# ansonb/FeTA_TMLR

Hardware: AMD Instinct MI355X
Metric: graphs/sec fwd+bwd, ZINC batch (N<=37,d=64,K=16) (higher is better)
Workload: dtype f32; 1 GPU; ZINC-shaped synthetic padded-graph batch, ChebConvDynamic block (attention + coefficient generator + spectral filter), fwd+bwd; graphs_per_gpu=128, global_batch=128, n_pad=37, d_model=64, heads=4, filter_order=4, k_eig=16, filter_mode=spectral, layers=3, norm=batch(per-rank stats), hip_graph=True, backward=single, two_phase=False, graph_collectives=False, ranks=1, parallelism=dp1

## Files before the change

feta_tmlr_amd/build.py:

```python
import os
import subprocess
import sys
from concurrent.futures import ThreadPoolExecutor

PKG = os.path.dirname(os.path.abspath(__file__))
ROOT = os.path.dirname(PKG)
CSRC = os.path.join(PKG, 'csrc')
OUT = os.path.join(PKG, 'libfeta_hip.so')
OBJ = os.path.join(PKG, 'csrc', 'build')
ARCH = 'gfx950'


def _hipcc():
    for c in (os.environ.get('HIPCC'), '/opt/rocm/bin/hipcc', 'hipcc'):
        if c and (os.path.isabs(c) and os.path.exists(c) or not os.path.isabs(c)):
            return c
    raise RuntimeError('hipcc not found')


def sources():
    return sorted(os.path.join(CSRC, f) for f in os.listdir(CSRC) if f.endswith('.hip'))


def _deps():
    hdr = [os.path.join(CSRC, f) for f in os.listdir(CSRC) if f.endswith('.h')]
    return hdr + [os.path.join(ROOT, 'include', 'feta_hip.h'), os.path.abspath(__file__)]


def build(force=False, report=False, verbose=True):
    os.makedirs(OBJ, exist_ok=True)
    flags = ['--offload-arch=' + ARCH, '-O3', '-std=c++17', '-fPIC',
             '-I' + os.path.join(ROOT, 'include'), '-I' + CSRC]
    if report:
        flags.append('-Rpass-analysis=kernel-resource-usage')
    dep_t = max(os.path.getmtime(p) for p in _deps())
    jobs = []
    for src in sources():
        obj = os.path.join(OBJ, os.path.basename(src)[:-4] + '.o')
        if force or not os.path.exists(obj) or os.path.getmtime(obj) < max(os.path.getmtime(src), dep_t):
            jobs.append((src, obj))

    def cc(job):
        src, obj = job
        r = subprocess.run([_hipcc()] + flags + ['-c', src, '-o', obj], capture_output=True, text=True)
        return job, r

    with ThreadPoolExecutor(max_workers=min(4, max(1, len(jobs)))) as ex:
        for (src, obj), r in ex.map(cc, jobs):
            if r.returncode != 0:
                raise RuntimeError('hipcc failed on %s:\n%s' % (src, r.stderr[-4000:]))
            if report:
                sys.stderr.write(r.stderr)
            if verbose:
                print('hipcc -c', os.path.relpath(src, ROOT))
    objs = [os.path.join(OBJ, os.path.basename(s)[:-4] + '.o') for s in sources()]
    if jobs or not os.path.exists(OUT):
        r = subprocess.run([_hipcc(), '--offload-arch=' + ARCH, '-shared', '-fPIC', '-o', OUT] + objs,
                           capture_output=True, text=True)
        if r.returncode != 0:
            raise RuntimeError('link failed:\n' + r.stderr[-4000:])
        if verbose:
            print('linked', os.path.relpath(OUT, ROOT))
    return OUT


if __name__ == '__main__':
    build(force='--force' in sys.argv, report='--report' in sys.argv)
```

feta_tmlr_amd/csrc/block.hip:

```cpp
#include <cstdlib>
#include <type_traits>

#include "feta_abi_common.h"
#include "feta_colsum.h"
#include "feta_ln.h"
#include "feta_lp.h"
#include "feta_rowops.h"

namespace feta {

typedef feta_attn_block BlockArgs;

constexpr int kBlkD = 64, kBlkH = 4, kBlkDH = 16;
constexpr int kBlkP = kBlkD + 4;
constexpr int kBlkMaxGrid = 256;

template <class T>
__host__ __device__ inline int block_lds_bytes(int nt, bool attn) {
  const int nr = 16 * nt, P = kBlkD + Lp<T>::PAD;
  int b = (int)sizeof(T) * (3 * kBlkD * P + kBlkD * P);
  b += (int)sizeof(T) * 2 * nr * P;
  int f = 2 * kBlkD;
  const int fin = reduce_scratch_floats(kBlkD);
  const int stg = attn ? kBlkH * 16 * (nr + 1) : 0;
// ... 113 lines not shown
        a.x_bn_out[3 * D + c] = rstd;
        if (a.x_rmean != nullptr) {
          const float unbiased = a.M > 1 ? var * (float)a.M / (float)(a.M - 1) : var;
          a.x_rmean[c] = (1.0f - a.momentum) * a.x_rmean[c] + a.momentum * mean;
          a.x_rvar[c] = (1.0f - a.momentum) * a.x_rvar[c] + a.momentum * unbiased;
        }
        if (c == 0 && a.x_nbt != nullptr) *a.x_nbt += 1;
      }
    }
  } else if (a.x_bn != nullptr) {
    for (int c = tid; c < 2 * D; c += kRowThreads) xss[c] = a.x_bn[c];
  } else if (a.x_ln_gamma != nullptr) {
    for (int c = tid; c < 2 * D; c += kRowThreads) xss[c] = c < D ? a.x_ln_gamma[c] : a.x_ln_beta[c - D];
  }
  const bool x_ln = a.x_ln_gamma != nullptr;
  FETA_STAMP(7);
  bool first = true;
  for (int b = blockIdx.x; b < a.B; b += main_grid) {
  if (!first) {
    __syncthreads();
    request_graph(b);
  }
  const bool late_weights = first && weights_last;
  first = false;
  if (late_weights) lds_barrier();
  else __syncthreads();
#pragma unroll
  for (int i = 0; i < XI; ++i) {
    const int idx = tid + kRowThreads * i, node = idx / RV, q = idx % RV;
    if (XI * kRowThreads != NR * RV && idx >= NR * RV) continue;
    Vec v = xv[i];
    if (x_norm) {
      float f[L::VEC];
      L::unpack(v, f);
#pragma unroll
      for (int e = 0; e < L::VEC; ++e) f[e] = f[e] * xss[L::VEC * q + e] + xss[D + L::VEC * q + e];
      v = L::pack(f);
    } else if (x_ln) {
      float f[L::VEC];
      L::unpack(v, f);
      ln_apply<L::VEC>(f, xss + L::VEC * q, xss + D + L::VEC * q, a.eps);
      v = L::pack(f);
    }
    L::stv(Xs + node * P + L::VEC * q, v);
  }
  {
    const float rn = 1.0f / (float)a.N;
#pragma unroll
    for (int i = 0; i < PEI; ++i) {
      const int idx = tid + kRowThreads * i;
      const int qq = (int)(((float)idx + 0.5f) * rn), kk = idx - qq * a.N;
      if (idx < nn) Pe[qq * PEP + kk] = pel[i];
    }
  }
  if (late_weights) store_weights();
  __syncthreads();
  FETA_STAMP(1);

  Op qs[NT], kf[NT], vbo[NT];
  {
    RowOp<T, D> xf[NT];
#pragma unroll
    for (int nt = 0; nt < NT; ++nt) load_row_op<T, D>(xf[nt], Xs + (16 * nt + lq) * P, g);
#pragma unroll
    for (int part = 0; part < 3; ++part) {
      if (part == 1 && a.tie_qk) continue;
      RowOp<T, D> wf;
      load_row_op<T, D>(wf, Wi + (part * D + DH * h + lq) * P, g);
      const float4 bv4 = bin4[part];
      const float bv1 = bin1;
#pragma unroll
      for (int nt = 0; nt < NT; ++nt) {
        const int node = 16 * nt + lq;
        if (part > 0 && 16 * nt >= n) {
          if (part == 1) kf[nt] = L::zero();
          else vbo[nt] = L::zero();
          continue;
        }
        if (part < 2) {
          f32x4 t = dot_row_ops<T, D>(wf, xf[nt], zero4());
          t[0] += bv4.x; t[1] += bv4.y; t[2] += bv4.z; t[3] += bv4.w;
          if (node < a.N) {
            const int64_t row = (int64_t)b * a.row_sb + (int64_t)node * a.row_sn;
            L::st4(gqkv + row * 3 * D + part * D + DH * h + 4 * g, t[0], t[1], t[2], t[3]);
          }
          if (part == 0) {
            qs[nt] = L::mk(t[0] * a.scale, t[1] * a.scale, t[2] * a.scale, t[3] * a.scale);
            if (a.tie_qk) kf[nt] = L::mk(t);
          } else {
            kf[nt] = L::mk(t);
          }
        } else {
          f32x4 t = dot_row_ops<T, D>(xf[nt], wf, zero4());
#pragma unroll
          for (int r = 0; r < 4; ++r) {
            t[r] += bv1;
            const int nd = 16 * nt + 4 * g + r;
            if (nd < a.N) {
              const int64_t row = (int64_t)b * a.row_sb + (int64_t)nd * a.row_sn;
              L::st1(gqkv + row * 3 * D + 2 * D + DH * h + lq, t[r]);
            }
            if (nd >= n) t[r] = 0.0f;
          }
          vbo[nt] = L::mk(t);
        }
      }
    }
  }

  FETA_STAMP(2);
  const int bh = b * kBlkH + h;
  float* stg = scr + h * 16 * KP;
  f32x4 acc[NT][NT];
#pragma unroll
  for (int kt = 0; kt < NT; ++kt) {
#pragma unroll
    for (int qb = 0; qb < NT; ++qb) acc[qb][kt] = zero4();
    if (16 * kt < n) {
#pragma unroll
      for (int qb = 0; qb < NT; ++qb) acc[qb][kt] = L::mma(kf[kt], qs[qb], zero4());
    }
  }
  float mx[NT], zs[NT], rinv[NT];
#pragma unroll
  for (int qb = 0; qb < NT; ++qb) {
    float m = -INFINITY;
#pragma unroll
    for (int kt = 0; kt < NT; ++kt)
#pragma unroll
      for (int r = 0; r < 4; ++r)
        if (16 * kt + 4 * g + r < n) m = fmaxf(m, acc[qb][kt][r]);
    mx[qb] = m;
  }
#pragma unroll
  for (int qb = 0; qb < NT; ++qb) mx[qb] = fmaxf(mx[qb], shfl_xor(mx[qb], 16));
#pragma unroll
  for (int qb = 0; qb < NT; ++qb) mx[qb] = fmaxf(mx[qb], shfl_xor(mx[qb], 32));
#pragma unroll
  for (int qb = 0; qb < NT; ++qb) zs[qb] = 0.0f;
  float pv[NT][NT][4];
#pragma unroll
  for (int qb = 0; qb < NT; ++qb) {
    const int qc = min(16 * qb + lq, a.N - 1);
#pragma unroll
    for (int kt = 0; kt < NT; ++kt) {
      const float4 t = *reinterpret_cast<const float4*>(Pe + qc * PEP + 16 * kt + 4 * g);
      pv[qb][kt][0] = t.x; pv[qb][kt][1] = t.y; pv[qb][kt][2] = t.z; pv[qb][kt][3] = t.w;
    }
  }
#pragma unroll
  for (int kt = 0; kt < NT; ++kt) {
    if (16 * kt >= n) continue;
#pragma unroll
    for (int qb = 0; qb < NT; ++qb)
#pragma unroll
      for (int r = 0; r < 4; ++r) {
        const bool kok = 16 * kt + 4 * g + r < n;
        const float e = kok ? fast_exp(acc[qb][kt][r] - mx[qb]) * pv[qb][kt][r] : 0.0f;
        acc[qb][kt][r] = e;
        zs[qb] += e;
      }
  }
#pragma unroll
  for (int qb = 0; qb < NT; ++qb) zs[qb] += shfl_xor(zs[qb], 16);
#pragma unroll
  for (int qb = 0; qb < NT; ++qb) zs[qb] += shfl_xor(zs[qb], 32);
  f32x4 o[NT];
#pragma unroll
  for (int qb = 0; qb < NT; ++qb) {
    rinv[qb] = 1.0f / fmaxf(zs[qb], 1e-6f);
    o[qb] = zero4();
    const int q = 16 * qb + lq;
    if (g == 0 && q < a.N) {
      float* st = a.attn_stats + ((int64_t)bh * a.N + q) * 2;
      st[0] = mx[qb];
      st[1] = zs[qb];
    }
  }
#pragma unroll
  for (int kt = 0; kt < NT; ++kt) {
    if (16 * kt >= n) continue;
#pragma unroll
    for (int qb = 0; qb < NT; ++qb) {
#pragma unroll
      for (int r = 0; r < 4; ++r) acc[qb][kt][r] *= rinv[qb];
      o[qb] = L::mma(L::mk(acc[qb][kt]), vbo[kt], o[qb]);
    }
  }
#pragma unroll
  for (int qb = 0; qb < NT; ++qb)
#pragma unroll
    for (int r = 0; r < 4; ++r) L::st1(Os + (16 * qb + 4 * g + r) * P + DH * h + lq, o[qb][r]);
  if (a.attn != nullptr) {
#pragma unroll
    for (int qb = 0; qb < NT; ++qb) {
#pragma unroll
      for (int kt = 0; kt < NT; ++kt)
#pragma unroll
        for (int r = 0; r < 4; ++r) stg[lq * KP + 16 * kt + 4 * g + r] = acc[qb][kt][r];
      wave_lds_sync();
      const int rows = min(16, a.N - 16 * qb);
      float* dst = a.attn + ((int64_t)bh * a.N + 16 * qb) * a.N;
      for (int i = lane; i < rows * a.N; i += 64) {
        const int qq = i / a.N, kk = i - qq * a.N;
        dst[i] = stg[qq * KP + kk];
      }
      wave_lds_sync();
    }
  }
  FETA_STAMP(3);
  __syncthreads();
  FETA_STAMP(4);

#pragma unroll
  for (int i = 0; i < XI; ++i) {
    const int idx = tid + kRowThreads * i, node = idx / RV, q = idx % RV;
    if (node < a.N) {
      const int64_t row = (int64_t)b * a.row_sb + (int64_t)node * a.row_sn;
      const Vec ov = L::ldv(Os + node * P + L::VEC * q);
      L::stv(gout + row * D + L::VEC * q, ov);
      if (a.out_f32 != nullptr) {
        float f[L::VEC];
        L::unpack(ov, f);
#pragma unroll
        for (int e = 0; e < L::VEC; e += 4)
          *reinterpret_cast<float4*>(a.out_f32 + row * D + L::VEC * q + e) = make_float4(f[e], f[e + 1], f[e + 2], f[e + 3]);
      }
    }
  }
  {
    RowOp<T, D> wf;
    load_row_op<T, D>(wf, Wo + (DH * h + lq) * P, g);
    const int o0 = DH * h + 4 * g;
    float s1[4] = {0.0f, 0.0f, 0.0f, 0.0f}, s2[4] = {0.0f, 0.0f, 0.0f, 0.0f};
    float4 ks = make_float4(0.0f, 0.0f, 0.0f, 0.0f);
    if (a.y_shift != nullptr) ks = *reinterpret_cast<const float4*>(a.y_shift + o0);
    const float kv[4] = {ks.x, ks.y, ks.z, ks.w};
#pragma unroll
    for (int nt = 0; nt < NT; ++nt) {
      if (16 * nt >= a.N) break;
      const int node = 16 * nt + lq;
      const bool rok = node < a.N;
      const int64_t row = (int64_t)b * a.row_sb + (int64_t)min(node, a.N - 1) * a.row_sn;
      const float rs = rsv[nt];
      RowOp<T, D> of;
      load_row_op<T, D>(of, Os + node * P, g);
      const f32x4 t = dot_row_ops<T, D>(wf, of, zero4());
      float res[4];
      L::ld4(Xs + node * P + o0, res);
      float v[4] = {(t[0] + bo.x) * rs + res[0], (t[1] + bo.y) * rs + res[1], (t[2] + bo.z) * rs + res[2],
                    (t[3] + bo.w) * rs + res[3]};
      if (rok) L::st4(gy + row * D + o0, v[0], v[1], v[2], v[3]);
      if (a.y_stats != nullptr) {
#pragma unroll
        for (int r = 0; r < 4; ++r) {
          const float x1 = rok ? v[r] - kv[r] : 0.0f;
          s1[r] += row16_sum(x1);
          s2[r] += row16_sum(x1 * x1);
        }
      }
    }
    if (lq == 0 && a.y_stats != nullptr) {
      float* st = a.y_stats + (int64_t)b * 2 * D;
      *reinterpret_cast<float4*>(st + o0) = make_float4(s1[0], s1[1], s1[2], s1[3]);
      *reinterpret_cast<float4*>(st + D + o0) = make_float4(s2[0], s2[1], s2[2], s2[3]);
      if (b == 0) *reinterpret_cast<float4*>(a.y_stats + (int64_t)a.B * 2 * D + o0) = ks;
    }
  }
  }
  FETA_STAMP(5);
  FETA_RT_LAUNCH_DONE(feta_block_launch);
}

constexpr int kBlk8Threads = 512;

template <class T>
__host__ __device__ inline int block8_region_floats(int nt) {
  const int stg = 16 * (16 * nt + 1), xch = nt * 64 * (int)sizeof(typename Lp<T>::Op) / 4;
  return stg > xch ? stg : xch;
}

template <class T>
__host__ __device__ inline int block8_lds_bytes(int nt) {
  const int nr = 16 * nt, P = kBlkD + Lp<T>::PAD;
  int b = (int)sizeof(T) * (4 * kBlkD * P + 2 * nr * P);
  int f = 2 * kBlkD + 128;
  const int fin = reduce_scratch_floats(kBlkD, kBlk8Threads), reg = 8 * block8_region_floats<T>(nt);
  f += fin > reg ? fin : reg;
  f += nr * (nr + 4);
  const int role = 4 * colsum_role_lds_floats(kBlk8Threads);
  const int tot = b + 4 * f;
  return tot > role ? tot : role;
}

template <class T, int NT, int WGS, bool TWO>
__global__ __launch_bounds__(kBlk8Threads) void attn_block_fwd8_kernel(BlockArgs a, ColsumPlan sums, int main_grid) {
  typedef Lp<T> L;
  typedef typename L::Op Op;
  typedef typename L::Vec Vec;
  constexpr int TH = kBlk8Threads;
  constexpr int D = kBlkD, DH = kBlkDH, P = kBlkD + L::PAD, NR = 16 * NT, KP = NR + 1;
  constexpr int S = 2 * WGS;
  constexpr int NQ = (NT + S - 1) / S;
  constexpr int KVU = NT >= 4 ? 2 : NT;
  constexpr int RV = D / L::VEC;
  constexpr int XI = (NR * RV + TH - 1) / TH;
  constexpr int QR = WGS == 1 ? NR : (NR < 32 ? NR : 32);
  constexpr int PEI = (QR * NR + TH - 1) / TH;
  if ((int)blockIdx.x >= main_grid) {
    colsum_role<TH>(sums, (int)blockIdx.x - main_grid);
    return;
  }
  const int tid = threadIdx.x, lane = tid & 63, wv = tid >> 6, h = wv & 3, p = wv >> 2, lq = lane & 15, g = lane >> 4;
  const int gp = main_grid / WGS;
  const int w = (int)blockIdx.x / gp, b0 = (int)blockIdx.x % gp;
  const int slot = 2 * w + p;
  T* Wi = reinterpret_cast<T*>(lds_bytes());
  T* Wo = Wi + 3 * D * P;
  T* Xs = Wo + D * P;
  T* Os = Xs + NR * P;
  float* xss = reinterpret_cast<float*>(Os + NR * P);
  float* sx = xss + 2 * D;
  float* scr = sx + 128;
  const int PER = block8_region_floats<T>(NT);
  Op* XK = reinterpret_cast<Op*>(scr + (2 * h) * PER);
  Op* XV = reinterpret_cast<Op*>(scr + (2 * h + 1) * PER);
  float* stg = scr + (2 * h + p) * PER;
  constexpr int PEP = NR + 4;
  float* Pe = reinterpret_cast<float*>(lds_bytes() + block8_lds_bytes<T>(NT)) - NR * PEP;
  const T* gx = reinterpret_cast<const T*>(a.x);
  const T* gpe = reinterpret_cast<const T*>(a.pe);
  T* gqkv = reinterpret_cast<T*>(a.qkv);
  T* gout = reinterpret_cast<T*>(a.out);
  T* gy = reinterpret_cast<T*>(a.y);
  const bool x_norm = a.x_stats != nullptr || a.x_bn != nullptr;
  FETA_STAMP(0);

  PartialBatchT<16> pb;
  partials_request_t<TH, 16>(a.x_stats != nullptr ? a.x_stats : a.w_in, a.x_stats != nullptr ? a.Gx : 0, D, pb);
  const bool has_pe = a.pe != nullptr;
  Vec xv[XI];
  T pel[PEI];
  float rsn[NQ], rsv[NQ];
  int n = 0, n_req = 0;
  const int nn = a.N * a.N;
  const int q0 = WGS == 1 ? 0 : 32 * w, q1 = WGS == 1 ? a.N : min(a.N, 32 * w + 32);
  const int pe0 = q0 * a.N, pecnt = max(q1 - q0, 0) * a.N;
  auto request_graph = [&](int b) {
    n_req = a.n_real[b];
// ... 47 lines not shown
      bn_moments_k(xk, D, a.M, scr, c, mean, var);
      const float rstd = rsqrtf(var + a.eps);
      const float scale = xg * rstd;
      const float shift = xb - mean * scale;
      xss[c] = scale;
      xss[D + c] = shift;
      if (blockIdx.x == 0) {
        a.x_bn_out[c] = scale;
        a.x_bn_out[D + c] = shift;
        a.x_bn_out[2 * D + c] = mean;
        a.x_bn_out[3 * D + c] = rstd;
        if (a.x_rmean != nullptr) {
          const float unbiased = a.M > 1 ? var * (float)a.M / (float)(a.M - 1) : var;
          a.x_rmean[c] = (1.0f - a.momentum) * a.x_rmean[c] + a.momentum * mean;
          a.x_rvar[c] = (1.0f - a.momentum) * a.x_rvar[c] + a.momentum * unbiased;
        }
        if (c == 0 && a.x_nbt != nullptr) *a.x_nbt += 1;
      }
    }
  } else if (a.x_bn != nullptr) {
    for (int c = tid; c < 2 * D; c += TH) xss[c] = a.x_bn[c];
  } else if (a.x_ln_gamma != nullptr) {
    for (int c = tid; c < 2 * D; c += TH) xss[c] = c < D ? a.x_ln_gamma[c] : a.x_ln_beta[c - D];
  }
  const bool x_ln = a.x_ln_gamma != nullptr;
  FETA_STAMP(7);
  const int lane0 = lane;
  float s1[4] = {0.0f, 0.0f, 0.0f, 0.0f}, s2[4] = {0.0f, 0.0f, 0.0f, 0.0f};
  for (int b = b0; b < a.B; b += gp) {
  n = n_req;
#pragma unroll
  for (int i = 0; i < NQ; ++i) rsv[i] = rsn[i];
  int lane_l = lane0;
  FETA_OPAQUE_LANE(lane_l);
  const int lane = lane_l, tid = (wv << 6) | lane, lq = lane & 15, g = lane >> 4;
  lds_barrier();
#pragma unroll
  for (int i = 0; i < XI; ++i) {
    const int idx = tid + TH * i, node = idx / RV, q = idx % RV;
    if (XI * TH != NR * RV && idx >= NR * RV) continue;
    Vec v = xv[i];
    if (x_norm) {
      float f[L::VEC];
      L::unpack(v, f);
#pragma unroll
      for (int e = 0; e < L::VEC; ++e) f[e] = f[e] * xss[L::VEC * q + e] + xss[D + L::VEC * q + e];
      v = L::pack(f);
    } else if (x_ln) {
      float f[L::VEC];
      L::unpack(v, f);
      ln_apply<L::VEC>(f, xss + L::VEC * q, xss + D + L::VEC * q, a.eps);
      v = L::pack(f);
    }
    L::stv(Xs + node * P + L::VEC * q, v);
  }
  {
    const float rn = 1.0f / (float)a.N;
#pragma unroll
    for (int i = 0; i < PEI; ++i) {
      const int idx = tid + TH * i, e = pe0 + idx;
      const int qq = (int)(((float)e + 0.5f) * rn), kk = e - qq * a.N;
      if (idx < pecnt) Pe[qq * PEP + kk] = L::to_f(pel[i]);
    }
  }
  if (b + gp < a.B) request_graph(b + gp);
  lds_barrier();
  FETA_STAMP(1);

  Op qs[NQ], kf[NT], vbo[NT];
  {
    {
      RowOp<T, D> wf;
      load_row_op<T, D>(wf, Wi + (DH * h + lq) * P, g);
#pragma unroll
      for (int nt = 0; nt < NT; ++nt) {
        if ((nt & (S - 1)) != slot) continue;
        const int node = 16 * nt + lq;
        RowOp<T, D> xf;
        load_row_op<T, D>(xf, Xs + node * P, g);
        f32x4 t = dot_row_ops<T, D>(wf, xf, zero4());
        t[0] += binq.x; t[1] += binq.y; t[2] += binq.z; t[3] += binq.w;
        if (node < a.N) {
          const int64_t row = (int64_t)b * a.row_sb + (int64_t)node * a.row_sn;
          L::st4(gqkv + row * 3 * D + DH * h + 4 * g, t[0], t[1], t[2], t[3]);
        }
        qs[nt / S] = L::mk(t[0] * a.scale, t[1] * a.scale, t[2] * a.scale, t[3] * a.scale);
      }
    }
    if (p == 0) {
      RowOp<T, D> wf;
      load_row_op<T, D>(wf, Wi + ((a.tie_qk ? 0 : D) + DH * h + lq) * P, g);
#pragma unroll KVU
      for (int nt = 0; nt < NT; ++nt) {
        Op kk = L::zero();
        if (16 * nt < n) {
          const int node = 16 * nt + lq;
          RowOp<T, D> xf;
          load_row_op<T, D>(xf, Xs + node * P, g);
          f32x4 t = dot_row_ops<T, D>(wf, xf, zero4());
          t[0] += bink.x; t[1] += bink.y; t[2] += bink.z; t[3] += bink.w;
          if (!a.tie_qk && node < a.N && (nt % WGS) == w) {
            const int64_t row = (int64_t)b * a.row_sb + (int64_t)node * a.row_sn;
            L::st4(gqkv + row * 3 * D + D + DH * h + 4 * g, t[0], t[1], t[2], t[3]);
          }
          kk = L::mk(t);
        }
        L::sto(XK + nt * 64 + lane, kk);
      }
    } else {
      RowOp<T, D> wf;
      load_row_op<T, D>(wf, Wi + (2 * D + DH * h + lq) * P, g);
#pragma unroll KVU
      for (int nt = 0; nt < NT; ++nt) {
        Op vv = L::zero();
        if (16 * nt < n) {
          RowOp<T, D> xf;
          load_row_op<T, D>(xf, Xs + (16 * nt + lq) * P, g);
          f32x4 t = dot_row_ops<T, D>(xf, wf, zero4());
#pragma unroll
          for (int r = 0; r < 4; ++r) {
            t[r] += bin1;
            const int nd = 16 * nt + 4 * g + r;
            if (nd < a.N && (nt % WGS) == w) {
              const int64_t row = (int64_t)b * a.row_sb + (int64_t)nd * a.row_sn;
              L::st1(gqkv + row * 3 * D + 2 * D + DH * h + lq, t[r]);
            }
            if (nd >= n) t[r] = 0.0f;
          }
          vv = L::mk(t);
        }
        L::sto(XV + nt * 64 + lane, vv);
      }
    }
  }
  lds_barrier();
#pragma unroll
  for (int nt = 0; nt < NT; ++nt) {
    kf[nt] = L::ldo(XK + nt * 64 + lane);
    vbo[nt] = L::ldo(XV + nt * 64 + lane);
  }
  FETA_STAMP(2);

  if constexpr (!TWO) {
  const int bh = b * kBlkH + h;
  float acc[NQ][NT][4];
#pragma unroll
  for (int kt = 0; kt < NT; ++kt) {
#pragma unroll
    for (int i = 0; i < NQ; ++i) {
      f32x4 t = zero4();
      if (16 * kt < n && slot + S * i < NT) t = L::mma(kf[kt], qs[i], zero4());
#pragma unroll
      for (int r = 0; r < 4; ++r) acc[i][kt][r] = t[r];
    }
  }
  float mx[NQ], zs[NQ], rinv[NQ];
#pragma unroll
  for (int i = 0; i < NQ; ++i) {
    float m = -INFINITY;
#pragma unroll
    for (int kt = 0; kt < NT; ++kt)
#pragma unroll
      for (int r = 0; r < 4; ++r)
        if (16 * kt + 4 * g + r < n) m = fmaxf(m, acc[i][kt][r]);
    mx[i] = m;
  }
#pragma unroll
  for (int i = 0; i < NQ; ++i) mx[i] = fmaxf(mx[i], shfl_xor(mx[i], 16));
#pragma unroll
  for (int i = 0; i < NQ; ++i) mx[i] = fmaxf(mx[i], shfl_xor(mx[i], 32));
#pragma unroll
  for (int i = 0; i < NQ; ++i) zs[i] = 0.0f;
#pragma unroll
  for (int kt = 0; kt < NT; ++kt) {
    if (16 * kt >= n) continue;
#pragma unroll
    for (int i = 0; i < NQ; ++i) {
      if (slot + S * i >= NT) continue;
      const int qc = min(16 * (slot + S * i) + lq, a.N - 1);
      const float4 t = *reinterpret_cast<const float4*>(Pe + qc * PEP + 16 * kt + 4 * g);
      const float pv[4] = {t.x, t.y, t.z, t.w};
#pragma unroll
      for (int r = 0; r < 4; ++r) {
        const bool kok = 16 * kt + 4 * g + r < n;
        const float e = kok ? fast_exp(acc[i][kt][r] - mx[i]) * pv[r] : 0.0f;
        acc[i][kt][r] = e;
        zs[i] += e;
      }
    }
  }
#pragma unroll
  for (int i = 0; i < NQ; ++i) zs[i] += shfl_xor(zs[i], 16);
#pragma unroll
  for (int i = 0; i < NQ; ++i) zs[i] += shfl_xor(zs[i], 32);
  f32x4 o[NQ];
#pragma unroll
  for (int i = 0; i < NQ; ++i) {
    rinv[i] = 1.0f / fmaxf(zs[i], 1e-6f);
    o[i] = zero4();
    const int qb = slot + S * i, q = 16 * qb + lq;
    if (g == 0 && qb < NT && q < a.N) {
      float* st = a.attn_stats + ((int64_t)bh * a.N + q) * 2;
      st[0] = mx[i];
      st[1] = zs[i];
    }
  }
#pragma unroll
  for (int kt = 0; kt < NT; ++kt) {
    if (16 * kt >= n) continue;
#pragma unroll
    for (int i = 0; i < NQ; ++i) {
      if (slot + S * i >= NT) continue;
#pragma unroll
      for (int r = 0; r < 4; ++r) acc[i][kt][r] *= rinv[i];
      o[i] = L::mma(L::mk(acc[i][kt][0], acc[i][kt][1], acc[i][kt][2], acc[i][kt][3]), vbo[kt], o[i]);
    }
  }
#pragma unroll
  for (int i = 0; i < NQ; ++i) {
    const int qb = slot + S * i;
    if (qb < NT) {
#pragma unroll
      for (int r = 0; r < 4; ++r) L::st1(Os + (16 * qb + 4 * g + r) * P + DH * h + lq, o[i][r]);
    }
  }
  if (a.attn != nullptr) {
    lds_barrier();
#pragma unroll
    for (int i = 0; i < NQ; ++i) {
      const int qb = slot + S * i;
      if (qb >= NT) continue;
#pragma unroll
      for (int kt = 0; kt < NT; ++kt)
#pragma unroll
        for (int r = 0; r < 4; ++r) stg[lq * KP + 16 * kt + 4 * g + r] = acc[i][kt][r];
      wave_lds_sync();
      const int rows = min(16, a.N - 16 * qb);
      float* dst = a.attn + ((int64_t)bh * a.N + 16 * qb) * a.N;
      for (int j = lane; j < rows * a.N; j += 64) {
        const int qq = j / a.N, kk = j - qq * a.N;
        dst[j] = stg[qq * KP + kk];
      }
      wave_lds_sync();
    }
  }
  } else {
  constexpr int NS = TWO ? 2 : 1;
  f32x4 o[NQ];
  auto attn_head = [&](auto shc) __attribute__((always_inline)) {
  constexpr int sh = decltype(shc)::value;
  const bool ga = (g >> 1) == sh, la = (lq >> 3) == sh;
  const int bh = b * (kBlkH * NS) + NS * h + sh;
  float acc[NQ][NT][4];
#pragma unroll
  for (int kt = 0; kt < NT; ++kt) {
#pragma unroll
    for (int i = 0; i < NQ; ++i) {
      f32x4 t = zero4();
      if (16 * kt < n && slot + S * i < NT) t = L::mma(kf[kt], L::sel(ga, qs[i], L::zero()), zero4());
#pragma unroll
      for (int r = 0; r < 4; ++r) acc[i][kt][r] = t[r];
    }
  }
  float mx[NQ], zs[NQ], rinv[NQ];
#pragma unroll
  for (int i = 0; i < NQ; ++i) {
    float m = -INFINITY;
#pragma unroll
    for (int kt = 0; kt < NT; ++kt)
#pragma unroll
      for (int r = 0; r < 4; ++r)
        if (16 * kt + 4 * g + r < n) m = fmaxf(m, acc[i][kt][r]);
    mx[i] = m;
  }
#pragma unroll
  for (int i = 0; i < NQ; ++i) mx[i] = fmaxf(mx[i], shfl_xor(mx[i], 16));
#pragma unroll
  for (int i = 0; i < NQ; ++i) mx[i] = fmaxf(mx[i], shfl_xor(mx[i], 32));
#pragma unroll
  for (int i = 0; i < NQ; ++i) zs[i] = 0.0f;
#pragma unroll
  for (int kt = 0; kt < NT; ++kt) {
    if (16 * kt >= n) continue;
#pragma unroll
    for (int i = 0; i < NQ; ++i) {
      if (slot + S * i >= NT) continue;
      const int qc = min(16 * (slot + S * i) + lq, a.N - 1);
      const float4 t = *reinterpret_cast<const float4*>(Pe + qc * PEP + 16 * kt + 4 * g);
      const float pv[4] = {t.x, t.y, t.z, t.w};
#pragma unroll
      for (int r = 0; r < 4; ++r) {
        const bool kok = 16 * kt + 4 * g + r < n;
        const float e = kok ? fast_exp(acc[i][kt][r] - mx[i]) * pv[r] : 0.0f;
        acc[i][kt][r] = e;
        zs[i] += e;
      }
    }
  }
#pragma unroll
  for (int i = 0; i < NQ; ++i) zs[i] += shfl_xor(zs[i], 16);
#pragma unroll
  for (int i = 0; i < NQ; ++i) zs[i] += shfl_xor(zs[i], 32);
#pragma unroll
  for (int i = 0; i < NQ; ++i) {
    rinv[i] = 1.0f / fmaxf(zs[i], 1e-6f);
    if (sh == 0) o[i] = zero4();
    const int qb = slot + S * i, q = 16 * qb + lq;
    if (g == 0 && qb < NT && q < a.N) {
      float* st = a.attn_stats + ((int64_t)bh * a.N + q) * 2;
      st[0] = mx[i];
      st[1] = zs[i];
    }
  }
#pragma unroll
  for (int kt = 0; kt < NT; ++kt) {
    if (16 * kt >= n) continue;
#pragma unroll
    for (int i = 0; i < NQ; ++i) {
      if (slot + S * i >= NT) continue;
#pragma unroll
      for (int r = 0; r < 4; ++r) acc[i][kt][r] *= rinv[i];
      o[i] = L::mma(L::mk(acc[i][kt][0], acc[i][kt][1], acc[i][kt][2], acc[i][kt][3]),
                    L::sel(la, vbo[kt], L::zero()), o[i]);
    }
  }
  if (sh == NS - 1) {
#pragma unroll
    for (int i = 0; i < NQ; ++i) {
      const int qb = slot + S * i;
      if (qb < NT) {
#pragma unroll
        for (int r = 0; r < 4; ++r) L::st1(Os + (16 * qb + 4 * g + r) * P + DH * h + lq, o[i][r]);
      }
    }
  }
  if (a.attn != nullptr) {
    if (sh == 0) lds_barrier();
#pragma unroll
    for (int i = 0; i < NQ; ++i) {
      const int qb = slot + S * i;
      if (qb >= NT) continue;
#pragma unroll
      for (int kt = 0; kt < NT; ++kt)
#pragma unroll
        for (int r = 0; r < 4; ++r) stg[lq * KP + 16 * kt + 4 * g + r] = acc[i][kt][r];
      wave_lds_sync();
      const int rows = min(16, a.N - 16 * qb);
      float* dst = a.attn + ((int64_t)bh * a.N + 16 * qb) * a.N;
      for (int j = lane; j < rows * a.N; j += 64) {
        const int qq = j / a.N, kk = j - qq * a.N;
        dst[j] = stg[qq * KP + kk];
      }
      wave_lds_sync();
    }
  }
  };
  attn_head(std::integral_constant<int, 0>{});
  attn_head(std::integral_constant<int, 1>{});
  }
  FETA_STAMP(3);
  lds_barrier();
  FETA_STAMP(4);

#pragma unroll
  for (int i = 0; i < XI; ++i) {
    const int idx = tid + TH * i, node = idx / RV, q = idx % RV;
    if (node < a.N && (((node >> 4) & (S - 1)) >> 1) == w) {
      const int64_t row = (int64_t)b * a.row_sb + (int64_t)node * a.row_sn;
      const Vec ov = L::ldv(Os + node * P + L::VEC * q);
      L::stv(gout + row * D + L::VEC * q, ov);
      if (a.out_f32 != nullptr) {
        float f[L::VEC];
        L::unpack(ov, f);
#pragma unroll
        for (int e = 0; e < L::VEC; e += 4)
          *reinterpret_cast<float4*>(a.out_f32 + row * D + L::VEC * q + e) = make_float4(f[e], f[e + 1], f[e + 2], f[e + 3]);
      }
    }
  }
  {
    RowOp<T, D> wf;
    load_row_op<T, D>(wf, Wo + (DH * h + lq) * P, g);
    const int o0 = DH * h + 4 * g;
    float4 ks = make_float4(0.0f, 0.0f, 0.0f, 0.0f);
    if (a.y_shift != nullptr) ks = *reinterpret_cast<const float4*>(a.y_shift + o0);
    const float kv[4] = {ks.x, ks.y, ks.z, ks.w};
#pragma unroll
    for (int i = 0; i < NQ; ++i) {
      const int qb = slot + S * i;
      if (qb >= NT) continue;
      const int node = 16 * qb + lq;
      const bool rok = node < a.N;
      const int64_t row = (int64_t)b * a.row_sb + (int64_t)min(node, a.N - 1) * a.row_sn;
      const float rs = rsv[i];
      RowOp<T, D> of;
      load_row_op<T, D>(of, Os + node * P, g);
      const f32x4 t = dot_row_ops<T, D>(wf, of, zero4());
      float res[4];
      L::ld4(Xs + node * P + o0, res);
      float v[4] = {(t[0] + bo.x) * rs + res[0], (t[1] + bo.y) * rs + res[1], (t[2] + bo.z) * rs + res[2],
                    (t[3] + bo.w) * rs + res[3]};
      if (rok) L::st4(gy + row * D + o0, v[0], v[1], v[2], v[3]);
      if (a.y_stats != nullptr) {
#pragma unroll
        for (int r = 0; r < 4; ++r) {
          const float x1 = rok ? v[r] - kv[r] : 0.0f;
          s1[r] += row16_sum(x1);
          s2[r] += row16_sum(x1 * x1);
        }
      }
    }
  }
  }
  if (a.y_stats != nullptr) {
    const int o0 = DH * h + 4 * g;
    if (p == 1 && lq == 0) {
      float* e = sx + (4 * h + g) * 8;
      *reinterpret_cast<float4*>(e) = make_float4(s1[0], s1[1], s1[2], s1[3]);
      *reinterpret_cast<float4*>(e + 4) = make_float4(s2[0], s2[1], s2[2], s2[3]);
    }
    lds_barrier();
    if (p == 0 && lq == 0) {
      const float* e = sx + (4 * h + g) * 8;
      const float4 t1 = *reinterpret_cast<const float4*>(e), t2 = *reinterpret_cast<const float4*>(e + 4);
      float* st = a.y_stats + ((int64_t)b0 * WGS + w) * 2 * D;
      *reinterpret_cast<float4*>(st + o0) = make_float4(s1[0] + t1.x, s1[1] + t1.y, s1[2] + t1.z, s1[3] + t1.w);
      *reinterpret_cast<float4*>(st + D + o0) = make_float4(s2[0] + t2.x, s2[1] + t2.y, s2[2] + t2.z, s2[3] + t2.w);
      if (b0 == 0 && w == 0) {
        float4 ks = make_float4(0.0f, 0.0f, 0.0f, 0.0f);
        if (a.y_shift != nullptr) ks = *reinterpret_cast<const float4*>(a.y_shift + o0);
        *reinterpret_cast<float4*>(a.y_stats + (int64_t)gp * WGS * 2 * D + o0) = ks;
      }
    }
  }
  FETA_STAMP(5);
  FETA_RT_LAUNCH_DONE(feta_block_launch);
}

struct BlockFwdForm {
  int waves, wgs, cap;
};
static BlockFwdForm block_fwd_form(int B, int N) {
  BlockFwdForm f{8, 1, kBlkMaxGrid};
  if (const char* e = getenv("FETA_BLOCK_MAX_GRID")) f.cap = atoi(e) > 0 ? atoi(e) : f.cap;
  if (const char* e = getenv("FETA_BLOCK_FWD_WAVES")) f.waves = atoi(e) == 4 ? 4 : 8;
  if (f.waves == 4) return f;
  const int nt = (N + 15) / 16;
  f.wgs = (nt >= 3 && 2 * B <= f.cap) ? 2 : 1;
  if (const char* e = getenv("FETA_BLOCK_FWD_WGS")) {
    const int v = atoi(e);
    if (v == 1 || (v == 2 && nt >= 3)) f.wgs = v;
  }
  return f;
}

template <class T, int NT, int WGS, bool TWO = false>
int launch_block_fwd8(const BlockArgs& a, const feta_colsum_seg* segs, int nseg, int cap, hipStream_t stream) {
  const size_t lds = block8_lds_bytes<T>(NT);
  auto kern = attn_block_fwd8_kernel<T, NT, WGS, TWO>;
  static LdsSeen lds_seen;
  allow_dynamic_lds(kern, lds, lds_seen);
  int gp = cap / WGS;
  if (gp < 1) gp = 1;
  if (a.B < gp) gp = a.B;
  const int grid = gp * WGS;
  ColsumPlan plan{};
  const int tiles = plan_colsum(segs, nseg, plan);
  hipLaunchKernelGGL(kern, dim3(grid + tiles), dim3(kBlk8Threads), lds, stream, a, plan, grid);
  return check_launch("feta_attn_block_fwd");
}

template <class T, int NT>
int launch_block_fwd(const BlockArgs& a, const feta_colsum_seg* segs, int nseg, hipStream_t stream) {
  const size_t lds = block_lds_bytes<T>(NT, a.attn != nullptr);
  auto kern = attn_block_fwd_kernel<T, NT>;
  static LdsSeen lds_seen;
  allow_dynamic_lds(kern, lds, lds_seen);
  int cap = kBlkMaxGrid;
  if (const char* e = getenv("FETA_BLOCK_MAX_GRID")) cap = atoi(e) > 0 ? atoi(e) : cap;
  const int grid = a.B < cap ? a.B : cap;
  ColsumPlan plan{};
  const int tiles = plan_colsum(segs, nseg, plan);
  int weights_last = 0;
  if (const char* e = getenv("FETA_BLOCK_WEIGHTS_LAST")) weights_last = atoi(e) != 0 && !(NT == 4 && sizeof(T) == sizeof(float));
  hipLaunchKernelGGL(kern, dim3(grid + tiles), dim3(kRowThreads), lds, stream, a, plan, grid, weights_last);
  return check_launch("feta_attn_block_fwd");
}

static int dispatch_block_fwd_two(const BlockArgs& a, const feta_colsum_seg* segs, int nseg, hipStream_t stream) {
  BlockFwdForm f = block_fwd_form(a.B, a.N);
  if (f.waves == 4) {
    f.wgs = 1;
    f.cap = a.B;
  }
  if (f.wgs == 2) {
    if ((a.N + 15) / 16 == 3) return launch_block_fwd8<float, 3, 2, true>(a, segs, nseg, f.cap, stream);
    return launch_block_fwd8<float, 4, 2, true>(a, segs, nseg, f.cap, stream);
  }
  switch ((a.N + 15) / 16) {
    case 1: return launch_block_fwd8<float, 1, 1, true>(a, segs, nseg, f.cap, stream);
    case 2: return launch_block_fwd8<float, 2, 1, true>(a, segs, nseg, f.cap, stream);
    case 3: return launch_block_fwd8<float, 3, 1, true>(a, segs, nseg, f.cap, stream);
    default: return launch_block_fwd8<float, 4, 1, true>(a, segs, nseg, f.cap, stream);
  }
}

template <class T>
int dispatch_block_fwd(const BlockArgs& a, const feta_colsum_seg* segs, int nseg, hipStream_t stream) {
  const BlockFwdForm f = block_fwd_form(a.B, a.N);
  if (f.waves == 8) {
    if (f.wgs == 2) {
      if ((a.N + 15) / 16 == 3) return launch_block_fwd8<T, 3, 2>(a, segs, nseg, f.cap, stream);
      return launch_block_fwd8<T, 4, 2>(a, segs, nseg, f.cap, stream);
    }
// ... 71 lines not shown
```

feta_tmlr_amd/csrc/block_bwd.hip:

```cpp
#include <cstdlib>
#include <type_traits>

#include "feta_abi_common.h"
#include "feta_colsum.h"
#include "feta_lin_dw.h"
#include "feta_ln.h"
#include "feta_lp.h"
#include "feta_rowops.h"

namespace feta {

typedef feta_attn_block_grad BwdArgs;

constexpr int kBbD = 64, kBbH = 4, kBbDH = 16;
constexpr int kBbP = kBbD + 4;
constexpr int kBbThreads = 512;
constexpr int kBbMaxGrid = 256;

template <class T>
__host__ __device__ inline int block_bwd_lds_bytes(int nt, bool gbn, bool gln = false, int heads = kBbH) {
  const int nr = 16 * nt, P = kBbD + Lp<T>::PAD;
  return (int)sizeof(T) * 7 * nr * P
         + 4 * (nr * (nr + 1)
                + heads * nr * 2 + nr
                + 8 * kBbD + 8 * 2 * 16
                + (gbn ? 5 * kBbD + reduce_scratch_floats(kBbD, 512) : 0)
                + (gln ? 8 * 2 * kBbD : 0));
}

#ifdef FETA_TIMING
__device__ unsigned long long feta_bbwd_stamps[4 * 8 * 8];
__device__ unsigned int feta_bbwd_launch;
#endif
#define BB_STAMP(i) FETA_RT_STAMP(feta_bbwd_stamps, feta_bbwd_launch, i)

__device__ __forceinline__ void acc_to(float* p, float v, bool first) {
  if (first) *p = v;
  else atomicAdd(p, v);
}

static_assert(kDwThreads == kBbThreads, "the dW role is written for the workgroup size of attn_block_bwd_kernel");

template <class T, int NT, bool SPLIT, bool LOOP, bool TWO, bool DW = false>
__global__ __launch_bounds__(kBbThreads) void attn_block_bwd_kernel(BwdArgs a, ColsumPlan sums, int main_grid, LinDwHost<DW> dw) {
  static_assert(!DW || (std::is_same<T, float>::value && !SPLIT && !LOOP), "the dW role: fp32, one workgroup per graph");
  if ((int)blockIdx.x >= main_grid) {
    int rb = (int)blockIdx.x - main_grid;
    if constexpr (DW) {
      if (rb < dw.p.wgs) {
        lin_dw_role(dw.p, rb);
        return;
      }
      rb -= dw.p.wgs;
    }
    colsum_role<kBbThreads>(sums, rb);
    return;
  }
  typedef Lp<T> L;
  typedef typename L::Op Op;
  typedef typename L::Vec Vec;
  constexpr int NS = TWO ? 2 : 1;
  constexpr int D = kBbD, DH = kBbDH, H = kBbH * NS, P = kBbD + L::PAD, NR = 16 * NT, PEP = NR + 1;
  constexpr int VEC = L::VEC, RV = D / VEC;
  const int tid = threadIdx.x, lane = tid & 63, wv = tid >> 6, lq = lane & 15, g = lane >> 4;
  const int hp = SPLIT ? ((int)blockIdx.x >= a.B ? 1 : 0) : 0;
  const int h = SPLIT ? 2 * hp + (wv & 1) : (wv & 3);
  const int role = SPLIT ? ((wv >> 1) & 1) : (wv >> 2);
  const int half = wv >> 2;
  const int ct = SPLIT ? 2 * hp + (wv & 1) : (wv & 3);
  const int ktile = wv & 3;
  auto mine_dc = [&](int rt) { return SPLIT ? rt == (wv >> 1) : (rt & 1) == (wv >> 2); };
  auto mine_dx = [&](int rt) { return (rt & 1) == (wv >> 2); };
  T* Qs = reinterpret_cast<T*>(lds_bytes());
  T* Ks = Qs + NR * P;
  T* Vs = Ks + NR * P;
  T* Ds = Vs + NR * P;
  T* Os = Ds + NR * P;
  T* Gt = Os + NR * P;
  T* X0 = Gt + NR * P;
  float* PE = reinterpret_cast<float*>(X0 + NR * P);
  float* ST = PE + NR * PEP;
  float* RS = ST + H * NR * 2;
  float* DBO = RS + NR;
  float* DBS = DBO + 8 * D;
  float* gv = DBS + 8 * 2 * 16;
  const T* gdy = reinterpret_cast<const T*>(a.dy);
  const T* gy1 = reinterpret_cast<const T*>(a.y1);
  const T* gqkv = reinterpret_cast<const T*>(a.qkv);
  const T* gout = reinterpret_cast<const T*>(a.out);
  const T* gd2 = reinterpret_cast<const T*>(a.dout2);
  const T* gpe = reinterpret_cast<const T*>(a.pe);
  const T* gx0 = reinterpret_cast<const T*>(a.x0);
  const bool gbn = a.bn1 != nullptr;
  const bool gln = a.ln1_gamma != nullptr, x0ln = a.x0_ln_gamma != nullptr;
  const bool has_y1 = a.y1 != nullptr;
  float* DGL = gv;
  const bool has_pe = a.pe != nullptr;
  const bool want_sums = a.sum_out != nullptr;
  const bool xbn = a.bn0 != nullptr;
  const bool d2_f32 = a.dout2 != nullptr && a.dout2_f32 != 0 && sizeof(T) != sizeof(float);
  BB_STAMP(0);

  if (gbn) {
    float* scr = gv + 5 * D;
    const int cpre = min(tid, D - 1);
    const float bn_scale = a.bn1[cpre], bn_mean = a.bn1[2 * D + cpre], bn_rstd = a.bn1[3 * D + cpre];
    if (a.g_sum != nullptr) {
      reduce_partials_t<kBbThreads, 16>(a.g_sum, a.Gs, D, scr + 2 * D, scr);
      for (int c = tid; c < D; c += kBbThreads) {
        gv[3 * D + c] = scr[c] / (float)a.M;
        gv[4 * D + c] = scr[D + c] / (float)a.M;
        if (blockIdx.x == 0) {
          if (a.dbeta != nullptr) a.dbeta[c] = scr[c];
          if (a.dgamma != nullptr) a.dgamma[c] = scr[D + c];
          if (a.fin_out != nullptr) {
            a.fin_out[c] = gv[3 * D + c];
            a.fin_out[D + c] = gv[4 * D + c];
          }
        }
      }
    }
    if (tid < D) {
      gv[tid] = bn_scale;
      gv[D + tid] = bn_mean;
      gv[2 * D + tid] = bn_rstd;
    }
    __syncthreads();
  }
// ... 113 lines not shown
          for (int e = 0; e < VEC; ++e) f[e] = keep ? f[e] : 0.0f;
          L::stv(dst + off, L::pack(f));
        };
        put(Qs, qv[i], rk);
        put(Ks, kv[i], rkv);
        put(Vs, vv[i], rkv);
        put(Os, ov[i], rk);
        if (x0ln) {
          float f[VEC];
          L::unpack(x0v[i], f);
          ln_apply<VEC>(f, gl0, bl0, a.ln_eps);
#pragma unroll
          for (int e = 0; e < VEC; ++e) f[e] = rk ? f[e] : 0.0f;
          L::stv(X0 + off, L::pack(f));
        } else {
          put(X0, x0v[i], rk);
        }
        put(Ds, d2v[i], dk2);
        float v[VEC];
        L::unpack(dyv[i], v);
        if (gln) {
          float yy[VEC];
          L::unpack(y1v[i], yy);
          ln_backward<VEC>(v, yy, gl1, a.ln_eps, rk, dgam, dbet);
        }
        if (gbn) {
          float yy[VEC];
          L::unpack(y1v[i], yy);
#pragma unroll
          for (int s = 0; s < VEC; ++s) {
            const int o = c4 + s;
            const float xh = (yy[s] - gv[D + o]) * gv[2 * D + o];
            v[s] = gv[o] * (v[s] - gv[3 * D + o] - xh * gv[4 * D + o]);
          }
        }
#pragma unroll
        for (int s = 0; s < VEC; ++s) {
          v[s] = rk ? v[s] : 0.0f;
          dbo[s] += rsn[i] * v[s];
        }
        L::stv(Gt + off, L::pack(v));
      }
    }
#pragma unroll
    for (int e = 0; e < VEC; ++e) {
      float sv = dbo[e];
      if (RV <= 8) sv += shfl_xor(sv, 8);
      sv += shfl_xor(sv, 16);
      sv += shfl_xor(sv, 32);
      if (lane < RV) DBO[wv * D + VEC * lane + e] = sv;
    }
    if (gln) {
#pragma unroll
      for (int e = 0; e < VEC; ++e) {
        float sg = dgam[e], sb = dbet[e];
        if (RV <= 8) {
          sg += shfl_xor(sg, 8);
          sb += shfl_xor(sb, 8);
        }
        sg += shfl_xor(sg, 16);
        sb += shfl_xor(sb, 16);
        sg += shfl_xor(sg, 32);
        sb += shfl_xor(sb, 32);
        if (lane < RV) {
          DGL[(wv * 2 + 0) * D + VEC * lane + e] = sg;
          DGL[(wv * 2 + 1) * D + VEC * lane + e] = sb;
        }
      }
    }
#pragma unroll
    for (int i = 0; i < PEI; ++i) {
      const int idx = tid + kBbThreads * i;
      if (idx < NR * NR) PE[(idx / NR) * PEP + idx % NR] = pev[i];
    }
    __syncthreads();
    BB_STAMP(2);
    float* prow = a.partial + (int64_t)(SPLIT ? b : (int)blockIdx.x) *
                                  (a.partial_ld > 0 ? (int64_t)a.partial_ld
                                                    : (int64_t)(4 * D * D + 4 * D + (gln ? 2 * D : 0)));
    if (hp == 0 && tid < D) {
      float sv = 0.0f;
#pragma unroll
      for (int w8 = 0; w8 < 8; ++w8) sv += DBO[w8 * D + tid];
      acc_to(prow + D * D + tid, sv, first);
    }
    if (gln && hp == 0 && tid >= D && tid < 3 * D) {
      const int which = (tid - D) / D, c = (tid - D) % D;
      float sv = 0.0f;
#pragma unroll
      for (int w8 = 0; w8 < 8; ++w8) sv += DGL[(w8 * 2 + which) * D + c];
      acc_to(prow + 4 * D * D + 4 * D + which * D + c, sv, first);
    }

    {
      Op woA[4];
#pragma unroll
      for (int j = 0; j < 4; ++j) {
        const feta_gcf p = w_out_p + (int64_t)(16 * j + 4 * g) * D + 16 * ct + lq;
        woA[j] = L::mk(p[0], p[D], p[2 * D], p[3 * D]);
      }
#pragma unroll
      for (int rt = 0; rt < NT; ++rt) {
        if (!mine_dc(rt)) continue;
        const int rowl = 16 * rt + lq;
        RowOp<T, D> gf;
        load_row_op_scaled<T, D>(gf, Gt + rowl * P, g, RS[rowl]);
        f32x4 acc = zero4();
#pragma unroll
        for (int j = 0; j < 4; ++j) acc = L::mma(woA[j], gf.o[j], acc);
        T* dst = Ds + rowl * P + 16 * ct + 4 * g;
        float d2[4];
        L::ld4(dst, d2);
        L::st4(dst, acc[0] + d2[0], acc[1] + d2[1], acc[2] + d2[2], acc[3] + d2[3]);
      }
    }
    __syncthreads();
    BB_STAMP(3);

    const int co = DH * h;
    f32x4 r0[NT], r1[NT];
#pragma unroll
    for (int t = 0; t < NT; ++t) {
      r0[t] = zero4();
      r1[t] = zero4();
    }
    if constexpr (!TWO) {
    if (role == 0) {
      Op kf[NT], vf[NT], kb[NT];
#pragma unroll
      for (int t = 0; t < NT; ++t) {
        const int rowl = 16 * t + lq;
        kf[t] = L::ld(Ks + rowl * P + co + 4 * g);
        vf[t] = L::ld(Vs + rowl * P + co + 4 * g);
        kb[t] = L::gather(Ks + (16 * t + 4 * g) * P + co + lq, P);
      }
#pragma unroll
      for (int qb = 0; qb < NT; ++qb) {
        const int q = 16 * qb + lq;
        const Op qf = L::ld_scaled(Qs + q * P + co + 4 * g, a.scale);
        const Op dof = L::ld(Ds + q * P + co + 4 * g);
        const Op of = L::ld(Os + q * P + co + 4 * g);
        float delta = L::get(dof, 0) * L::get(of, 0) + L::get(dof, 1) * L::get(of, 1) + L::get(dof, 2) * L::get(of, 2) +
                      L::get(dof, 3) * L::get(of, 3);
        delta += shfl_xor(delta, 16);
        delta += shfl_xor(delta, 32);
        const float m = ST[(h * NR + q) * 2], z = ST[(h * NR + q) * 2 + 1];
        const float rinv = fast_rcp(fmaxf(z, 1e-6f));
        if (z < 1e-6f) delta = 0.0f;
#pragma unroll
        for (int kt = 0; kt < NT; ++kt) {
          if (16 * kt >= n) continue;
          if (SPLIT && ((qb * NT + kt) & 1) != half) continue;
          const f32x4 s = L::mma(kf[kt], qf, zero4());
          const f32x4 da = L::mma(vf[kt], dof, zero4());
          float pd[4];
#pragma unroll
          for (int r = 0; r < 4; ++r) {
            const int key = 16 * kt + 4 * g + r;
            const float p = key < n ? fast_exp(s[r] - m) * PE[q * PEP + key] * rinv : 0.0f;
            pd[r] = p * (da[r] - delta);
          }
          r0[qb] = L::mma(L::mk(pd[0], pd[1], pd[2], pd[3]), kb[kt], r0[qb]);
        }
      }
    } else {
      Op qf[NT], dof[NT], qb4[NT], dob[NT];
      float sd[NT][4], mq[NT][4], rz[NT][4];
#pragma unroll
      for (int t = 0; t < NT; ++t) {
        const int rowl = 16 * t + lq;
        qf[t] = L::ld_scaled(Qs + rowl * P + co + 4 * g, a.scale);
        dof[t] = L::ld(Ds + rowl * P + co + 4 * g);
        const T* colq = Qs + (16 * t + 4 * g) * P + co + lq;
        const T* cold = Ds + (16 * t + 4 * g) * P + co + lq;
// ... 102 lines not shown
          const int rr = 16 * t + 4 * g + r;
          const bool ok = rr < a.N;
          dv4[r] = L::ld1(cold + r * P);
          qv4[r] = L::ld1(colq + r * P) * a.scale;
          if (!la) dv4[r] = qv4[r] = 0.0f;
          sd[t][r] = row16_sum(dv4[r] * L::ld1(colo + r * P));
          const float z = ST[(hs * NR + rr) * 2 + 1];
          mq[t][r] = ST[(hs * NR + rr) * 2];
          rz[t][r] = ok ? fast_rcp(fmaxf(z, 1e-6f)) : 0.0f;
          if (z < 1e-6f) sd[t][r] = 0.0f;
        }
        qb4[t] = L::mk(qv4[0], qv4[1], qv4[2], qv4[3]);
        dob[t] = L::mk(dv4[0], dv4[1], dv4[2], dv4[3]);
      }
#pragma unroll
      for (int kt = 0; kt < NT; ++kt) {
        if (16 * kt >= n) continue;
        const int key = 16 * kt + lq;
        const Op kf = L::ld(Ks + key * P + co + 4 * g);
        const Op vf = L::ld(Vs + key * P + co + 4 * g);
#pragma unroll
        for (int qb = 0; qb < NT; ++qb) {
          if (SPLIT && ((kt * NT + qb) & 1) != half) continue;
          const Op qfq = LOOP ? mg(L::ld_scaled(Qs + (16 * qb + lq) * P + co + 4 * g, a.scale)) : qf[qb];
          const Op dfq = LOOP ? mg(L::ld(Ds + (16 * qb + lq) * P + co + 4 * g)) : dof[qb];
          const f32x4 s = L::mma(qfq, kf, zero4());
          const f32x4 da = L::mma(dfq, vf, zero4());
          float pp[4], ds[4];
#pragma unroll
          for (int r = 0; r < 4; ++r) {
            const int q = 16 * qb + 4 * g + r;
            pp[r] = key < n ? fast_exp(s[r] - mq[qb][r]) * PE[q * PEP + key] * rz[qb][r] : 0.0f;
            ds[r] = pp[r] * (da[r] - sd[qb][r]);
          }
          r1[kt] = L::mma(L::mk(pp[0], pp[1], pp[2], pp[3]), dob[qb], r1[kt]);
          r0[kt] = L::mma(L::mk(ds[0], ds[1], ds[2], ds[3]), qb4[qb], r0[kt]);
        }
      }
    }
    };
    attn_head(std::integral_constant<int, 0>{});
    attn_head(std::integral_constant<int, 1>{});
    }
    {
      float c0 = 0.0f, c1 = 0.0f;
#pragma unroll
      for (int t = 0; t < NT; ++t)
#pragma unroll
        for (int r = 0; r < 4; ++r) {
          c0 += r0[t][r];
          c1 += r1[t][r];
        }
      c0 += shfl_xor(c0, 16);
      c0 += shfl_xor(c0, 32);
      c1 += shfl_xor(c1, 16);
      c1 += shfl_xor(c1, 32);
      if (g == 0) {
        DBS[(wv * 2 + 0) * 16 + lq] = role == 0 ? c0 * a.scale : c0;
        DBS[(wv * 2 + 1) * 16 + lq] = c1;
      }
    }
    constexpr int NWO = SPLIT ? 2 : 4;
    if (role == 0) {
      const int ot = SPLIT ? (wv & 1) + 2 * (wv >> 2) : (wv & 3);
      f32x4 aWo[NWO];
#pragma unroll
      for (int i = 0; i < NWO; ++i) aWo[i] = zero4();
#pragma unroll 1
      for (int q4 = 0; q4 < NT; ++q4) {
        const int rr = 16 * q4 + g;
        float gvv[4];
#pragma unroll
        for (int s4 = 0; s4 < 4; ++s4) gvv[s4] = RS[rr + 4 * s4] * L::ld1(Gt + (rr + 4 * s4) * P + 16 * ot + lq);
        const Op ga = L::mk(gvv[0], gvv[1], gvv[2], gvv[3]);
#pragma unroll
        for (int i = 0; i < NWO; ++i)
          aWo[i] = L::mma(ga, L::gather(Os + rr * P + 16 * (SPLIT ? 2 * hp + i : i) + lq, 4 * P), aWo[i]);
      }
#pragma unroll
      for (int i = 0; i < NWO; ++i)
#pragma unroll
        for (int r = 0; r < 4; ++r)
        {
          acc_to(prow + (int64_t)(16 * ot + 4 * g + r) * D + 16 * (SPLIT ? 2 * hp + i : i) + lq, aWo[i][r], first);
        }
    }
    BB_STAMP(4);
    __syncthreads();
#pragma unroll
    for (int pass = 0; pass < (SPLIT ? 2 : 1); ++pass) {
      if (!SPLIT || half == pass) {
#pragma unroll
        for (int t = 0; t < NT; ++t) {
#pragma unroll
          for (int r = 0; r < 4; ++r) {
            const int rr = 16 * t + 4 * g + r;
            if (role == 0) {
              T* dq = Qs + rr * P + co + lq;
              L::st1(dq, (pass == 0 ? 0.0f : L::ld1(dq)) + r0[t][r] * a.scale);
            } else {
              T* dk = Ks + rr * P + co + lq;
              T* dv = Vs + rr * P + co + lq;
              L::st1(dk, (pass == 0 ? 0.0f : L::ld1(dk)) + r0[t][r]);
              L::st1(dv, (pass == 0 ? 0.0f : L::ld1(dv)) + r1[t][r]);
            }
          }
        }
      }
      __syncthreads();
    }

    BB_STAMP(5);
    constexpr int NJX = SPLIT ? 2 : 4;
    f32x4 dxa[NT];
#pragma unroll
    for (int rt = 0; rt < NT; ++rt) dxa[rt] = zero4();
#pragma unroll
    for (int part = 0; part < 3; ++part) {
      Op wiA[NJX];
#pragma unroll
      for (int j = 0; j < NJX; ++j) {
        const feta_gcf p = w_in_p + (int64_t)(64 * part + 16 * (SPLIT ? 2 * hp + j : j) + 4 * g) * D + 16 * ktile + lq;
        wiA[j] = L::mk(p[0], p[D], p[2 * D], p[3 * D]);
      }
#pragma unroll
      for (int rt = 0; rt < NT; ++rt) {
        if (!mine_dx(rt)) continue;
        const T* drow = (part == 0 ? Qs : (part == 1 ? Ks : Vs)) + (16 * rt + lq) * P + (SPLIT ? 32 * hp : 0);
#pragma unroll
        for (int j = 0; j < NJX; ++j) dxa[rt] = L::mma(wiA[j], L::ld(drow + 16 * j + 4 * g), dxa[rt]);
      }
    }
    T* dxo = reinterpret_cast<T*>((SPLIT && hp == 1) ? a.dx_b : a.dx);
    const float resw = (SPLIT && hp == 1) ? 0.0f : 1.0f;
#pragma unroll
    for (int rt = 0; rt < NT; ++rt) {
      if (!mine_dx(rt)) continue;
      const int rowl = 16 * rt + lq;
      const f32x4 acc = dxa[rt];
      float res[4];
      L::ld4(Gt + rowl * P + 16 * ktile + 4 * g, res);
      const float v[4] = {acc[0] + resw * res[0], acc[1] + resw * res[1], acc[2] + resw * res[2], acc[3] + resw * res[3]};
      const bool rok = rowl < a.N;
      if (rok) L::st4(dxo + grow(rowl) * D + 16 * ktile + 4 * g, v[0], v[1], v[2], v[3]);
      if (want_sums) {
        float xx[4];
        L::ld4(X0 + rowl * P + 16 * ktile + 4 * g, xx);
#pragma unroll
        for (int r = 0; r < 4; ++r) {
          const float s1 = rok ? v[r] : 0.0f;
          sum1[r] += s1;
          sum2[r] += s1 * (xx[r] - mean0[r]) * rstd0[r];
        }
      }
    }
    if (want_sums) {
      float s1v[4], s2v[4];
#pragma unroll
      for (int r = 0; r < 4; ++r) {
        s1v[r] = row16_sum(sum1[r]);
        s2v[r] = row16_sum(sum2[r]);
      }
      if (SPLIT) {
        float* red = PE;
        if ((wv >> 2) == 1 && lq == 0) {
#pragma unroll
          for (int r = 0; r < 4; ++r) {
            red[(ktile * 2 + 0) * 16 + 4 * g + r] = s1v[r];
            red[(ktile * 2 + 1) * 16 + 4 * g + r] = s2v[r];
          }
        }
        __syncthreads();
        if ((wv >> 2) == 0 && lq == 0) {
#pragma unroll
          for (int r = 0; r < 4; ++r) {
            a.sum_out[((int64_t)blockIdx.x * 2 + 0) * D + 16 * ktile + 4 * g + r] = s1v[r] + red[(ktile * 2 + 0) * 16 + 4 * g + r];
            a.sum_out[((int64_t)blockIdx.x * 2 + 1) * D + 16 * ktile + 4 * g + r] = s2v[r] + red[(ktile * 2 + 1) * 16 + 4 * g + r];
          }
        }
      } else if (lq == 0 && (!LOOP || b + nwg >= a.B)) {
        const int64_t prow2 = (int64_t)blockIdx.x * 2 + (wv >> 2);
#pragma unroll
        for (int r = 0; r < 4; ++r) {
          a.sum_out[(prow2 * 2 + 0) * D + 16 * ktile + 4 * g + r] = s1v[r];
          a.sum_out[(prow2 * 2 + 1) * D + 16 * ktile + 4 * g + r] = s2v[r];
        }
      }
    }

    BB_STAMP(6);
    constexpr int NWI = SPLIT ? 3 : 6;
    const int grp = wv >> 2;
    f32x4 aWi[NWI];
#pragma unroll
    for (int i = 0; i < NWI; ++i) aWi[i] = zero4();
    auto wi_part = [&](int i) { return SPLIT ? (3 * grp + i) >> 1 : (6 * grp + i) >> 2; };
    auto wi_head = [&](int i) { return SPLIT ? 2 * hp + ((3 * grp + i) & 1) : ((6 * grp + i) & 3); };
#pragma unroll 1
    for (int q4 = 0; q4 < NT; ++q4) {
      const int rr = 16 * q4 + g;
      float xv4[4];
#pragma unroll
      for (int s4 = 0; s4 < 4; ++s4) xv4[s4] = L::ld1(X0 + (rr + 4 * s4) * P + 16 * ktile + lq) * sc0 + sh0;
      const Op xb = L::mk(xv4[0], xv4[1], xv4[2], xv4[3]);
#pragma unroll
      for (int i = 0; i < NWI; ++i) {
        const int part = wi_part(i);
        const T* src = part == 0 ? Qs : (part == 1 ? Ks : Vs);
        aWi[i] = L::mma(L::gather(src + rr * P + 16 * wi_head(i) + lq, 4 * P), xb, aWi[i]);
      }
    }
    float* pWi = prow + D * D + D;
    float* pbi = pWi + 3 * D * D;
#pragma unroll
    for (int i = 0; i < NWI; ++i)
#pragma unroll
      for (int r = 0; r < 4; ++r)
      {
        acc_to(pWi + (int64_t)(64 * wi_part(i) + 16 * wi_head(i) + 4 * g + r) * D + 16 * ktile + lq, aWi[i][r], first);
      }
    if (tid < 3 * D) {
      const int part = tid >> 6, hh = (tid >> 4) & 3, c = tid & 15;
      const int rl = part == 0 ? 0 : 1, which = part == 2 ? 1 : 0;
      if (SPLIT) {
        if ((hh >> 1) == hp) {
          const int wa = (hh & 1) + 2 * rl;
          pbi[tid] = DBS[(wa * 2 + which) * 16 + c] + DBS[((wa + 4) * 2 + which) * 16 + c];
        }
      } else {
        acc_to(pbi + tid, DBS[((hh + 4 * rl) * 2 + which) * 16 + c], first);
      }
    }
    b += nwg;
  } while (LOOP && b < a.B);
  BB_STAMP(7);
  FETA_RT_LAUNCH_DONE(feta_bbwd_launch);
}

template <int NT, bool TWO>
size_t block_bwd_dw_lds() {
  size_t lds = block_bwd_lds_bytes<float>(NT, true, false, TWO ? 2 * kBbH : kBbH);
  const size_t lds_ln = block_bwd_lds_bytes<float>(NT, false, true, TWO ? 2 * kBbH : kBbH);
  if (lds < lds_ln) lds = lds_ln;
  if (lds < (size_t)lin_dw_lds_bytes()) lds = lin_dw_lds_bytes();
  if (lds < sizeof(float) * colsum_role_lds_floats(kBbThreads)) lds = sizeof(float) * colsum_role_lds_floats(kBbThreads);
  return lds;
}
template <int NT, bool TWO>
int block_bwd_dw_slots() {
  static std::atomic<int> slots[kMaxDevices];
  int dev = 0;
  if (hipGetDevice(&dev) != hipSuccess || dev < 0 || dev >= kMaxDevices) {
    (void)hipGetLastError();
    return 0;
  }
  int have = slots[dev].load(std::memory_order_acquire);
  if (have == 0) {
    const size_t lds = block_bwd_dw_lds<NT, TWO>();
    auto kern = attn_block_bwd_kernel<float, NT, false, false, TWO, true>;
    static LdsSeen lds_seen;
    allow_dynamic_lds(kern, lds, lds_seen);
    int cus = 0, per = 0;
    if (hipDeviceGetAttribute(&cus, hipDeviceAttributeMultiprocessorCount, dev) != hipSuccess ||
        hipOccupancyMaxActiveBlocksPerMultiprocessor(&per, kern, kBbThreads, lds) != hipSuccess || cus < 1 || per < 1) {
      (void)hipGetLastError();
      return 0;
    }
    have = cus * per;
    slots[dev].store(have, std::memory_order_release);
  }
  return have;
}
static int block_bwd_dw_slots_of(int N, int heads) {
  const bool two = heads == 8;
  switch ((N + 15) / 16) {
    case 1: return two ? block_bwd_dw_slots<1, true>() : block_bwd_dw_slots<1, false>();
    case 2: return two ? block_bwd_dw_slots<2, true>() : block_bwd_dw_slots<2, false>();
    case 3: return two ? block_bwd_dw_slots<3, true>() : block_bwd_dw_slots<3, false>();
    default: return two ? block_bwd_dw_slots<4, true>() : block_bwd_dw_slots<4, false>();
  }
}
static int block_bwd_dw_wgs(int slots, int grid, int tiles) {
  if (const char* e = getenv("FETA_LIN_DW_WGS")) if (atoi(e) > 0) return atoi(e) < tiles ? atoi(e) : tiles;
  int free_slots = slots - grid;
  if (free_slots < 1) return 0;
  if (free_slots > tiles) free_slots = tiles;
  return free_slots >= 8 ? (free_slots & ~7) : free_slots;
}

template <class T, int NT, bool TWO = false>
int launch_block_bwd(const BwdArgs& a, const feta_colsum_seg* segs, int nseg, const feta_lin_dw* dw, hipStream_t stream) {
  size_t lds = block_bwd_lds_bytes<T>(NT, a.bn1 != nullptr, a.ln1_gamma != nullptr, TWO ? 2 * kBbH : kBbH);
  const int grid = feta_attn_block_bwd_blocks(a.B);
  ColsumPlan plan{};
  const int tiles = plan_colsum(segs, nseg, plan);
  if (tiles > 0 && lds < sizeof(float) * colsum_role_lds_floats(kBbThreads)) lds = sizeof(float) * colsum_role_lds_floats(kBbThreads);
  if (a.dx_b != nullptr) {
    auto kern = attn_block_bwd_kernel<T, NT, true, false, TWO>;
    static LdsSeen lds_seen;
    allow_dynamic_lds(kern, lds, lds_seen);
    hipLaunchKernelGGL(kern, dim3(2 * a.B + tiles), dim3(kBbThreads), lds, stream, a, plan, 2 * a.B, LinDwHost<false>{});
  } else if (grid == a.B) {
    if constexpr (std::is_same<T, float>::value) {
      if (dw != nullptr) {
        LinDwHost<true> host{};
        LinDwPlan& p = host.p;
        p.dy = dw->dy; p.x = dw->x; p.dw = dw->dw; p.db = dw->db;
        p.R = dw->R; p.K = dw->K; p.N = dw->N;
        p.tj = dw->K / kDwJ;
        p.tiles = lin_dw_tiles(dw->K, dw->N);
        p.wgs = block_bwd_dw_wgs(block_bwd_dw_slots<NT, TWO>(), grid, p.tiles);
        FETA_REQUIRE(p.wgs > 0, "attn_block_bwd_sums_dw: %d graphs leave no workgroup slot free (feta_attn_block_bwd_dw_supported)", a.B);
        lds = block_bwd_dw_lds<NT, TWO>();
// ... 127 lines not shown
```

feta_tmlr_amd/csrc/feta_coeff.h:

```cpp
#pragma once
#include <cmath>

#include "feta_abi_common.h"
#include <feta_device.h>

namespace feta {

constexpr int kCoeffThreads = 256;
constexpr int kCoeffWideThreads = 1024;
constexpr int kCoeffGroupsMax = 128;
constexpr int kCoeffLdsTileMax = 12 * 1024;

template <int TH = 256>
__device__ __forceinline__ void coeff_fwd_body(
    const float* __restrict__ attn, const int32_t* __restrict__ n_real, const float* __restrict__ s,
    const float* __restrict__ gbias, float* __restrict__ cj_out, float* __restrict__ pooled, int B,
    int N, int H, int C, int stage, int blk, int cs = 0, int CS = 1) {
  float* dis = feta_lds;
  float* cjs = feta_lds + N;
  float* ps = feta_lds + 2 * N;
  float* tile = ps + 4 * 64;
  const int h = blk / B, b = blk % B;
  const int n = n_real[b];
  const float* a = attn + ((int64_t)b * H + h) * N * N;
  const int j = threadIdx.x;

  if (stage && N <= 64) {
    const int cnt = n * N;
    float v[16];
#pragma unroll
    for (int u = 0; u < 16; ++u) {
      const int idx = threadIdx.x + u * TH;
      v[u] = a[idx < cnt ? idx : (cnt > 0 ? cnt - 1 : 0)];
    }
#pragma unroll
    for (int u = 0; u < 16; ++u) {
      const int idx = threadIdx.x + u * TH;
      if (idx < cnt) tile[idx] = v[u];
    }
    __syncthreads();
    const int col = threadIdx.x & 63, sl = threadIdx.x >> 6;
    float wjj = 0.0f;
    if (col < n) {
      wjj = tile[col * N + col];
      if (wjj == 0.0f) wjj = 1.0f;
    }
    float part = 0.0f;
    if (col < n)
      for (int i = sl; i < n; i += 4) part += (i == col) ? wjj : tile[i * N + col];
    ps[sl * 64 + col] = part;
    __syncthreads();
    if (sl == 0 && col < n) {
      const float deg = (ps[col] + ps[64 + col]) + (ps[128 + col] + ps[192 + col]);
      dis[col] = deg > 0.0f ? rsqrtf(deg) : 0.0f;
    }
    __syncthreads();
    part = 0.0f;
    if (col < n)
      for (int i = sl; i < n; i += 4) part += dis[i] * ((i == col) ? wjj : tile[i * N + col]);
    __syncthreads();
    ps[sl * 64 + col] = part;
    __syncthreads();
    if (sl == 0 && col < N) {
      float c = 0.0f;
      if (col < n) c = ((ps[col] + ps[64 + col]) + (ps[128 + col] + ps[192 + col])) * dis[col];
      cjs[col] = c;
      if (cs == 0) cj_out[(int64_t)blk * N + col] = c;
    }
    __syncthreads();
  } else if (stage == 2) {
    const int NP = (N + 3) & ~3, NC4 = NP >> 2, SL = TH / NC4;
    float* ps2 = feta_lds + 2 * N;
    float* tl = ps2 + 4 * TH;
    if ((N & 3) == 0) {
      const int cnt4 = n * NC4;
      const float4* a4 = reinterpret_cast<const float4*>(a);
      for (int base = threadIdx.x; base < cnt4; base += 8 * TH) {
        float4 v[8];
#pragma unroll
        for (int u = 0; u < 8; ++u) {
          const int idx = base + u * TH;
          v[u] = a4[idx < cnt4 ? idx : cnt4 - 1];
        }
#pragma unroll
        for (int u = 0; u < 8; ++u) {
          const int idx = base + u * TH;
          if (idx < cnt4) reinterpret_cast<float4*>(tl)[idx] = v[u];
        }
      }
    } else {
      const int cnt = n * N;
      for (int base = threadIdx.x; base < cnt; base += 8 * TH) {
        float v[8];
#pragma unroll
        for (int u = 0; u < 8; ++u) {
          const int idx = base + u * TH;
          v[u] = a[idx < cnt ? idx : cnt - 1];
        }
#pragma unroll
        for (int u = 0; u < 8; ++u) {
          const int idx = base + u * TH;
          if (idx < cnt) tl[(idx / N) * NP + idx % N] = v[u];
        }
      }
      for (int i = threadIdx.x; i < n * (NP - N); i += TH) tl[(i / (NP - N)) * NP + N + i % (NP - N)] = 0.0f;
    }
    __syncthreads();
    const int cg = threadIdx.x % NC4, sl = threadIdx.x / NC4;
    const bool act = sl < SL;
    float4 acc = make_float4(0.0f, 0.0f, 0.0f, 0.0f);
    if (act)
      for (int i = sl; i < n; i += SL) {
        const float4 v = *reinterpret_cast<const float4*>(tl + i * NP + 4 * cg);
        acc.x += v.x; acc.y += v.y; acc.z += v.z; acc.w += v.w;
      }
    if (act) *reinterpret_cast<float4*>(ps2 + sl * NP + 4 * cg) = acc;
    __syncthreads();
    float dj = 0.0f, diag0 = 0.0f;
    if (j < n) {
      float deg = 0.0f;
      for (int q = 0; q < SL; ++q) deg += ps2[q * NP + j];
      diag0 = tl[j * NP + j] == 0.0f ? 1.0f : 0.0f;
      deg += diag0;
      dj = deg > 0.0f ? rsqrtf(deg) : 0.0f;
      dis[j] = dj;
    }
    __syncthreads();
    acc = make_float4(0.0f, 0.0f, 0.0f, 0.0f);
    if (act)
      for (int i = sl; i < n; i += SL) {
        const float4 v = *reinterpret_cast<const float4*>(tl + i * NP + 4 * cg);
        const float di = dis[i];
        acc.x += di * v.x; acc.y += di * v.y; acc.z += di * v.z; acc.w += di * v.w;
      }
    if (act) *reinterpret_cast<float4*>(ps2 + sl * NP + 4 * cg) = acc;
    __syncthreads();
    if (j < N) {
      float c = 0.0f;
      if (j < n) {
        for (int q = 0; q < SL; ++q) c += ps2[q * NP + j];
        c = (c + diag0 * dj) * dj;
      }
      cjs[j] = c;
      if (cs == 0) cj_out[(int64_t)blk * N + j] = c;
    }
    __syncthreads();
  } else {
    const float* src = a;
    if (stage) {
      const int cnt = n * N;
      for (int base = threadIdx.x; base < cnt; base += 8 * TH) {
        float v[8];
#pragma unroll
        for (int u = 0; u < 8; ++u) {
          const int idx = base + u * TH;
          v[u] = a[idx < cnt ? idx : cnt - 1];
        }
#pragma unroll
        for (int u = 0; u < 8; ++u) {
          const int idx = base + u * TH;
          if (idx < cnt) tile[idx] = v[u];
        }
      }
      __syncthreads();
      src = tile;
    }
    float wjj = 0.0f, deg = 0.0f;
    if (j < n) {
      wjj = src[j * N + j];
      if (wjj == 0.0f) wjj = 1.0f;
      for (int i = 0; i < n; ++i) deg += (i == j) ? wjj : src[i * N + j];
      dis[j] = deg > 0.0f ? rsqrtf(deg) : 0.0f;
    }
    __syncthreads();
    if (j < N) {
      float c = 0.0f;
      if (j < n) {
        for (int i = 0; i < n; ++i) c += dis[i] * ((i == j) ? wjj : src[i * N + j]);
        c *= dis[j];
      }
      cjs[j] = c;
      if (cs == 0) cj_out[(int64_t)blk * N + j] = c;
    }
    __syncthreads();
  }
  const float inv_n = 1.0f / (float)n;
  const int cw = ((C + CS - 1) / CS + TH - 1) / TH * TH;
  const int cend = min(C, (cs + 1) * cw);
  if (cw < 4 * TH) {
    for (int c = cs * cw + threadIdx.x; c < cend; c += TH) {
      const float sc = s[c], bc = gbias[c];
      float acc = 0.0f;
      for (int i = 0; i < n; ++i) acc += fast_tanh(cjs[i] * sc + bc);
      pooled[(int64_t)blk * C + c] = acc * inv_n;
    }
    return;
  }
  for (int c0 = cs * cw + threadIdx.x; c0 < cend; c0 += 4 * TH) {
    float sc[4], bc[4], acc[4];
#pragma unroll
    for (int k = 0; k < 4; ++k) {
      const int c = min(c0 + k * TH, C - 1);
      sc[k] = s[c];
      bc[k] = gbias[c];
      acc[k] = 0.0f;
    }
#pragma unroll 2
    for (int i = 0; i < n; ++i) {
      const float ci = cjs[i];
#pragma unroll
      for (int k = 0; k < 4; ++k) acc[k] += fast_tanh(ci * sc[k] + bc[k]);
    }
#pragma unroll
    for (int k = 0; k < 4; ++k) {
      const int c = c0 + k * TH;
      if (c < cend) pooled[(int64_t)blk * C + c] = acc[k] * inv_n;
    }
  }
}

constexpr int kCoeffPass = 4;
__device__ __forceinline__ void coeff_bwd_body(
    const float* __restrict__ cj, const int32_t* __restrict__ n_real, const float* __restrict__ s,
    const float* __restrict__ gbias, const float* __restrict__ dpooled, float* __restrict__ partial,
    int B, int N, int H, int C, int G, int bx, int grp) {
  float* cjs = feta_lds;
  const int c = bx * kCoeffThreads + threadIdx.x;
  const int cc = c < C ? c : C - 1;
  const int total = B * H;
  const float sc = s[cc], bc = gbias[cc];
  float as = 0.0f, ab = 0.0f;
  for (int blk0 = grp; blk0 < total; blk0 += G * kCoeffPass) {
    float dp[kCoeffPass];
    int nn[kCoeffPass];
#pragma unroll
    for (int u = 0; u < kCoeffPass; ++u) {
      const int blk = blk0 + u * G;
      const int bc_ = blk < total ? blk : total - 1;
      nn[u] = blk < total ? n_real[bc_ % B] : 0;
      dp[u] = dpooled[(int64_t)bc_ * C + cc];
    }
    __syncthreads();
    for (int i = threadIdx.x; i < kCoeffPass * N; i += kCoeffThreads) {
      const int u = i / N, k = i - u * N;
      const int blk = blk0 + u * G;
      cjs[i] = blk < total ? cj[(int64_t)blk * N + k] : 0.0f;
    }
    __syncthreads();
    int nmax = 0;
#pragma unroll
    for (int u = 0; u < kCoeffPass; ++u) nmax = max(nmax, nn[u]);
    if (N <= 64 && (int64_t)total * N <= 32768) {
      float dpn[kCoeffPass], as_[kCoeffPass], ab_[kCoeffPass];
#pragma unroll
      for (int u = 0; u < kCoeffPass; ++u) {
        dpn[u] = nn[u] > 0 ? dp[u] / (float)nn[u] : 0.0f;
        as_[u] = ab_[u] = 0.0f;
      }
      for (int i = 0; i < nmax; ++i) {
#pragma unroll
        for (int u = 0; u < kCoeffPass; ++u) {
          const float ci = cjs[u * N + i];
          const float z = fast_tanh(ci * sc + bc);
          const float t = i < nn[u] ? dpn[u] * (1.0f - z * z) : 0.0f;
          as_[u] += t * ci;
          ab_[u] += t;
        }
      }
#pragma unroll
      for (int u = 0; u < kCoeffPass; ++u) {
        as += as_[u];
        ab += ab_[u];
      }
    } else {
#pragma unroll
      for (int u = 0; u < kCoeffPass; ++u) {
        const int n = nn[u];
        if (n == 0) continue;
        const float dpn = dp[u] / (float)n;
        for (int i = 0; i < n; ++i) {
          const float ci = cjs[u * N + i];
          const float z = fast_tanh(ci * sc + bc);
          const float t = dpn * (1.0f - z * z);
          as += t * ci;
          ab += t;
        }
      }
    }
  }
  if (c < C) {
    partial[(int64_t)grp * 2 * C + c] = as;
    partial[(int64_t)grp * 2 * C + C + c] = ab;
  }
}


__device__ __forceinline__ void coeff_dsum_body(
    const float* __restrict__ cj, const int32_t* __restrict__ n_real, const float* __restrict__ s,
    const float* __restrict__ gbias, float* __restrict__ A, float* __restrict__ Bm, int B, int N, int C, int blk) {
  float* cjs = feta_lds;
  const int n = min(n_real[blk % B], N);
  __syncthreads();
  for (int i = threadIdx.x; i < N; i += kCoeffThreads) cjs[i] = cj[(int64_t)blk * N + i];
  __syncthreads();
  const float inv_n = n > 0 ? 1.0f / (float)n : 0.0f;
  for (int c0 = threadIdx.x; c0 < C; c0 += 4 * kCoeffThreads) {
    float sc[4], bc[4], as[4], ab[4];
#pragma unroll
    for (int k = 0; k < 4; ++k) {
      const int c = min(c0 + k * kCoeffThreads, C - 1);
      sc[k] = s[c];
      bc[k] = gbias[c];
      as[k] = ab[k] = 0.0f;
    }
#pragma unroll 2
    for (int i = 0; i < n; ++i) {
      const float ci = cjs[i];
#pragma unroll
      for (int k = 0; k < 4; ++k) {
        const float z = fast_tanh(ci * sc[k] + bc[k]);
        const float t = 1.0f - z * z;
        as[k] += t * ci;
        ab[k] += t;
      }
    }
#pragma unroll
    for (int k = 0; k < 4; ++k) {
      const int c = c0 + k * kCoeffThreads;
      if (c < C) {
        A[(int64_t)blk * C + c] = as[k] * inv_n;
        Bm[(int64_t)blk * C + c] = ab[k] * inv_n;
      }
    }
  }
}

__host__ __device__ inline int coeff_bwd_saved_groups(int total) {
  const int g = total / 64 > 8 ? total / 64 : 8;
  return total < g ? total : g;
}

constexpr int kCoeffSavedPass = 8;
__device__ __forceinline__ void coeff_bwd_saved_body(
    const float* __restrict__ dpooled, const float* __restrict__ A, const float* __restrict__ Bm,
    float* __restrict__ partial, int total, int C, int G, int bx, int grp) {
  const int c = bx * kCoeffThreads + threadIdx.x;
  const int cc = c < C ? c : C - 1;
  float as = 0.0f, ab = 0.0f;
  for (int blk0 = grp; blk0 < total; blk0 += G * kCoeffSavedPass) {
    float dp[kCoeffSavedPass], av[kCoeffSavedPass], bv[kCoeffSavedPass];
#pragma unroll
    for (int u = 0; u < kCoeffSavedPass; ++u) {
      const int blk = blk0 + u * G;
      const int64_t o = (int64_t)(blk < total ? blk : total - 1) * C + cc;
      dp[u] = blk < total ? dpooled[o] : 0.0f;
      av[u] = blk < total ? A[o] : 0.0f;
      bv[u] = blk < total ? Bm[o] : 0.0f;
    }
#pragma unroll
    for (int u = 0; u < kCoeffSavedPass; ++u) {
      as += dp[u] * av[u];
      ab += dp[u] * bv[u];
    }
  }
  if (c < C) {
    partial[(int64_t)grp * 2 * C + c] = as;
    partial[(int64_t)grp * 2 * C + C + c] = ab;
  }
}

__host__ __device__ inline int coeff_fwd_stage(int N) {
  if (N <= 64) return 1;
  return N * ((N + 3) & ~3) <= kCoeffLdsTileMax ? 2 : 0;
}
__host__ __device__ inline int coeff_fwd_lds_floats_mode(int N, int stage, int threads = kCoeffThreads) {
  return 2 * N + (stage == 2 ? 4 * threads + N * ((N + 3) & ~3) : 4 * 64 + (stage == 1 ? N * N : 0));
}
__host__ __device__ inline int coeff_fwd_lds_floats(int N) { return coeff_fwd_lds_floats_mode(N, coeff_fwd_stage(N)); }

struct CoeffFwdRole {
  const float* attn; const int32_t* n_real; const float* s; const float* gbias; float* cj; float* pooled;
  int B, N, H, C;
};
struct CoeffBwdRole {
  const float* cj; const int32_t* n_real; const float* s; const float* gbias; const float* dpooled; float* partial;
  int B, N, H, C, G;
  const float* A; const float* Bm;
};
struct CoeffDsumRole {
  const float* cj; const int32_t* n_real; const float* s; const float* gbias; float* A; float* Bm;
  int B, N, H, C;
};

}
```

feta_tmlr_amd/csrc/feta_colsum.h:

```cpp
#pragma once
#include <cstdlib>

#include "feta_abi_common.h"
#include <feta_device.h>

namespace feta {

constexpr int kColsumRoleThreads = 256;
constexpr int kColsumMixedThreads = 1024;

struct ColsumPlan {
  feta_colsum_seg seg[FETA_COLSUM_MAX_SEGS];
  int tile_end[FETA_COLSUM_MAX_SEGS];
  int wide[FETA_COLSUM_MAX_SEGS];
  int nseg;
  int wq;
};

inline bool colsum_seg_ok(const feta_colsum_seg& s) {
  return s.in && s.out && s.R > 0 && s.C > 0 && (s.ld == 0 || s.ld >= s.C) && (s.bcast_out == nullptr || s.bcast_rows > 0);
}

inline bool colsum_seg_wide(const feta_colsum_seg& s, int min_cols) {
  const int ld = s.ld > 0 ? s.ld : s.C;
  return s.R <= 512 && s.C >= min_cols && (s.C & 3) == 0 && (ld & 3) == 0 && aligned16(s.in) && aligned16(s.out) &&
         s.bcast_out == nullptr;
}

constexpr int colsum_wide_q(int threads) { return threads >= 1024 ? 64 : 256; }
inline int colsum_wide_adapt() {
  const char* e = getenv("FETA_COLSUM_ADAPT");
  return (e != nullptr && e[0] == '0') ? 0 : 1;
}

inline int plan_colsum(const feta_colsum_seg* segs, int nseg, ColsumPlan& p, int threads = 256) {
  int wq = colsum_wide_q(threads);
  p.nseg = nseg;
  for (;;) {
    int tiles = 0;
    for (int i = 0; i < nseg; ++i) {
      const bool wide = colsum_seg_wide(segs[i], 4096);
      p.seg[i] = segs[i];
      p.wide[i] = wide ? 1 : 0;
      tiles += wide ? (segs[i].C / 4 + wq - 1) / wq : (segs[i].C + 15) / 16;
      p.tile_end[i] = tiles;
    }
    p.wq = wq;
    if (threads < 1024 || tiles <= 512 || wq >= 256 || colsum_wide_adapt() == 0) return tiles;
    wq *= 2;
  }
}

constexpr int colsum_role_lds_floats(int threads) { return threads > 256 ? 4 * threads : threads; }

__device__ __forceinline__ void add4(float4& a, const float4& v) {
  a.x += v.x; a.y += v.y; a.z += v.z; a.w += v.w;
}

template <int THREADS>
__device__ __forceinline__ void colsum_role(const ColsumPlan& sg, int tile_id) {
  int si = 0;
  while (si + 1 < sg.nseg && tile_id >= sg.tile_end[si]) ++si;
  const feta_colsum_seg s = sg.seg[si];
  const int tile = tile_id - (si > 0 ? sg.tile_end[si - 1] : 0);
  const int ld = s.ld > 0 ? s.ld : s.C;
  const int tid = threadIdx.x;
  if (sg.wide[si]) {
    const int WQ = sg.wq, SLW = THREADS / WQ;
    const int c4 = tile * WQ + (tid % WQ), slice = tid / WQ;
    const bool ok = c4 < s.C / 4;
    const float* p = s.in + 4 * (int64_t)(ok ? c4 : 0);
    float4 acc = make_float4(0.0f, 0.0f, 0.0f, 0.0f);
    int r = slice;
    for (; r + 7 * SLW < s.R; r += 8 * SLW) {
      float4 v[8];
#pragma unroll
      for (int i = 0; i < 8; ++i) v[i] = *reinterpret_cast<const float4*>(p + (int64_t)(r + i * SLW) * ld);
#pragma unroll
      for (int i = 0; i < 8; ++i) add4(acc, v[i]);
    }
    for (; r < s.R; r += SLW) add4(acc, *reinterpret_cast<const float4*>(p + (int64_t)r * ld));
    if (SLW > 1) {
      float4* red = reinterpret_cast<float4*>(feta_lds);
      red[tid] = acc;
      __syncthreads();
      for (int half = SLW / 2; half >= 1; half >>= 1) {
        if (slice < half) add4(red[tid], red[tid + half * WQ]);
        __syncthreads();
      }
      acc = red[tid % WQ];
    }
    if (ok && slice == 0) *reinterpret_cast<float4*>(s.out + 4 * (int64_t)c4) = acc;
    return;
  }
  constexpr int COLS = 16, SL = THREADS / COLS;
  float* red = feta_lds;
  const int lc = tid & (COLS - 1), slice = tid / COLS;
  const int col = tile * COLS + lc;
  float acc = 0.0f;
  if (col < s.C) {
    const float* p = s.in + col;
    int r = slice;
    for (; r + 3 * SL < s.R; r += 4 * SL) {
      const float v0 = p[(int64_t)r * ld], v1 = p[(int64_t)(r + SL) * ld], v2 = p[(int64_t)(r + 2 * SL) * ld],
                  v3 = p[(int64_t)(r + 3 * SL) * ld];
      acc += v0; acc += v1; acc += v2; acc += v3;
    }
    for (; r < s.R; r += SL) acc += p[(int64_t)r * ld];
  }
  red[tid] = acc;
  __syncthreads();
  for (int half = SL / 2; half >= 1; half >>= 1) {
    if (slice < half) red[tid] += red[tid + half * COLS];
    __syncthreads();
  }
  if (col < s.C) {
    const float v = red[lc];
    if (slice == 0) s.out[col] = v;
    if (s.bcast_out != nullptr)
      for (int r = slice; r < s.bcast_rows; r += SL) s.bcast_out[(int64_t)r * s.C + col] = v;
  }
}

}
```

feta_tmlr_amd/csrc/feta_device.h:

```cpp
#pragma once
#include <hip/hip_runtime.h>

typedef float f32x4 __attribute__((ext_vector_type(4)));

extern __shared__ __attribute__((aligned(16))) float feta_lds[];

#define FETA_OPAQUE_PTR(p) asm volatile("" : "+s"(p))
#define FETA_OPAQUE_LANE(x) asm volatile("" : "+v"(x))
typedef const float __attribute__((address_space(1)))* feta_gcf;

namespace feta {

__device__ __forceinline__ int lane_id() { return threadIdx.x & 63; }
__device__ __forceinline__ int wave_id() { return threadIdx.x >> 6; }

__device__ __forceinline__ f32x4 mfma16(float a, float b, f32x4 c) {
  return __builtin_amdgcn_mfma_f32_16x16x4f32(a, b, c, 0, 0, 0);
}

struct bf16_t {
  unsigned short bits;
};
struct __attribute__((aligned(8))) bf16x4_raw {
  bf16_t v[4];
};
typedef short bf16x4_mfma __attribute__((ext_vector_type(4)));

__device__ __forceinline__ float bf2f(bf16_t x) { return __builtin_bit_cast(float, (unsigned)x.bits << 16); }
__device__ __forceinline__ bf16_t f2bf(float x) {
  bf16_t r;
  r.bits = __builtin_bit_cast(unsigned short, static_cast<__bf16>(x));
  return r;
}
__device__ __forceinline__ f32x4 mfma16_bf16(const float (&a)[4], const float (&b)[4], f32x4 c) {
  bf16x4_mfma av, bv;
#pragma unroll
  for (int i = 0; i < 4; ++i) {
    av[i] = (short)f2bf(a[i]).bits;
    bv[i] = (short)f2bf(b[i]).bits;
  }
  return __builtin_amdgcn_mfma_f32_16x16x16bf16_1k(av, bv, c, 0, 0, 0);
}

struct __attribute__((aligned(8))) bf16x4_pk {
  bf16x4_mfma v;
};
__device__ __forceinline__ bf16x4_pk pack_bf16x4(float a, float b, float c, float d) {
  typedef __bf16 bf16x4_native __attribute__((ext_vector_type(4)));
  const f32x4 v = {a, b, c, d};
  bf16x4_pk r;
  r.v = __builtin_bit_cast(bf16x4_mfma, __builtin_convertvector(v, bf16x4_native));
  return r;
}
__device__ __forceinline__ bf16x4_pk pack_bf16x4_raw(bf16_t a, bf16_t b, bf16_t c, bf16_t d) {
  bf16x4_pk r;
  r.v[0] = (short)a.bits; r.v[1] = (short)b.bits; r.v[2] = (short)c.bits; r.v[3] = (short)d.bits;
  return r;
}
__device__ __forceinline__ float bf16x4_get(const bf16x4_pk& p, int i) {
  bf16_t t;
  t.bits = (unsigned short)p.v[i];
  return bf2f(t);
}
__device__ __forceinline__ f32x4 mfma16_bf16_pk(const bf16x4_pk& a, const bf16x4_pk& b, f32x4 c) {
  return __builtin_amdgcn_mfma_f32_16x16x16bf16_1k(a.v, b.v, c, 0, 0, 0);
}

__device__ __forceinline__ float shfl_xor(float v, int mask) { return __shfl_xor(v, mask, 64); }
__device__ __forceinline__ float shfl(float v, int src) { return __shfl(v, src, 64); }

__device__ __forceinline__ float row16_sum(float v) {
  v += __builtin_bit_cast(float, __builtin_amdgcn_update_dpp(0, __builtin_bit_cast(int, v), 0x128, 0xf, 0xf, false));
  v += __builtin_bit_cast(float, __builtin_amdgcn_update_dpp(0, __builtin_bit_cast(int, v), 0x124, 0xf, 0xf, false));
  v += __builtin_bit_cast(float, __builtin_amdgcn_update_dpp(0, __builtin_bit_cast(int, v), 0x122, 0xf, 0xf, false));
  v += __builtin_bit_cast(float, __builtin_amdgcn_update_dpp(0, __builtin_bit_cast(int, v), 0x121, 0xf, 0xf, false));
  return v;
}

__device__ __forceinline__ float row8_sum(float v) {
  v += __builtin_bit_cast(float, __builtin_amdgcn_update_dpp(0, __builtin_bit_cast(int, v), 0xB1, 0xf, 0xf, false));
  v += __builtin_bit_cast(float, __builtin_amdgcn_update_dpp(0, __builtin_bit_cast(int, v), 0x4E, 0xf, 0xf, false));
  v += __builtin_bit_cast(float, __builtin_amdgcn_update_dpp(0, __builtin_bit_cast(int, v), 0x141, 0xf, 0xf, false));
  return v;
}

__device__ __forceinline__ void wave_lds_sync() {
  __builtin_amdgcn_fence(__ATOMIC_RELEASE, "wavefront");
  __builtin_amdgcn_wave_barrier();
  __builtin_amdgcn_fence(__ATOMIC_ACQUIRE, "wavefront");
}

__device__ __forceinline__ void lds_barrier() {
  __builtin_amdgcn_fence(__ATOMIC_RELEASE, "workgroup", "local");
  __builtin_amdgcn_s_barrier();
  __builtin_amdgcn_fence(__ATOMIC_ACQUIRE, "workgroup", "local");
}

__device__ __forceinline__ float fast_exp(float x) { return __expf(x); }
__device__ __forceinline__ float fast_tanh(float x) {
  return 1.0f - 2.0f * __builtin_amdgcn_rcpf(1.0f + __expf(2.0f * x));
}

__device__ __forceinline__ float fast_rcp(float x) { return __builtin_amdgcn_rcpf(x); }
__device__ __forceinline__ float fast_sqrt(float x) { return __builtin_amdgcn_sqrtf(x); }
__device__ __forceinline__ float fast_rsqrt(float x) { return __builtin_amdgcn_rsqf(x); }

}
```

feta_tmlr_amd/csrc/feta_lin_dw.h:

```cpp
#pragma once
#include "feta_abi_common.h"
#include <feta_device.h>
#include "feta_tiles.h"

namespace feta {

constexpr int kDwThreads = 512;
constexpr int kDwI = 128, kDwJ = 64, kDwK = 64;
constexpr int kDwPP = kDwI + 4, kDwQP = kDwJ + 4;
constexpr int kDwPSZ = kDwK * kDwPP, kDwQSZ = kDwK * kDwQP;

__host__ __device__ constexpr int lin_dw_lds_bytes() { return 2 * (kDwPSZ + kDwQSZ) * (int)sizeof(float); }

struct LinDwPlan {
  const float* dy;
  const float* x;
  float* dw;
  float* db;
  int R, K, N;
  int tj;
  int tiles;
  int wgs;
};

inline int lin_dw_tiles(int K, int N) { return (N / kDwI) * (K / kDwJ); }

inline bool lin_dw_shape_ok(int R, int K, int N) {
  return R >= kDwK && R % kDwK == 0 && K >= kDwJ && K % kDwJ == 0 && N >= kDwI && N % kDwI == 0;
}

__device__ __forceinline__ void lin_dw_tile_of(int t, int tiles, int TJ, int& ti, int& tj) {
  const int lin = (tiles & 7) == 0 ? (t & 7) * (tiles >> 3) + (t >> 3) : t;
  ti = lin / TJ;
  tj = lin - ti * TJ;
}

template <int COLS>
struct DwStage {
  static constexpr int NV = kDwK * COLS / 4 / kDwThreads;
  f32x4 v0, v1, v2, v3;
  __device__ __forceinline__ static const f32x4* at(const float* src, int64_t ld, int r0, int c0, int u) {
    const int idx = threadIdx.x + u * kDwThreads, rr = idx / (COLS / 4), c4 = idx % (COLS / 4);
    return reinterpret_cast<const f32x4*>(src + (int64_t)(r0 + rr) * ld + c0 + 4 * c4);
  }
  __device__ __forceinline__ void load(const float* src, int64_t ld, int r0, int c0) {
    v0 = *at(src, ld, r0, c0, 0);
    v1 = *at(src, ld, r0, c0, 1);
    if constexpr (NV > 2) {
      v2 = *at(src, ld, r0, c0, 2);
      v3 = *at(src, ld, r0, c0, 3);
    }
  }
  __device__ __forceinline__ static f32x4* slot(float* tile, int pitch, int u) {
    const int idx = threadIdx.x + u * kDwThreads, rr = idx / (COLS / 4), c4 = idx % (COLS / 4);
    return reinterpret_cast<f32x4*>(tile + rr * pitch + 4 * c4);
  }
  __device__ __forceinline__ void store(float* tile, int pitch) const {
    *slot(tile, pitch, 0) = v0;
    *slot(tile, pitch, 1) = v1;
    if constexpr (NV > 2) {
      *slot(tile, pitch, 2) = v2;
      *slot(tile, pitch, 3) = v3;
    }
  }
};

__device__ __forceinline__ void lin_dw_tile(const LinDwPlan& a, int ti, int tj) {
  const int lane = threadIdx.x & 63, wv = threadIdx.x >> 6, lq = lane & 15, g = lane >> 4;
  const int iw = wv & 3, jw = wv >> 2;
  float* base = feta_lds;
  const int i0 = kDwI * ti, j0 = kDwJ * tj;
  DwStage<kDwI> psA, psB;
  DwStage<kDwJ> qsA, qsB;
  const float* gp = a.dy;
  const float* gq = a.x;
  const int ldp = a.N, ldq = a.K;
  auto request = [gp, gq, ldp, ldq, i0, j0](DwStage<kDwI>& ps, DwStage<kDwJ>& qs, int c) __attribute__((always_inline)) {
    ps.load(gp, ldp, kDwK * c, i0);
    qs.load(gq, ldq, kDwK * c, j0);
  };
  float rs0 = 0.0f, rs1 = 0.0f, rs2 = 0.0f, rs3 = 0.0f;
  auto commit = [&rs0, &rs1, &rs2, &rs3, base](const DwStage<kDwI>& ps, const DwStage<kDwJ>& qs, int buf) __attribute__((always_inline)) {
    ps.store(base + buf * kDwPSZ, kDwPP);
    qs.store(base + 2 * kDwPSZ + buf * kDwQSZ, kDwQP);
    rs0 += ps.v0[0]; rs1 += ps.v0[1]; rs2 += ps.v0[2]; rs3 += ps.v0[3];
    rs0 += ps.v1[0]; rs1 += ps.v1[1]; rs2 += ps.v1[2]; rs3 += ps.v1[3];
    rs0 += ps.v2[0]; rs1 += ps.v2[1]; rs2 += ps.v2[2]; rs3 += ps.v2[3];
    rs0 += ps.v3[0]; rs1 += ps.v3[1]; rs2 += ps.v3[2]; rs3 += ps.v3[3];
  };
  f32x4 a00 = zero4(), a01 = zero4(), a10 = zero4(), a11 = zero4();
  auto compute = [&a00, &a01, &a10, &a11, base, iw, jw, lq, g](int buf) __attribute__((always_inline)) {
    const float* pt = base + buf * kDwPSZ + g * kDwPP + 32 * iw + 2 * lq;
    const float* qt = base + 2 * kDwPSZ + buf * kDwQSZ + g * kDwQP + 32 * jw + 2 * lq;
#pragma unroll
    for (int s = 0; s < kDwK / 4; ++s) {
      const float2 p = *reinterpret_cast<const float2*>(pt + 4 * s * kDwPP);
      const float2 q = *reinterpret_cast<const float2*>(qt + 4 * s * kDwQP);
      a00 = mfma16(p.x, q.x, a00);
      a01 = mfma16(p.x, q.y, a01);
      a10 = mfma16(p.y, q.x, a10);
      a11 = mfma16(p.y, q.y, a11);
    }
  };
  const int nc = a.R / kDwK;
  request(psA, qsA, 0);
  commit(psA, qsA, 0);
  if (1 < nc) request(psA, qsA, 1);
  if (2 < nc) request(psB, qsB, 2);
  __syncthreads();
  for (int c = 0; c < nc; c += 2) {
    compute(0);
    if (c + 1 < nc) commit(psA, qsA, 1);
    if (c + 3 < nc) request(psA, qsA, c + 3);
    __syncthreads();
    if (c + 1 < nc) {
      compute(1);
      if (c + 2 < nc) commit(psB, qsB, 0);
      if (c + 4 < nc) request(psB, qsB, c + 4);
      __syncthreads();
    }
  }
  float* out = a.dw + (int64_t)(i0 + 32 * iw + 8 * g) * a.K + j0 + 32 * jw + 2 * lq;
#pragma unroll
  for (int r = 0; r < 4; ++r) {
    float2 v0, v1;
    v0.x = a00[r]; v0.y = a01[r];
    v1.x = a10[r]; v1.y = a11[r];
    *reinterpret_cast<float2*>(out + (int64_t)(2 * r) * a.K) = v0;
    *reinterpret_cast<float2*>(out + (int64_t)(2 * r + 1) * a.K) = v1;
  }
  if (a.db != nullptr && tj == 0) {
    float* red = feta_lds;
    red[threadIdx.x * 4 + 0] = rs0; red[threadIdx.x * 4 + 1] = rs1;
    red[threadIdx.x * 4 + 2] = rs2; red[threadIdx.x * 4 + 3] = rs3;
    __syncthreads();
    if (threadIdx.x < kDwI) {
      const int c4 = threadIdx.x >> 2, e = threadIdx.x & 3;
      float sv = 0.0f;
      for (int k = 0; k < kDwThreads / 32; ++k) sv += red[(c4 + 32 * k) * 4 + e];
      a.db[i0 + threadIdx.x] = sv;
    }
  }
}

__device__ __forceinline__ void lin_dw_role(const LinDwPlan& a, int w) {
  for (int t = w; t < a.tiles; t += a.wgs) {
    if (t != w) __syncthreads();
    int ti, tj;
    lin_dw_tile_of(t, a.tiles, a.tj, ti, tj);
    lin_dw_tile(a, ti, tj);
  }
}

template <bool ON>
struct LinDwHost {};
template <>
struct LinDwHost<true> {
  LinDwPlan p;
};

}
```

feta_tmlr_amd/csrc/feta_lp.h:

```cpp
#pragma once
#include "feta_tiles.h"

namespace feta {

template <class T>
struct Lp;

template <>
struct Lp<float> {
  static constexpr int VEC = 4;
  static constexpr int PAD = 4;
  struct Op {
    float v[4];
  };
  struct Vec {
    float4 raw;
  };
  static __device__ __forceinline__ Op zero() { return Op{{0.0f, 0.0f, 0.0f, 0.0f}}; }
  static __device__ __forceinline__ Op mk(float a, float b, float c, float d) { return Op{{a, b, c, d}}; }
  static __device__ __forceinline__ Op mk(const f32x4& a) { return Op{{a[0], a[1], a[2], a[3]}}; }
  static __device__ __forceinline__ Op ld(const float* p) {
    const float4 x = *reinterpret_cast<const float4*>(p);
    return Op{{x.x, x.y, x.z, x.w}};
  }
  static __device__ __forceinline__ Op ldo(const Op* p) { return ld(reinterpret_cast<const float*>(p)); }
  static __device__ __forceinline__ void sto(Op* p, const Op& o) {
    *reinterpret_cast<float4*>(p) = make_float4(o.v[0], o.v[1], o.v[2], o.v[3]);
  }
  static __device__ __forceinline__ Op ld_scaled(const float* p, float s) {
    const float4 x = *reinterpret_cast<const float4*>(p);
    return Op{{x.x * s, x.y * s, x.z * s, x.w * s}};
  }
  static __device__ __forceinline__ Op gather(const float* p, int stride) {
    return Op{{p[0], p[stride], p[2 * stride], p[3 * stride]}};
  }
  static __device__ __forceinline__ float get(const Op& o, int i) { return o.v[i]; }
  static __device__ __forceinline__ Op sel(bool c, const Op& a, const Op& b) {
    return Op{{c ? a.v[0] : b.v[0], c ? a.v[1] : b.v[1], c ? a.v[2] : b.v[2], c ? a.v[3] : b.v[3]}};
  }
  static __device__ __forceinline__ f32x4 mma(const Op& a, const Op& b, f32x4 acc) {
#pragma unroll
    for (int s = 0; s < 4; ++s) acc = mfma16(a.v[s], b.v[s], acc);
    return acc;
  }
  static __device__ __forceinline__ float ld1(const float* p) { return *p; }
  static __device__ __forceinline__ float to_f(float v) { return v; }
  static __device__ __forceinline__ float one() { return 1.0f; }
  static __device__ __forceinline__ void st1(float* p, float v) { *p = v; }
  static __device__ __forceinline__ void ld4(const float* p, float (&v)[4]) {
    const float4 x = *reinterpret_cast<const float4*>(p);
    v[0] = x.x; v[1] = x.y; v[2] = x.z; v[3] = x.w;
  }
  static __device__ __forceinline__ void st4(float* p, float a, float b, float c, float d) {
    *reinterpret_cast<float4*>(p) = make_float4(a, b, c, d);
  }
  static __device__ __forceinline__ Vec ldv(const float* p) { return Vec{*reinterpret_cast<const float4*>(p)}; }
  static __device__ __forceinline__ void stv(float* p, const Vec& v) { *reinterpret_cast<float4*>(p) = v.raw; }
  static __device__ __forceinline__ void unpack(const Vec& v, float (&f)[VEC]) {
    f[0] = v.raw.x; f[1] = v.raw.y; f[2] = v.raw.z; f[3] = v.raw.w;
  }
  static __device__ __forceinline__ Vec pack(const float (&f)[VEC]) { return Vec{make_float4(f[0], f[1], f[2], f[3])}; }
};

template <>
struct Lp<bf16_t> {
  static constexpr int VEC = 8;
  static constexpr int PAD = 8;
  typedef bf16x4_pk Op;
  struct __attribute__((aligned(16))) Vec {
    bf16x4_pk lo, hi;
  };
  static __device__ __forceinline__ Op zero() { return pack_bf16x4(0.0f, 0.0f, 0.0f, 0.0f); }
  static __device__ __forceinline__ Op mk(float a, float b, float c, float d) { return pack_bf16x4(a, b, c, d); }
  static __device__ __forceinline__ Op mk(const f32x4& a) { return pack_bf16x4(a[0], a[1], a[2], a[3]); }
  static __device__ __forceinline__ Op ld(const bf16_t* p) { return *reinterpret_cast<const bf16x4_pk*>(p); }
  static __device__ __forceinline__ Op ldo(const Op* p) { return *p; }
  static __device__ __forceinline__ void sto(Op* p, const Op& o) { *p = o; }
  static __device__ __forceinline__ Op ld_scaled(const bf16_t* p, float s) {
    const Op x = ld(p);
    return pack_bf16x4(bf16x4_get(x, 0) * s, bf16x4_get(x, 1) * s, bf16x4_get(x, 2) * s, bf16x4_get(x, 3) * s);
  }
  static __device__ __forceinline__ Op gather(const bf16_t* p, int stride) {
    return pack_bf16x4_raw(p[0], p[stride], p[2 * stride], p[3 * stride]);
  }
  static __device__ __forceinline__ float get(const Op& o, int i) { return bf16x4_get(o, i); }
  static __device__ __forceinline__ Op sel(bool c, const Op& a, const Op& b) {
    Op r;
    r.v[0] = c ? a.v[0] : b.v[0]; r.v[1] = c ? a.v[1] : b.v[1]; r.v[2] = c ? a.v[2] : b.v[2]; r.v[3] = c ? a.v[3] : b.v[3];
    return r;
  }
  static __device__ __forceinline__ f32x4 mma(const Op& a, const Op& b, f32x4 acc) { return mfma16_bf16_pk(a, b, acc); }
  static __device__ __forceinline__ float ld1(const bf16_t* p) { return bf2f(*p); }
  static __device__ __forceinline__ float to_f(bf16_t v) { return bf2f(v); }
  static __device__ __forceinline__ bf16_t one() { return f2bf(1.0f); }
  static __device__ __forceinline__ void st1(bf16_t* p, float v) { *p = f2bf(v); }
  static __device__ __forceinline__ void ld4(const bf16_t* p, float (&v)[4]) {
    const Op x = ld(p);
    v[0] = bf16x4_get(x, 0); v[1] = bf16x4_get(x, 1); v[2] = bf16x4_get(x, 2); v[3] = bf16x4_get(x, 3);
  }
  static __device__ __forceinline__ void st4(bf16_t* p, float a, float b, float c, float d) {
    *reinterpret_cast<bf16x4_pk*>(p) = pack_bf16x4(a, b, c, d);
  }
  static __device__ __forceinline__ Vec ldv(const bf16_t* p) { return *reinterpret_cast<const Vec*>(p); }
  static __device__ __forceinline__ void stv(bf16_t* p, const Vec& v) { *reinterpret_cast<Vec*>(p) = v; }
  static __device__ __forceinline__ void unpack(const Vec& v, float (&f)[VEC]) {
#pragma unroll
    for (int i = 0; i < 4; ++i) {
      f[i] = bf16x4_get(v.lo, i);
      f[4 + i] = bf16x4_get(v.hi, i);
    }
  }
  static __device__ __forceinline__ Vec pack(const float (&f)[VEC]) {
    Vec v;
    v.lo = pack_bf16x4(f[0], f[1], f[2], f[3]);
    v.hi = pack_bf16x4(f[4], f[5], f[6], f[7]);
    return v;
  }
};

template <class T, int DH>
struct RowOp {
  static constexpr int NJ = (DH + 15) / 16;
  typename Lp<T>::Op o[NJ];
};

template <class T, int DH>
__device__ __forceinline__ void load_row_op(RowOp<T, DH>& t, const T* row, int g) {
#pragma unroll
  for (int j = 0; j < RowOp<T, DH>::NJ; ++j) t.o[j] = Lp<T>::ld(row + 16 * j + 4 * g);
}
template <class T, int DH>
__device__ __forceinline__ void load_row_op_scaled(RowOp<T, DH>& t, const T* row, int g, float scale) {
#pragma unroll
  for (int j = 0; j < RowOp<T, DH>::NJ; ++j) t.o[j] = Lp<T>::ld_scaled(row + 16 * j + 4 * g, scale);
}
template <class T, int DH>
__device__ __forceinline__ f32x4 dot_row_ops(const RowOp<T, DH>& a, const RowOp<T, DH>& b, f32x4 acc) {
#pragma unroll
  for (int j = 0; j < RowOp<T, DH>::NJ; ++j) acc = Lp<T>::mma(a.o[j], b.o[j], acc);
  return acc;
}

__device__ __forceinline__ char* lds_bytes() { return reinterpret_cast<char*>(feta_lds); }

}
```

feta_tmlr_amd/csrc/ffn.hip:

```cpp
#include <cstdlib>

#include "feta_abi_common.h"
#include "feta_coeff.h"
#include "feta_ln.h"
#include "feta_lp.h"
#include "feta_rowops.h"

namespace feta {

typedef feta_ffn FfnArgs;

constexpr int kFfnD = 64;
constexpr int kFfnRows = 32;

template <class T>
__host__ __device__ inline int ffn_lds_bytes(int ff) {
  const int pad = Lp<T>::PAD;
  return (int)sizeof(T) * (ff * (kFfnD + pad) + kFfnD * (ff + pad))
         + 4 * (2 * kFfnD
                + reduce_scratch_floats(kFfnD)
                + 4 * 2 * 4 * 64);
}

inline int ffn_grid(int M) {
// ... 106 lines not shown
        if (a.x_rmean != nullptr) {
          const float unbiased = a.M > 1 ? var * (float)a.M / (float)(a.M - 1) : var;
          a.x_rmean[c] = (1.0f - a.momentum) * a.x_rmean[c] + a.momentum * mean;
          a.x_rvar[c] = (1.0f - a.momentum) * a.x_rvar[c] + a.momentum * unbiased;
        }
        if (c == 0 && a.x_nbt != nullptr) *a.x_nbt += 1;
      }
    }
  } else if (a.x_ln_gamma != nullptr) {
    for (int c = tid; c < 2 * D; c += kRowThreads) xss[c] = c < D ? a.x_ln_gamma[c] : a.x_ln_beta[c - D];
  } else {
    for (int c = tid; c < 2 * D; c += kRowThreads) xss[c] = a.x_bn != nullptr ? a.x_bn[c] : (c < D ? 1.0f : 0.0f);
  }
  const bool x_ln = a.x_ln_gamma != nullptr;
  const float ln_eps = a.eps;
  __syncthreads();
  FFN_STAMP(2);
  const bool want_stats = a.y_stats != nullptr;
  float tot1[1] = {0.0f};
  const int lane0 = lane;
  for (int blk = blockIdx.x; blk < nblk; blk += main_grid) {
  int lane_l = lane0;
  FETA_OPAQUE_LANE(lane_l);
  const int lane = lane_l, tid = (wv << 6) | lane, lq = lane & 15, g = lane >> 4;
  if (blk != (int)blockIdx.x) {
    lds_barrier();
    row = blk * kFfnRows + 16 * rt + lq;
    rok = row < a.M;
    rowc = min(row, a.M - 1);
  }
#pragma unroll
  for (int j = 0; j < 4; ++j)
#pragma unroll
    for (int e = 0; e < 4; ++e) xr[j][e] = L::get(xq[j], e);
  if (blk + main_grid < nblk)
    request_x(min((blk + main_grid) * kFfnRows + 16 * rt + lq, a.M - 1));
  RowOp<T, D> xf;
  if (x_ln) {
    float s0 = 0.0f;
#pragma unroll
    for (int j = 0; j < 4; ++j) s0 += (xr[j][0] + xr[j][1]) + (xr[j][2] + xr[j][3]);
    s0 += shfl_xor(s0, 16);
    s0 += shfl_xor(s0, 32);
    const float mean = s0 * (1.0f / D);
    float q0 = 0.0f;
#pragma unroll
    for (int j = 0; j < 4; ++j)
#pragma unroll
      for (int e = 0; e < 4; ++e) {
        xr[j][e] -= mean;
        q0 += xr[j][e] * xr[j][e];
      }
    q0 += shfl_xor(q0, 16);
    q0 += shfl_xor(q0, 32);
    const float rstd = 1.0f / sqrtf(q0 * (1.0f / D) + ln_eps);
#pragma unroll
    for (int j = 0; j < 4; ++j)
#pragma unroll
      for (int e = 0; e < 4; ++e) xr[j][e] *= rstd;
  }
#pragma unroll
  for (int j = 0; j < 4; ++j) {
    const float4 sc = *reinterpret_cast<const float4*>(xss + 16 * j + 4 * g);
    const float4 sh = *reinterpret_cast<const float4*>(xss + D + 16 * j + 4 * g);
    xr[j][0] = xr[j][0] * sc.x + sh.x;
    xr[j][1] = xr[j][1] * sc.y + sh.y;
    xr[j][2] = xr[j][2] * sc.z + sh.z;
    xr[j][3] = xr[j][3] * sc.w + sh.w;
    xf.o[j] = L::mk(xr[j][0], xr[j][1], xr[j][2], xr[j][3]);
  }

  Op ho[HT];
#pragma unroll
  for (int t = 0; t < HT; ++t) {
    const int o = hh * (FF / 2) + 16 * t;
    RowOp<T, D> wf;
    load_row_op<T, D>(wf, W1 + (o + lq) * P1, g);
    f32x4 v = dot_row_ops<T, D>(wf, xf, zero4());
    v[0] = fmaxf(v[0] + b1v[t].x, 0.0f);
    v[1] = fmaxf(v[1] + b1v[t].y, 0.0f);
    v[2] = fmaxf(v[2] + b1v[t].z, 0.0f);
    v[3] = fmaxf(v[3] + b1v[t].w, 0.0f);
    ho[t] = L::mk(v);
    if (rok) L::st4(gh + (int64_t)row * FF + o + 4 * g, v[0], v[1], v[2], v[3]);
  }
  FFN_STAMP(3);
  f32x4 yp[4];
#pragma unroll
  for (int t2 = 0; t2 < 4; ++t2) {
    f32x4 acc = zero4();
#pragma unroll
    for (int t = 0; t < HT; ++t)
      acc = L::mma(L::ld(W2 + (16 * t2 + lq) * P2 + hh * (FF / 2) + 16 * t + 4 * g), ho[t], acc);
    yp[t2] = acc;
  }
  FFN_STAMP(4);
  {
    float* mine = xch + wv * (2 * 4 * 64);
#pragma unroll
    for (int t = 0; t < 2; ++t)
#pragma unroll
      for (int r = 0; r < 4; ++r)
        mine[(t * 4 + r) * 64 + lane] = hh ? yp[t][r] : yp[2 + t][r];
  }
  lds_barrier();
  const float* theirs = xch + (wv ^ 1) * (2 * 4 * 64);
  float* red = scr;
  float vv[2][4];
#pragma unroll
  for (int t = 0; t < 2; ++t) {
    const int t2 = 2 * hh + t, o2 = 16 * t2 + 4 * g;
    const float bb[4] = {b2v[t].x, b2v[t].y, b2v[t].z, b2v[t].w};
    float* v = vv[t];
#pragma unroll
    for (int r = 0; r < 4; ++r) {
      const float own = hh ? yp[2 + t][r] : yp[t][r];
      float x_hi = xr[2 + t][r], x_lo = xr[t][r];
      asm volatile("" : "+v"(x_hi), "+v"(x_lo));
      const float res = hh ? x_hi : x_lo;
      v[r] = own + theirs[(t * 4 + r) * 64 + lane] + bb[r] + res;
    }
    if (rok) {
      if (a.y_f32) *reinterpret_cast<float4*>(a.y + (int64_t)row * D + o2) = make_float4(v[0], v[1], v[2], v[3]);
      else L::st4(gy + (int64_t)row * D + o2, v[0], v[1], v[2], v[3]);
    }
    if (want_stats) {
      const float kk[4] = {ksv[t].x, ksv[t].y, ksv[t].z, ksv[t].w};
#pragma unroll
      for (int r = 0; r < 4; ++r) {
        const float x1 = rok ? v[r] - kk[r] : 0.0f;
        const float s1 = row16_sum(x1), s2 = row16_sum(x1 * x1);
        if (lq == 0) {
          red[(rt * 2 + 0) * D + o2 + r] = s1;
          red[(rt * 2 + 1) * D + o2 + r] = s2;
        }
      }
    }
  }
  if (want_stats) {
    lds_barrier();
    if (tid < 2 * D) tot1[0] += red[tid] + red[2 * D + tid];
  }
  if (y_ln) {
    float* lnx = scr;
    float s1 = ((vv[0][0] + vv[0][1]) + (vv[0][2] + vv[0][3])) + ((vv[1][0] + vv[1][1]) + (vv[1][2] + vv[1][3]));
    s1 += shfl_xor(s1, 16);
    s1 += shfl_xor(s1, 32);
    if (g == 0) lnx[wv * 16 + lq] = s1;
    lds_barrier();
    const float mean = (s1 + lnx[(wv ^ 1) * 16 + lq]) * (1.0f / (float)D);
    float s2 = 0.0f;
#pragma unroll
    for (int t = 0; t < 2; ++t)
#pragma unroll
      for (int r = 0; r < 4; ++r) {
        vv[t][r] -= mean;
        s2 += vv[t][r] * vv[t][r];
      }
    s2 += shfl_xor(s2, 16);
    s2 += shfl_xor(s2, 32);
    if (g == 0) lnx[64 + wv * 16 + lq] = s2;
    lds_barrier();
    const float rstd = rsqrtf((s2 + lnx[64 + (wv ^ 1) * 16 + lq]) * (1.0f / (float)D) + a.y_ln_eps);
    if (rok) {
#pragma unroll
      for (int t = 0; t < 2; ++t) {
        const int o2 = 16 * (2 * hh + t) + 4 * g;
        const float o0 = vv[t][0] * rstd * lgv[t].x + lbv[t].x, o1 = vv[t][1] * rstd * lgv[t].y + lbv[t].y;
        const float o2v = vv[t][2] * rstd * lgv[t].z + lbv[t].z, o3 = vv[t][3] * rstd * lgv[t].w + lbv[t].w;
        if (a.y_ln_f32) *reinterpret_cast<float4*>(a.y_ln_out + (int64_t)row * D + o2) = make_float4(o0, o1, o2v, o3);
        else L::st4(reinterpret_cast<T*>(a.y_ln_out) + (int64_t)row * D + o2, o0, o1, o2v, o3);
      }
    }
  }
  FFN_STAMP(5);
  }
  if (want_stats && tid < 2 * D) a.y_stats[(int64_t)blockIdx.x * 2 * D + tid] = tot1[0];
  if (want_stats && blockIdx.x == 0 && tid < D)
    a.y_stats[(int64_t)main_grid * 2 * D + tid] = a.y_shift != nullptr ? a.y_shift[tid] : 0.0f;
}

template <class T, int FF>
int launch_ffn_fwd(const FfnArgs& a, const CoeffFwdRole& cf, hipStream_t stream) {
  size_t lds = ffn_lds_bytes<T>(FF);
  const int role = cf.attn != nullptr ? cf.B * cf.H : 0;
  if (role > 0 && sizeof(float) * (size_t)coeff_fwd_lds_floats(cf.N) > lds) lds = sizeof(float) * coeff_fwd_lds_floats(cf.N);
  auto kern = ffn_fwd_kernel<T, FF>;
  static LdsSeen lds_seen;
  allow_dynamic_lds(kern, lds, lds_seen);
  const int grid = ffn_grid(a.M);
  hipLaunchKernelGGL(kern, dim3(grid + role), dim3(kRowThreads), lds, stream, a, cf, grid);
  return check_launch("feta_ffn_fwd");
}

template <class T>
int dispatch_ffn_fwd(const FfnArgs& a, const CoeffFwdRole& cf, hipStream_t stream) {
  switch (a.FF) {
    case 64: return launch_ffn_fwd<T, 64>(a, cf, stream);
    case 128: return launch_ffn_fwd<T, 128>(a, cf, stream);
    default: return launch_ffn_fwd<T, 256>(a, cf, stream);
  }
}

}

using namespace feta;

#ifdef FETA_TIMING
extern "C" int feta_debug_ffn_stamps(unsigned long long* out16) {
  return (int)hipMemcpyFromSymbol(out16, HIP_SYMBOL(feta_ffn_stamps), sizeof(unsigned long long) * 16);
}
#endif

extern "C" int feta_ffn_supported(int d_model, int ff) {
  return (d_model == kFfnD && (ff == 64 || ff == 128 || ff == 256)) ? 1 : 0;
}

extern "C" int feta_ffn_blocks(int M) { return ffn_grid(M); }

extern "C" int feta_ffn_fwd(const feta_ffn* d, feta_stream_t stream) { return feta_ffn_fwd_coeff(d, nullptr, stream); }

extern "C" int feta_ffn_fwd_coeff(const feta_ffn* d, const feta_coeff_fwd_role* c, feta_stream_t stream) {
  FETA_REQUIRE(d != nullptr, "ffn_fwd: null descriptor");
  CoeffFwdRole cf{};
  if (c != nullptr) {
    FETA_REQUIRE(c->attn && c->n_real && c->s && c->gcn_bias && c->cj && c->pooled, "ffn_fwd_coeff: null pointer");
    FETA_REQUIRE(c->B > 0 && c->H > 0 && c->C > 0 && c->N > 0 && c->N <= kCoeffThreads,
                 "ffn_fwd_coeff: need 0 < N <= %d (got %d)", kCoeffThreads, c->N);
    cf = CoeffFwdRole{c->attn, c->n_real, c->s, c->gcn_bias, c->cj, c->pooled, c->B, c->N, c->H, c->C};
  }
  const FfnArgs& a = *d;
  FETA_REQUIRE(a.x && a.w1 && a.w2 && a.h && a.y && a.M > 0, "ffn_fwd: null pointer / empty");
  FETA_REQUIRE(feta_ffn_supported(kFfnD, a.FF), "ffn_fwd: dim_feedforward %d not in {64,128,256}", a.FF);
  FETA_REQUIRE(a.x_stats == nullptr || (a.x_gamma && a.x_beta && a.x_bn_out && a.Gx > 0),
               "ffn_fwd: x_stats needs x_gamma, x_beta, x_bn_out, Gx");
  FETA_REQUIRE(a.x_ln_gamma == nullptr || (a.x_ln_beta != nullptr && a.x_stats == nullptr && a.x_bn == nullptr),
               "ffn_fwd: x_ln_gamma needs x_ln_beta and excludes x_bn / x_stats");
  FETA_REQUIRE(aligned16(a.x) && aligned16(a.w1) && aligned16(a.w2) && aligned16(a.h) && aligned16(a.y) &&
                   aligned16(a.b1) && aligned16(a.b2) && aligned16(a.x_stats) && aligned16(a.y_stats),
               "ffn_fwd: tensors must be 16-byte aligned");
  FETA_REQUIRE(a.y_ln_out == nullptr || (a.y_ln_gamma && a.y_ln_beta && a.y_stats == nullptr && aligned16(a.y_ln_out)),
               "ffn_fwd: y_ln_out needs y_ln_gamma, y_ln_beta and excludes y_stats");
  FETA_REQUIRE(a.dtype == FETA_F32 || a.dtype == FETA_BF16, "ffn_fwd: dtype %d", a.dtype);
  if (a.dtype == FETA_BF16) return dispatch_ffn_fwd<bf16_t>(a, cf, (hipStream_t)stream);
  return dispatch_ffn_fwd<float>(a, cf, (hipStream_t)stream);
}
```

feta_tmlr_amd/csrc/ffn_bwd.hip:

```cpp
#include <cstdlib>

#include "feta_abi_common.h"
#include "feta_coeff.h"
#include "feta_ln.h"
#include "feta_lp.h"
#include "feta_rowops.h"

namespace feta {

typedef feta_ffn_grad FfnGradArgs;

constexpr int kFbD = 64;
constexpr int kFbRows = 32;
constexpr int kFbSlice = 32;

struct FfnBwdGeom {
  int XB;
  int RC;
  int per;
  int NS;
  int xcd;
  int wxcd;
  int cxw;
  int main_grid;
// ... 174 lines not shown
    Op wA1[NJ2];
#pragma unroll
    for (int j = 0; j < NJ2; ++j) {
      const float* p = a.w1 + (int64_t)(16 * j + 4 * g) * D + 16 * w + lq;
      wA1[j] = L::mk(p[0], p[D], p[2 * D], p[3 * D]);
    }
    const bool want_sums = a.sum_out != nullptr;
    float mean1[4] = {0.0f, 0.0f, 0.0f, 0.0f}, rstd1[4] = {0.0f, 0.0f, 0.0f, 0.0f};
    if (want_sums) {
#pragma unroll
      for (int r = 0; r < 4; ++r) {
        mean1[r] = a.x_bn[2 * D + 16 * w + 4 * g + r];
        rstd1[r] = a.x_bn[3 * D + 16 * w + 4 * g + r];
      }
    }
    float sum1[4] = {0.0f, 0.0f, 0.0f, 0.0f}, sum2[4] = {0.0f, 0.0f, 0.0f, 0.0f};
    const int nblk = (a.M + kFbRows - 1) / kFbRows;
    const int row_last = a.M - 1;
    constexpr int NU = kFbRows * RV / kRowThreads;
    const int lane0 = lane;
    for (int blk = x_lo; blk < x_hi; blk += x_step) {
      int lane_l = lane0;
      FETA_OPAQUE_LANE(lane_l);
      const int lane = lane_l, tid = (w << 6) | lane, lq = lane & 15, g = lane >> 4;
      const int r0 = blk * kFbRows;
      if (blk != x_lo) __syncthreads();
      float dv[NU][VEC], yv[NU][VEC];
#pragma unroll
      for (int u = 0; u < NU; ++u) {
        const int idx = tid + u * kRowThreads, rr = idx / RV, c4 = idx % RV;
        load_g((int64_t)min(r0 + rr, row_last) * D + VEC * c4, dv[u], yv[u]);
      }
      float hv[2][CT2][4], sy[2][4];
#pragma unroll
      for (int rt = 0; rt < 2; ++rt) {
        const int64_t rowc = min(r0 + 16 * rt + lq, row_last);
#pragma unroll
        for (int t = 0; t < CT2; ++t) L::ld4(ghh + rowc * FF + 16 * (w * CT2 + t) + 4 * g, hv[rt][t]);
        L::ld4(gxx + rowc * D + 16 * w + 4 * g, sy[rt]);
      }
#pragma unroll
      for (int u = 0; u < NU; ++u) {
        const int idx = tid + u * kRowThreads, rr = idx / RV, c4 = idx % RV;
        g2_of<VEC>(dv[u], yv[u], gv, VEC * c4, gbn);
        const bool ok = r0 + rr < a.M;
        if (gln) {
          float dg_[VEC], db_[VEC];
#pragma unroll
          for (int e = 0; e < VEC; ++e) dg_[e] = db_[e] = 0.0f;
          ln_backward<VEC>(dv[u], yv[u], gl2, ln_eps, ok, dg_, db_);
        }
#pragma unroll
        for (int e = 0; e < VEC; ++e) dv[u][e] = ok ? dv[u][e] : 0.0f;
        L::stv(gt + rr * GP + VEC * c4, L::pack(dv[u]));
      }
      __syncthreads();
#pragma unroll
      for (int rt = 0; rt < 2; ++rt) {
        RowOp<T, D> gf;
        load_row_op<T, D>(gf, gt + (16 * rt + lq) * GP, g);
#pragma unroll
        for (int t = 0; t < CT2; ++t) {
          f32x4 acc = zero4();
#pragma unroll
          for (int j = 0; j < 4; ++j) acc = L::mma(wA2[t][j], gf.o[j], acc);
          L::st4(dht + (16 * rt + lq) * DP + 16 * (w * CT2 + t) + 4 * g,
                 hv[rt][t][0] > 0.0f ? acc[0] : 0.0f, hv[rt][t][1] > 0.0f ? acc[1] : 0.0f,
                 hv[rt][t][2] > 0.0f ? acc[2] : 0.0f, hv[rt][t][3] > 0.0f ? acc[3] : 0.0f);
        }
      }
      __syncthreads();
#pragma unroll
      for (int rt = 0; rt < 2; ++rt) {
        RowOp<T, FF> df;
        load_row_op<T, FF>(df, dht + (16 * rt + lq) * DP, g);
        f32x4 acc = zero4();
#pragma unroll
        for (int j = 0; j < NJ2; ++j) acc = L::mma(wA1[j], df.o[j], acc);
        float res[4];
        L::ld4(gt + (16 * rt + lq) * GP + 16 * w + 4 * g, res);
        const float v[4] = {acc[0] + res[0], acc[1] + res[1], acc[2] + res[2], acc[3] + res[3]};
        const int row = r0 + 16 * rt + lq;
        const bool rok = row < a.M;
        if (rok) L::st4(gdx + (int64_t)row * D + 16 * w + 4 * g, v[0], v[1], v[2], v[3]);
        if (want_sums) {
#pragma unroll
          for (int r = 0; r < 4; ++r) {
            const float xh = (sy[rt][r] - mean1[r]) * rstd1[r];
            const float s1 = rok ? v[r] : 0.0f;
            sum1[r] += s1;
            sum2[r] += s1 * xh;
          }
        }
      }
    }
    if (want_sums) {
#pragma unroll
      for (int r = 0; r < 4; ++r) {
        const float s1 = row16_sum(sum1[r]), s2 = row16_sum(sum2[r]);
        if (lq == 0) {
          a.sum_out[((int64_t)xblk * 2 + 0) * D + 16 * w + 4 * g + r] = s1;
          a.sum_out[((int64_t)xblk * 2 + 1) * D + 16 * w + 4 * g + r] = s2;
        }
      }
    }
    return;
  }

  constexpr int GPW = D + FbPad<T>::W, HP = kFbSlice + FbPad<T>::W, HV = kFbSlice / VEC;
  const int bi = wbi;
  const int si = bi % ge.NS, rc = bi / ge.NS;
  const int c0 = kFbSlice * si;
  T* gt = reinterpret_cast<T*>(after);
  T* xt = gt + 64 * GPW;
  T* hs = xt + 64 * GPW;
  T* dhs = hs + 64 * HP;
  Op wA2[2][4];
#pragma unroll
  for (int t = 0; t < 2; ++t)
#pragma unroll
    for (int j = 0; j < 4; ++j) {
      const float* p = a.w2 + (int64_t)(16 * j + 4 * g) * FF + c0 + 16 * t + lq;
      wA2[t][j] = L::mk(p[0], p[FF], p[2 * FF], p[3 * FF]);
    }
  const int row_lo = rc * ge.per * 16, row_hi = min((rc + 1) * ge.per * 16, a.M);
  const int row_last = max(row_hi - 1, 0);
  f32x4 aW2[2] = {zero4(), zero4()}, aW1[2] = {zero4(), zero4()};
  float cs2[VEC], cs1[2][4];
#pragma unroll
  for (int e = 0; e < VEC; ++e) cs2[e] = 0.0f;
#pragma unroll
  for (int t = 0; t < 2; ++t)
#pragma unroll
    for (int r = 0; r < 4; ++r) cs1[t][r] = 0.0f;
  const bool xbn = a.x_bn != nullptr;
  float dgam[VEC], dbet[VEC];
#pragma unroll
  for (int e = 0; e < VEC; ++e) dgam[e] = dbet[e] = 0.0f;
  constexpr int NG = 64 * RV / kRowThreads, NH = 64 * HV / kRowThreads;
  for (int r0 = row_lo; r0 < row_hi; r0 += 64) {
    if (r0 > row_lo) __syncthreads();
    float dv[NG][VEC], yv[NG][VEC];
    Vec xv[NG], hq[NH];
#pragma unroll
    for (int u = 0; u < NG; ++u) {
      const int idx = tid + u * kRowThreads, rr = idx / RV, c4 = idx % RV;
      const int64_t off = (int64_t)min(r0 + rr, row_last) * D + VEC * c4;
      load_g(off, dv[u], yv[u]);
      xv[u] = L::ldv(gxx + off);
    }
#pragma unroll
    for (int u = 0; u < NH; ++u) {
      const int idx = tid + u * kRowThreads, rr = idx / HV, c4 = idx % HV;
      hq[u] = L::ldv(ghh + (int64_t)min(r0 + rr, row_last) * FF + c0 + VEC * c4);
    }
#pragma unroll
    for (int u = 0; u < NG; ++u) {
      const int idx = tid + u * kRowThreads, rr = idx / RV, c4 = idx % RV;
      const bool ok = r0 + rr < row_hi;
      g2_of<VEC>(dv[u], yv[u], gv, VEC * c4, gbn);
      if (gln) ln_backward<VEC>(dv[u], yv[u], gl2, ln_eps, ok, dgam, dbet);
      float x[VEC];
      L::unpack(xv[u], x);
      if (xln) ln_apply<VEC>(x, gl1, bl1, ln_eps);
      if (xbn) {
#pragma unroll
        for (int e4 = 0; e4 < VEC; e4 += 4) {
          const float4 sc = *reinterpret_cast<const float4*>(a.x_bn + VEC * c4 + e4);
          const float4 sh = *reinterpret_cast<const float4*>(a.x_bn + D + VEC * c4 + e4);
          x[e4] = x[e4] * sc.x + sh.x;
          x[e4 + 1] = x[e4 + 1] * sc.y + sh.y;
          x[e4 + 2] = x[e4 + 2] * sc.z + sh.z;
          x[e4 + 3] = x[e4 + 3] * sc.w + sh.w;
        }
      }
#pragma unroll
      for (int e = 0; e < VEC; ++e) {
        dv[u][e] = ok ? dv[u][e] : 0.0f;
        cs2[e] += dv[u][e];
        x[e] = ok ? x[e] : 0.0f;
      }
      L::stv(gt + rr * GPW + VEC * c4, L::pack(dv[u]));
      L::stv(xt + rr * GPW + VEC * c4, L::pack(x));
    }
#pragma unroll
    for (int u = 0; u < NH; ++u) {
      const int idx = tid + u * kRowThreads, rr = idx / HV, c4 = idx % HV;
      const bool ok = r0 + rr < row_hi;
      float hf[VEC];
      L::unpack(hq[u], hf);
#pragma unroll
      for (int e = 0; e < VEC; ++e) hf[e] = ok ? hf[e] : 0.0f;
      L::stv(hs + rr * HP + VEC * c4, L::pack(hf));
    }
    __syncthreads();
    {
      RowOp<T, D> gf;
      load_row_op<T, D>(gf, gt + (16 * w + lq) * GPW, g);
#pragma unroll
      for (int t = 0; t < 2; ++t) {
        f32x4 acc = zero4();
#pragma unroll
        for (int j = 0; j < 4; ++j) acc = L::mma(wA2[t][j], gf.o[j], acc);
        float hh[4];
        L::ld4(hs + (16 * w + lq) * HP + 16 * t + 4 * g, hh);
        const float dm[4] = {hh[0] > 0.0f ? acc[0] : 0.0f, hh[1] > 0.0f ? acc[1] : 0.0f, hh[2] > 0.0f ? acc[2] : 0.0f,
                             hh[3] > 0.0f ? acc[3] : 0.0f};
        L::st4(dhs + (16 * w + lq) * HP + 16 * t + 4 * g, dm[0], dm[1], dm[2], dm[3]);
#pragma unroll
        for (int r = 0; r < 4; ++r) cs1[t][r] += dm[r];
      }
    }
    __syncthreads();
#pragma unroll 2
    for (int q = 0; q < 4; ++q) {
      const int rr = 16 * q + g;
      const Op ga = L::gather(gt + rr * GPW + 16 * w + lq, 4 * GPW);
      const Op xb = L::gather(xt + rr * GPW + 16 * w + lq, 4 * GPW);
#pragma unroll
      for (int ct = 0; ct < 2; ++ct) {
        const Op hb = L::gather(hs + rr * HP + 16 * ct + lq, 4 * HP);
        const Op da = L::gather(dhs + rr * HP + 16 * ct + lq, 4 * HP);
        aW2[ct] = L::mma(ga, hb, aW2[ct]);
        aW1[ct] = L::mma(da, xb, aW1[ct]);
      }
    }
  }
  float* p = a.partial + (int64_t)rc * (a.partial_ld > 0 ? (int64_t)a.partial_ld
                                                         : (int64_t)(2 * D * FF + D + FF + (gln ? 2 * D : 0)));
  float* pW2 = p;
  float* pb2 = p + D * FF;
  float* pW1 = pb2 + D;
  float* pb1 = pW1 + FF * D;
#pragma unroll
  for (int ct = 0; ct < 2; ++ct)
#pragma unroll
    for (int r = 0; r < 4; ++r) {
      pW2[(int64_t)(16 * w + 4 * g + r) * FF + c0 + 16 * ct + lq] = aW2[ct][r];
      pW1[(int64_t)(c0 + 16 * ct + 4 * g + r) * D + 16 * w + lq] = aW1[ct][r];
    }
  __syncthreads();
  float* red2 = after;
  float* red1 = after + kRowThreads * VEC;
  float* red3 = red1 + 4 * 2 * 16;
  float* red4 = red3 + kRowThreads * VEC;
  if (gln && si == 0) {
#pragma unroll
    for (int e = 0; e < VEC; ++e) {
      red3[tid * VEC + e] = dgam[e];
      red4[tid * VEC + e] = dbet[e];
    }
  }
#pragma unroll
  for (int e = 0; e < VEC; ++e) red2[tid * VEC + e] = cs2[e];
#pragma unroll
  for (int t = 0; t < 2; ++t)
#pragma unroll
    for (int r = 0; r < 4; ++r) {
      const float sv = row16_sum(cs1[t][r]);
      if (lq == 0) red1[(w * 2 + t) * 16 + 4 * g + r] = sv;
    }
  __syncthreads();
  if (si == 0 && tid < D) {
    const int c4 = tid / VEC, e = tid % VEC;
    float sv = 0.0f;
    for (int k = 0; k < kRowThreads / RV; ++k) sv += red2[(c4 + RV * k) * VEC + e];
    pb2[tid] = sv;
    if (gln) {
      float sg = 0.0f, sb = 0.0f;
      for (int k = 0; k < kRowThreads / RV; ++k) {
        sg += red3[(c4 + RV * k) * VEC + e];
        sb += red4[(c4 + RV * k) * VEC + e];
      }
      pb1[FF + tid] = sg;
      pb1[FF + D + tid] = sb;
    }
  }
  if (tid < kFbSlice) {
    const int t = tid >> 4, cc = tid & 15;
    pb1[c0 + tid] = (red1[(0 * 2 + t) * 16 + cc] + red1[(1 * 2 + t) * 16 + cc]) +
                    (red1[(2 * 2 + t) * 16 + cc] + red1[(3 * 2 + t) * 16 + cc]);
  }
}

extern int row_chunks(int M);

static int ffn_bwd_main_grid(int M, int RC, int NS) {
  const int XB = ffn_bwd_xblocks(M), nblk = (M + kFbRows - 1) / kFbRows, nrb16 = (M + 15) / 16;
  const int per = (nrb16 + RC - 1) / RC;
  const bool xcd = XB == nblk && per == 4;
  return xcd ? 8 * ((RC + 7) / 8) * (2 + NS) : XB + 8 * ((RC + 7) / 8) * NS;
}
static int ffn_bwd_chunks_for(int M, int ff) {
  const int rc = row_chunks(M), ns = ff / kFbSlice;
  if (const char* e = getenv("FETA_FFN_BWD_RC_HALF"))
    if (atoi(e) == 0) return rc;
  const int half = (rc + 1) / 2;
  if (rc >= 2 && ffn_bwd_main_grid(M, rc, ns) > 512 && ffn_bwd_main_grid(M, half, ns) <= 512) return half;
  return rc;
}

template <class T, int FF>
int launch_ffn_bwd(const FfnGradArgs& a, const CoeffBwdRole& cb, hipStream_t stream) {
  FfnBwdGeom ge{};
  ge.XB = ffn_bwd_xblocks(a.M);
  ge.RC = ffn_bwd_chunks_for(a.M, FF);
  const int nrb16 = (a.M + 15) / 16;
  ge.per = (nrb16 + ge.RC - 1) / ge.RC;
  ge.NS = FF / kFbSlice;
  size_t lds = ffn_bwd_lds_bytes<T>(FF, a.g_bn != nullptr);
  const bool saved = cb.A != nullptr;
  const int role = (cb.cj != nullptr || saved) ? ((cb.C + kCoeffThreads - 1) / kCoeffThreads) * cb.G : 0;
  if (role > 0 && !saved && sizeof(float) * (size_t)(kCoeffPass * cb.N) > lds) lds = sizeof(float) * (size_t)(kCoeffPass * cb.N);
  auto kern = ffn_bwd_kernel<T, FF>;
  static LdsSeen seen;
  allow_dynamic_lds(kern, lds, seen);
  const int nblk = (a.M + kFbRows - 1) / kFbRows;
  ge.xcd = (ge.XB == nblk && ge.per == 4) ? 1 : 0;
  if (const char* e = getenv("FETA_FFN_BWD_XCD")) ge.xcd = ge.xcd && atoi(e) != 0;
  ge.wxcd = ge.xcd ? 0 : 1;
  if (const char* e = getenv("FETA_FFN_BWD_WXCD")) ge.wxcd = ge.wxcd && atoi(e) != 0;
  ge.cxw = 0;
  if (const char* e = getenv("FETA_FFN_BWD_CXW")) {
    if (atoi(e) != 0 && !ge.xcd && ge.wxcd && ge.per % 2 == 0 && ge.XB >= ge.RC && ge.XB % ge.RC == 0) ge.cxw = ge.XB / ge.RC;
  }
  if (ge.cxw > 0) ge.wxcd = 0;
  const int grid = ge.xcd ? 8 * ((ge.RC + 7) / 8) * (2 + ge.NS)
                 : ge.cxw > 0 ? 8 * ((ge.RC + 7) / 8) * (ge.cxw + ge.NS)
                              : ge.XB + (ge.wxcd ? 8 * ((ge.RC + 7) / 8) * ge.NS : ge.RC * ge.NS);
  ge.main_grid = grid;
  ge.role = role;
  ge.role_lead = 8 * ((role + 7) / 8);
  if (const char* e = getenv("FETA_COEFF_ROLE_FIRST")) if (atoi(e) == 0) ge.role_lead = 0;
  if (saved) {
    const char* e = getenv("FETA_COEFF_SAVED_LEAD");
    if (e == nullptr || atoi(e) == 0) ge.role_lead = 0;
  }
  hipLaunchKernelGGL(kern, dim3(grid + (ge.role_lead > 0 ? ge.role_lead : role)), dim3(kRowThreads), lds, stream, a, ge, cb);
  return check_launch("feta_ffn_bwd");
}

}

using namespace feta;

extern "C" int feta_ffn_bwd_supported(int d_model, int ff) { return (d_model == kFbD && (ff == 64 || ff == 128)) ? 1 : 0; }

extern "C" int feta_ffn_bwd_blocks(int M) { return ffn_bwd_xblocks(M); }
extern "C" int feta_ffn_bwd_chunks(int M, int ff) { return (M < 1 || !feta_ffn_bwd_supported(kFbD, ff)) ? 0 : ffn_bwd_chunks_for(M, ff); }

static int ffn_bwd_checked(const feta_ffn_grad* d, const CoeffBwdRole& cb, feta_stream_t stream);

extern "C" int feta_ffn_bwd(const feta_ffn_grad* d, feta_stream_t stream) { return feta_ffn_bwd_coeff(d, nullptr, stream); }

extern "C" int feta_ffn_bwd_coeff(const feta_ffn_grad* d, const feta_coeff_bwd_role* c, feta_stream_t stream) {
  FETA_REQUIRE(d != nullptr, "ffn_bwd: null descriptor");
  CoeffBwdRole cb{};
  if (c != nullptr) {
    FETA_REQUIRE(c->cj && c->n_real && c->s && c->gcn_bias && c->dpooled && c->partial, "ffn_bwd_coeff: null pointer");
    FETA_REQUIRE(c->B > 0 && c->H > 0 && c->C > 0 && c->N > 0, "ffn_bwd_coeff: empty shape");
    cb = CoeffBwdRole{c->cj, c->n_real, c->s, c->gcn_bias, c->dpooled, c->partial, c->B, c->N, c->H, c->C,
                      feta_coeff_bwd_groups(c->B, c->H), nullptr, nullptr};
  }
  return ffn_bwd_checked(d, cb, stream);
// ... 33 lines not shown
```

feta_tmlr_amd/csrc/filter.hip:

```cpp
#include <cstdlib>

#include "feta_abi_common.h"
#include "feta_coeff.h"
#include "feta_rowops.h"
#include "feta_tiles.h"

namespace feta {

struct FilterArgs {
  const float* x;
  const float* lhat;
  const float* u;
  const float* lam;
  const float* coeff;
  const float* bias;
  const int32_t* n_real;
  const float* dy;
  float* y;
  float* dx;
  float* dcoeff;
  float* dbias_part;
  int64_t xsb, xsn, ysb, ysn;
  int B, N, H, P, K;
  int share;
// ... 1409 lines not shown

  f32x4 xtT[ET_MAX];
#pragma unroll
  for (int et = 0; et < ET_MAX; ++et) xtT[et] = zero4();
#pragma unroll
  for (int nt = 0; nt < NT_MAX; ++nt) {
    if (16 * nt < n) {
#pragma unroll
      for (int r = 0; r < 4; ++r) {
        const int nd = 16 * nt + 4 * g + r;
        const float xa = Xs[nd * XP + DH * h + lq];
#pragma unroll
        for (int et = 0; et < ET_MAX; ++et) xtT[et] = mfma16(xa, Us[nd * UP + 16 * et + lq], xtT[et]);
      }
    }
  }
  f32x4 yt[ET_MAX];
#pragma unroll
  for (int et = 0; et < ET_MAX; ++et) {
    float tk[kMaxOrder];
    cheb_poly(lams[16 * et + lq], PP, tk);
    yt[et] = zero4();
#pragma unroll
    for (int k = 0; k < PP; ++k)
#pragma unroll
      for (int r = 0; r < 4; ++r)
        yt[et] = mfma16(xtT[et][r] * tk[k], Ws[(k * DH + 4 * g + r) * WP + lq], yt[et]);
#pragma unroll
    for (int r = 0; r < 4; ++r) YT[(16 * et + 4 * g + r) * YP + DH * h + lq] = yt[et][r];
  }
  __syncthreads();
  f32x4 ytp[ET_MAX];
#pragma unroll
  for (int et = 0; et < ET_MAX; ++et) {
    Feat<D> yf;
    load_row<D>(yf, YT + (16 * et + lq) * YP, g);
    ytp[et] = dot_rows<D>(yf, wbf, zero4());
  }
  float cbo = 0.0f;
#pragma unroll
  for (int j = 0; j < 4; ++j)
    cbo += (wbf.f[j][0] * bs4.x + wbf.f[j][1] * bs4.y) + (wbf.f[j][2] * bs4.z + wbf.f[j][3] * bs4.w);
  cbo += shfl_xor(cbo, 16);
  cbo += shfl_xor(cbo, 32);
  f32x4 y[NT_MAX], o[NT_MAX];
#pragma unroll
  for (int nt = 0; nt < NT_MAX; ++nt) {
    y[nt] = zero4();
    o[nt] = zero4();
    if (16 * nt < a.N) {
      Feat<D> xf;
      load_row<D>(xf, Ys + (16 * nt + lq) * XP, g);
      o[nt] = dot_rows<D>(xf, waf, zero4());
    }
    if (16 * nt < n) {
#pragma unroll
      for (int et = 0; et < ET_MAX; ++et) {
        const float4 ub = *reinterpret_cast<const float4*>(Us + (16 * nt + lq) * UP + 16 * et + 4 * g);
        y[nt] = mfma16(ub.x, yt[et][0], y[nt]);
        y[nt] = mfma16(ub.y, yt[et][1], y[nt]);
        y[nt] = mfma16(ub.z, yt[et][2], y[nt]);
        y[nt] = mfma16(ub.w, yt[et][3], y[nt]);
        o[nt] = mfma16(ub.x, ytp[et][0], o[nt]);
        o[nt] = mfma16(ub.y, ytp[et][1], o[nt]);
        o[nt] = mfma16(ub.z, ytp[et][2], o[nt]);
        o[nt] = mfma16(ub.w, ytp[et][3], o[nt]);
      }
    }
  }
  __syncthreads();
#pragma unroll
  for (int nt = 0; nt < NT_MAX; ++nt)
#pragma unroll
    for (int r = 0; r < 4; ++r) {
      const int nd = 16 * nt + 4 * g + r;
      Xs[nd * XP + DH * h + lq] = nd < n ? y[nt][r] + bv : 0.0f;
      Ys[nd * XP + DH * h + lq] = o[nt][r] + bcat + (nd < n ? cbo : 0.0f);
    }
  __syncthreads();
#pragma unroll
  for (int i = 0; i < NT_MAX; ++i) {
    const int idx = tid + 256 * i, node = idx >> 4, q = idx & 15;
    if (node < a.N) {
      *reinterpret_cast<float4*>(tok_row(a.y, a.ysb, a.ysn, b, node, 0, DH) + 4 * q) =
          *reinterpret_cast<const float4*>(Xs + node * XP + 4 * q);
      *reinterpret_cast<float4*>(tok_row(c.out, a.ysb, a.ysn, b, node, 0, DH) + 4 * q) =
          *reinterpret_cast<const float4*>(Ys + node * XP + 4 * q);
    }
  }
}

constexpr int kCatRoleWalkMax = 2;
template <int NT_MAX, int ET_MAX>
int spec_cat_fwd_slots() {
  static int slots = 0;
  if (slots == 0) {
    const size_t lds = sizeof(float) * spec_cat_fwd_lds_floats<NT_MAX, ET_MAX>(4);
    auto kern = spec_cat_fwd_graph_kernel<NT_MAX, ET_MAX, 4, true>;
    static LdsSeen lds_seen;
    allow_dynamic_lds(kern, lds, lds_seen);
    int dev = 0, cus = 0, per = 0;
    if (hipGetDevice(&dev) != hipSuccess || hipDeviceGetAttribute(&cus, hipDeviceAttributeMultiprocessorCount, dev) != hipSuccess ||
        hipOccupancyMaxActiveBlocksPerMultiprocessor(&per, kern, 256, lds) != hipSuccess || cus < 1 || per < 1) {
      (void)hipGetLastError();
      return 0;
    }
    slots = cus * per;
  }
  return slots;
}
inline int spec_cat_fwd_role_grid(int slots, int B, int total) {
  if (const char* e = getenv("FETA_COEFF_DSUM_WGS")) if (atoi(e) > 0) return atoi(e) < total ? atoi(e) : total;
  if (slots < 1) return 0;
  const int free_slots = slots - B % slots;
  const int grid = total < free_slots ? total : free_slots;
  return (total + grid - 1) / grid <= kCatRoleWalkMax ? grid : 0;
}

template <int NT_MAX, int ET_MAX>
int launch_spec_cat_fwd(const FilterArgs& a, const CatArgs& c, const CoeffDsumRole* cr, hipStream_t stream) {
  size_t lds = sizeof(float) * spec_cat_fwd_lds_floats<NT_MAX, ET_MAX>(4);
  if constexpr (NT_MAX <= 4) {
    if (a.H == 8) {
      auto kern = spec_cat_fwd_graph_kernel<NT_MAX, ET_MAX, 4, false, true>;
      static LdsSeen lds_seen;
      allow_dynamic_lds(kern, lds, lds_seen);
      hipLaunchKernelGGL(kern, dim3(a.B), dim3(256), lds, stream, a, c, CoeffDsumHost<false>{});
      return check_launch("feta_spec_filter_cat_fwd");
    }
    if (cr != nullptr) {
      if (sizeof(float) * (size_t)cr->N > lds) lds = sizeof(float) * (size_t)cr->N;
      const int role = spec_cat_fwd_role_grid(spec_cat_fwd_slots<NT_MAX, ET_MAX>(), a.B, cr->B * cr->H);
      FETA_REQUIRE(role > 0, "spec_filter_cat_fwd_coeff: %d blocks do not fit the slots %d graphs leave free (feta_spec_cat_fwd_coeff_fits)",
                   cr->B * cr->H, a.B);
      auto kern = spec_cat_fwd_graph_kernel<NT_MAX, ET_MAX, 4, true>;
      static LdsSeen lds_seen;
      allow_dynamic_lds(kern, lds, lds_seen);
      hipLaunchKernelGGL(kern, dim3(a.B + role), dim3(256), lds, stream, a, c, CoeffDsumHost<true>{*cr, role});
      return check_launch("feta_spec_filter_cat_fwd_coeff");
    }
  }
  auto kern = spec_cat_fwd_graph_kernel<NT_MAX, ET_MAX, 4, false>;
  static LdsSeen lds_seen;
  allow_dynamic_lds(kern, lds, lds_seen);
  hipLaunchKernelGGL(kern, dim3(a.B), dim3(256), lds, stream, a, c, CoeffDsumHost<false>{});
  return check_launch("feta_spec_filter_cat_fwd");
}

constexpr int kCatBwdMaxGrid = 512;
inline int spec_cat_bwd_rows(int B) { return B < kCatBwdMaxGrid ? B : kCatBwdMaxGrid; }

struct CatGradArgs {
  const float* dout;
  const float* y2;
  int64_t y2sb, y2sn;
  const float* y2_bn;
  const float* filt;
  const float* w_cat;
  float* dxn;
  float* gs;
  float* partial;
  int64_t partial_ld;
};

template <int NT_MAX, int ET_MAX>
__host__ __device__ inline int spec_cat_bwd_lds_floats() {
  constexpr int NR = 16 * NT_MAX, UP = 16 * ET_MAX + 4;
  return 2 * NR * kGraphXP + NR * UP + 16 * ET_MAX + 16 * ET_MAX * (kCatD + 4) + 2 * kCatD;
}

// ... 616 lines not shown
```

Measured before the change: 517,900 graphs/s.

## Tag global stores with cache policies by data lifetime (saved, handoff, partial)

Measured after the change: 529,900 graphs/s (median of 6 runs). 2.3% higher.

```diff
diff --git a/feta_tmlr_amd/build.py b/feta_tmlr_amd/build.py
--- a/feta_tmlr_amd/build.py
+++ b/feta_tmlr_amd/build.py
@@ -31,6 +31,7 @@
     os.makedirs(OBJ, exist_ok=True)
     flags = ['--offload-arch=' + ARCH, '-O3', '-std=c++17', '-fPIC',
              '-I' + os.path.join(ROOT, 'include'), '-I' + CSRC]
+    flags += os.environ.get('FETA_HIPCC_FLAGS', '').split()
     if report:
         flags.append('-Rpass-analysis=kernel-resource-usage')
     dep_t = max(os.path.getmtime(p) for p in _deps())
diff --git a/feta_tmlr_amd/csrc/block.hip b/feta_tmlr_amd/csrc/block.hip
--- a/feta_tmlr_amd/csrc/block.hip
+++ b/feta_tmlr_amd/csrc/block.hip
@@ -219,7 +219,7 @@
           t[0] += bv4.x; t[1] += bv4.y; t[2] += bv4.z; t[3] += bv4.w;
           if (node < a.N) {
             const int64_t row = (int64_t)b * a.row_sb + (int64_t)node * a.row_sn;
-            L::st4(gqkv + row * 3 * D + part * D + DH * h + 4 * g, t[0], t[1], t[2], t[3]);
+            L::template gst4<kStSaved>(gqkv + row * 3 * D + part * D + DH * h + 4 * g, t[0], t[1], t[2], t[3]);
           }
           if (part == 0) {
             qs[nt] = L::mk(t[0] * a.scale, t[1] * a.scale, t[2] * a.scale, t[3] * a.scale);
@@ -235,7 +235,7 @@
             const int nd = 16 * nt + 4 * g + r;
             if (nd < a.N) {
               const int64_t row = (int64_t)b * a.row_sb + (int64_t)nd * a.row_sn;
-              L::st1(gqkv + row * 3 * D + 2 * D + DH * h + lq, t[r]);
+              L::template gst1<kStSaved>(gqkv + row * 3 * D + 2 * D + DH * h + lq, t[r]);
             }
             if (nd >= n) t[r] = 0.0f;
           }
@@ -310,8 +310,8 @@
     const int q = 16 * qb + lq;
     if (g == 0 && q < a.N) {
       float* st = a.attn_stats + ((int64_t)bh * a.N + q) * 2;
-      st[0] = mx[qb];
-      st[1] = zs[qb];
+      gst1<kStSaved>(st, mx[qb]);
+      gst1<kStSaved>(st + 1, zs[qb]);
     }
   }
 #pragma unroll
@@ -340,7 +340,7 @@
       float* dst = a.attn + ((int64_t)bh * a.N + 16 * qb) * a.N;
       for (int i = lane; i < rows * a.N; i += 64) {
         const int qq = i / a.N, kk = i - qq * a.N;
-        dst[i] = stg[qq * KP + kk];
+        gst1<kStSaved>(dst + i, stg[qq * KP + kk]);
       }
       wave_lds_sync();
     }
@@ -355,13 +355,13 @@
     if (node < a.N) {
       const int64_t row = (int64_t)b * a.row_sb + (int64_t)node * a.row_sn;
       const Vec ov = L::ldv(Os + node * P + L::VEC * q);
-      L::stv(gout + row * D + L::VEC * q, ov);
+      L::template gstv<kStSaved>(gout + row * D + L::VEC * q, ov);
       if (a.out_f32 != nullptr) {
         float f[L::VEC];
         L::unpack(ov, f);
 #pragma unroll
         for (int e = 0; e < L::VEC; e += 4)
-          *reinterpret_cast<float4*>(a.out_f32 + row * D + L::VEC * q + e) = make_float4(f[e], f[e + 1], f[e + 2], f[e + 3]);
+          gst4<kStSaved>(a.out_f32 + row * D + L::VEC * q + e, f[e], f[e + 1], f[e + 2], f[e + 3]);
       }
     }
   }
@@ -387,7 +387,7 @@
       L::ld4(Xs + node * P + o0, res);
       float v[4] = {(t[0] + bo.x) * rs + res[0], (t[1] + bo.y) * rs + res[1], (t[2] + bo.z) * rs + res[2],
                     (t[3] + bo.w) * rs + res[3]};
-      if (rok) L::st4(gy + row * D + o0, v[0], v[1], v[2], v[3]);
+      if (rok) L::template gst4<kStHandoff>(gy + row * D + o0, v[0], v[1], v[2], v[3]);
       if (a.y_stats != nullptr) {
 #pragma unroll
         for (int r = 0; r < 4; ++r) {
@@ -399,9 +399,9 @@
     }
     if (lq == 0 && a.y_stats != nullptr) {
       float* st = a.y_stats + (int64_t)b * 2 * D;
-      *reinterpret_cast<float4*>(st + o0) = make_float4(s1[0], s1[1], s1[2], s1[3]);
-      *reinterpret_cast<float4*>(st + D + o0) = make_float4(s2[0], s2[1], s2[2], s2[3]);
-      if (b == 0) *reinterpret_cast<float4*>(a.y_stats + (int64_t)a.B * 2 * D + o0) = ks;
+      gst4<kStHandoff>(st + o0, s1[0], s1[1], s1[2], s1[3]);
+      gst4<kStHandoff>(st + D + o0, s2[0], s2[1], s2[2], s2[3]);
+      if (b == 0) gst4<kStHandoff>(a.y_stats + (int64_t)a.B * 2 * D + o0, ks.x, ks.y, ks.z, ks.w);
     }
   }
   }
@@ -615,7 +615,7 @@
         t[0] += binq.x; t[1] += binq.y; t[2] += binq.z; t[3] += binq.w;
         if (node < a.N) {
           const int64_t row = (int64_t)b * a.row_sb + (int64_t)node * a.row_sn;
-          L::st4(gqkv + row * 3 * D + DH * h + 4 * g, t[0], t[1], t[2], t[3]);
+          L::template gst4<kStSaved>(gqkv + row * 3 * D + DH * h + 4 * g, t[0], t[1], t[2], t[3]);
         }
         qs[nt / S] = L::mk(t[0] * a.scale, t[1] * a.scale, t[2] * a.scale, t[3] * a.scale);
       }
@@ -634,7 +634,7 @@
           t[0] += bink.x; t[1] += bink.y; t[2] += bink.z; t[3] += bink.w;
           if (!a.tie_qk && node < a.N && (nt % WGS) == w) {
             const int64_t row = (int64_t)b * a.row_sb + (int64_t)node * a.row_sn;
-            L::st4(gqkv + row * 3 * D + D + DH * h + 4 * g, t[0], t[1], t[2], t[3]);
+            L::template gst4<kStSaved>(gqkv + row * 3 * D + D + DH * h + 4 * g, t[0], t[1], t[2], t[3]);
           }
           kk = L::mk(t);
         }
@@ -656,7 +656,7 @@
             const int nd = 16 * nt + 4 * g + r;
             if (nd < a.N && (nt % WGS) == w) {
               const int64_t row = (int64_t)b * a.row_sb + (int64_t)nd * a.row_sn;
-              L::st1(gqkv + row * 3 * D + 2 * D + DH * h + lq, t[r]);
+              L::template gst1<kStSaved>(gqkv + row * 3 * D + 2 * D + DH * h + lq, t[r]);
             }
             if (nd >= n) t[r] = 0.0f;
           }
@@ -734,8 +734,8 @@
     const int qb = slot + S * i, q = 16 * qb + lq;
     if (g == 0 && qb < NT && q < a.N) {
       float* st = a.attn_stats + ((int64_t)bh * a.N + q) * 2;
-      st[0] = mx[i];
-      st[1] = zs[i];
+      gst1<kStSaved>(st, mx[i]);
+      gst1<kStSaved>(st + 1, zs[i]);
     }
   }
 #pragma unroll
@@ -772,7 +772,7 @@
       float* dst = a.attn + ((int64_t)bh * a.N + 16 * qb) * a.N;
       for (int j = lane; j < rows * a.N; j += 64) {
         const int qq = j / a.N, kk = j - qq * a.N;
-        dst[j] = stg[qq * KP + kk];
+        gst1<kStSaved>(dst + j, stg[qq * KP + kk]);
       }
       wave_lds_sync();
     }
@@ -841,8 +841,8 @@
     const int qb = slot + S * i, q = 16 * qb + lq;
     if (g == 0 && qb < NT && q < a.N) {
       float* st = a.attn_stats + ((int64_t)bh * a.N + q) * 2;
-      st[0] = mx[i];
-      st[1] = zs[i];
+      gst1<kStSaved>(st, mx[i]);
+      gst1<kStSaved>(st + 1, zs[i]);
     }
   }
 #pragma unroll
@@ -882,7 +882,7 @@
       float* dst = a.attn + ((int64_t)bh * a.N + 16 * qb) * a.N;
       for (int j = lane; j < rows * a.N; j += 64) {
         const int qq = j / a.N, kk = j - qq * a.N;
-        dst[j] = stg[qq * KP + kk];
+        gst1<kStSaved>(dst + j, stg[qq * KP + kk]);
       }
       wave_lds_sync();
     }
@@ -901,13 +901,13 @@
     if (node < a.N && (((node >> 4) & (S - 1)) >> 1) == w) {
       const int64_t row = (int64_t)b * a.row_sb + (int64_t)node * a.row_sn;
       const Vec ov = L::ldv(Os + node * P + L::VEC * q);
-      L::stv(gout + row * D + L::VEC * q, ov);
+      L::template gstv<kStSaved>(gout + row * D + L::VEC * q, ov);
       if (a.out_f32 != nullptr) {
         float f[L::VEC];
         L::unpack(ov, f);
 #pragma unroll
         for (int e = 0; e < L::VEC; e += 4)
-          *reinterpret_cast<float4*>(a.out_f32 + row * D + L::VEC * q + e) = make_float4(f[e], f[e + 1], f[e + 2], f[e + 3]);
+          gst4<kStSaved>(a.out_f32 + row * D + L::VEC * q + e, f[e], f[e + 1], f[e + 2], f[e + 3]);
       }
     }
   }
@@ -933,7 +933,7 @@
       L::ld4(Xs + node * P + o0, res);
       float v[4] = {(t[0] + bo.x) * rs + res[0], (t[1] + bo.y) * rs + res[1], (t[2] + bo.z) * rs + res[2],
                     (t[3] + bo.w) * rs + res[3]};
-      if (rok) L::st4(gy + row * D + o0, v[0], v[1], v[2], v[3]);
+      if (rok) L::template gst4<kStHandoff>(gy + row * D + o0, v[0], v[1], v[2], v[3]);
       if (a.y_stats != nullptr) {
 #pragma unroll
         for (int r = 0; r < 4; ++r) {
@@ -957,12 +957,12 @@
       const float* e = sx + (4 * h + g) * 8;
       const float4 t1 = *reinterpret_cast<const float4*>(e), t2 = *reinterpret_cast<const float4*>(e + 4);
       float* st = a.y_stats + ((int64_t)b0 * WGS + w) * 2 * D;
-      *reinterpret_cast<float4*>(st + o0) = make_float4(s1[0] + t1.x, s1[1] + t1.y, s1[2] + t1.z, s1[3] + t1.w);
-      *reinterpret_cast<float4*>(st + D + o0) = make_float4(s2[0] + t2.x, s2[1] + t2.y, s2[2] + t2.z, s2[3] + t2.w);
+      gst4<kStHandoff>(st + o0, s1[0] + t1.x, s1[1] + t1.y, s1[2] + t1.z, s1[3] + t1.w);
+      gst4<kStHandoff>(st + D + o0, s2[0] + t2.x, s2[1] + t2.y, s2[2] + t2.z, s2[3] + t2.w);
       if (b0 == 0 && w == 0) {
         float4 ks = make_float4(0.0f, 0.0f, 0.0f, 0.0f);
         if (a.y_shift != nullptr) ks = *reinterpret_cast<const float4*>(a.y_shift + o0);
-        *reinterpret_cast<float4*>(a.y_stats + (int64_t)gp * WGS * 2 * D + o0) = ks;
+        gst4<kStHandoff>(a.y_stats + (int64_t)gp * WGS * 2 * D + o0, ks.x, ks.y, ks.z, ks.w);
       }
     }
   }
diff --git a/feta_tmlr_amd/csrc/block_bwd.hip b/feta_tmlr_amd/csrc/block_bwd.hip
--- a/feta_tmlr_amd/csrc/block_bwd.hip
+++ b/feta_tmlr_amd/csrc/block_bwd.hip
@@ -34,8 +34,9 @@
 #endif
 #define BB_STAMP(i) FETA_RT_STAMP(feta_bbwd_stamps, feta_bbwd_launch, i)
 
+template <int POL>
 __device__ __forceinline__ void acc_to(float* p, float v, bool first) {
-  if (first) *p = v;
+  if (first) gst1<POL>(p, v);
   else atomicAdd(p, v);
 }
 
@@ -44,6 +45,7 @@
 template <class T, int NT, bool SPLIT, bool LOOP, bool TWO, bool DW = false>
 __global__ __launch_bounds__(kBbThreads) void attn_block_bwd_kernel(BwdArgs a, ColsumPlan sums, int main_grid, LinDwHost<DW> dw) {
   static_assert(!DW || (std::is_same<T, float>::value && !SPLIT && !LOOP), "the dW role: fp32, one workgroup per graph");
+  constexpr int kPr = LOOP ? kStPlain : kStPartial;
   if ((int)blockIdx.x >= main_grid) {
     int rb = (int)blockIdx.x - main_grid;
     if constexpr (DW) {
@@ -323,14 +325,14 @@
       float sv = 0.0f;
 #pragma unroll
       for (int w8 = 0; w8 < 8; ++w8) sv += DBO[w8 * D + tid];
-      acc_to(prow + D * D + tid, sv, first);
+      acc_to<kPr>(prow + D * D + tid, sv, first);
     }
     if (gln && hp == 0 && tid >= D && tid < 3 * D) {
       const int which = (tid - D) / D, c = (tid - D) % D;
       float sv = 0.0f;
 #pragma unroll
       for (int w8 = 0; w8 < 8; ++w8) sv += DGL[(w8 * 2 + which) * D + c];
-      acc_to(prow + 4 * D * D + 4 * D + which * D + c, sv, first);
+      acc_to<kPr>(prow + 4 * D * D + 4 * D + which * D + c, sv, first);
     }
 
     {
@@ -599,7 +601,7 @@
 #pragma unroll
         for (int r = 0; r < 4; ++r)
         {
-          acc_to(prow + (int64_t)(16 * ot + 4 * g + r) * D + 16 * (SPLIT ? 2 * hp + i : i) + lq, aWo[i][r], first);
+          acc_to<kPr>(prow + (int64_t)(16 * ot + 4 * g + r) * D + 16 * (SPLIT ? 2 * hp + i : i) + lq, aWo[i][r], first);
         }
     }
     BB_STAMP(4);
@@ -659,7 +661,7 @@
       L::ld4(Gt + rowl * P + 16 * ktile + 4 * g, res);
       const float v[4] = {acc[0] + resw * res[0], acc[1] + resw * res[1], acc[2] + resw * res[2], acc[3] + resw * res[3]};
       const bool rok = rowl < a.N;
-      if (rok) L::st4(dxo + grow(rowl) * D + 16 * ktile + 4 * g, v[0], v[1], v[2], v[3]);
+      if (rok) L::template gst4<kStHandoff>(dxo + grow(rowl) * D + 16 * ktile + 4 * g, v[0], v[1], v[2], v[3]);
       if (want_sums) {
         float xx[4];
         L::ld4(X0 + rowl * P + 16 * ktile + 4 * g, xx);
@@ -691,16 +693,16 @@
         if ((wv >> 2) == 0 && lq == 0) {
 #pragma unroll
           for (int r = 0; r < 4; ++r) {
-            a.sum_out[((int64_t)blockIdx.x * 2 + 0) * D + 16 * ktile + 4 * g + r] = s1v[r] + red[(ktile * 2 + 0) * 16 + 4 * g + r];
-            a.sum_out[((int64_t)blockIdx.x * 2 + 1) * D + 16 * ktile + 4 * g + r] = s2v[r] + red[(ktile * 2 + 1) * 16 + 4 * g + r];
+            gst1<kStHandoff>(a.sum_out + ((int64_t)blockIdx.x * 2 + 0) * D + 16 * ktile + 4 * g + r, s1v[r] + red[(ktile * 2 + 0) * 16 + 4 * g + r]);
+            gst1<kStHandoff>(a.sum_out + ((int64_t)blockIdx.x * 2 + 1) * D + 16 * ktile + 4 * g + r, s2v[r] + red[(ktile * 2 + 1) * 16 + 4 * g + r]);
           }
         }
       } else if (lq == 0 && (!LOOP || b + nwg >= a.B)) {
         const int64_t prow2 = (int64_t)blockIdx.x * 2 + (wv >> 2);
 #pragma unroll
         for (int r = 0; r < 4; ++r) {
-          a.sum_out[(prow2 * 2 + 0) * D + 16 * ktile + 4 * g + r] = s1v[r];
-          a.sum_out[(prow2 * 2 + 1) * D + 16 * ktile + 4 * g + r] = s2v[r];
+          gst1<kStHandoff>(a.sum_out + (prow2 * 2 + 0) * D + 16 * ktile + 4 * g + r, s1v[r]);
+          gst1<kStHandoff>(a.sum_out + (prow2 * 2 + 1) * D + 16 * ktile + 4 * g + r, s2v[r]);
         }
       }
     }
@@ -734,7 +736,7 @@
 #pragma unroll
       for (int r = 0; r < 4; ++r)
       {
-        acc_to(pWi + (int64_t)(64 * wi_part(i) + 16 * wi_head(i) + 4 * g + r) * D + 16 * ktile + lq, aWi[i][r], first);
+        acc_to<kPr>(pWi + (int64_t)(64 * wi_part(i) + 16 * wi_head(i) + 4 * g + r) * D + 16 * ktile + lq, aWi[i][r], first);
       }
     if (tid < 3 * D) {
       const int part = tid >> 6, hh = (tid >> 4) & 3, c = tid & 15;
@@ -742,10 +744,10 @@
       if (SPLIT) {
         if ((hh >> 1) == hp) {
           const int wa = (hh & 1) + 2 * rl;
-          pbi[tid] = DBS[(wa * 2 + which) * 16 + c] + DBS[((wa + 4) * 2 + which) * 16 + c];
+          gst1<kStPartial>(pbi + tid, DBS[(wa * 2 + which) * 16 + c] + DBS[((wa + 4) * 2 + which) * 16 + c]);
         }
       } else {
-        acc_to(pbi + tid, DBS[((hh + 4 * rl) * 2 + which) * 16 + c], first);
+        acc_to<kPr>(pbi + tid, DBS[((hh + 4 * rl) * 2 + which) * 16 + c], first);
       }
     }
     b += nwg;
diff --git a/feta_tmlr_amd/csrc/feta_coeff.h b/feta_tmlr_amd/csrc/feta_coeff.h
--- a/feta_tmlr_amd/csrc/feta_coeff.h
+++ b/feta_tmlr_amd/csrc/feta_coeff.h
@@ -3,6 +3,7 @@
 
 #include "feta_abi_common.h"
 #include <feta_device.h>
+#include "feta_gstore.h"
 
 namespace feta {
 
@@ -65,7 +66,7 @@
       float c = 0.0f;
       if (col < n) c = ((ps[col] + ps[64 + col]) + (ps[128 + col] + ps[192 + col])) * dis[col];
       cjs[col] = c;
-      if (cs == 0) cj_out[(int64_t)blk * N + col] = c;
+      if (cs == 0) gst1<kStSaved>(cj_out + (int64_t)blk * N + col, c);
     }
     __syncthreads();
   } else if (stage == 2) {
@@ -142,7 +143,7 @@
         c = (c + diag0 * dj) * dj;
       }
       cjs[j] = c;
-      if (cs == 0) cj_out[(int64_t)blk * N + j] = c;
+      if (cs == 0) gst1<kStSaved>(cj_out + (int64_t)blk * N + j, c);
     }
     __syncthreads();
   } else {
@@ -180,7 +181,7 @@
         c *= dis[j];
       }
       cjs[j] = c;
-      if (cs == 0) cj_out[(int64_t)blk * N + j] = c;
+      if (cs == 0) gst1<kStSaved>(cj_out + (int64_t)blk * N + j, c);
     }
     __syncthreads();
   }
@@ -192,7 +193,7 @@
       const float sc = s[c], bc = gbias[c];
       float acc = 0.0f;
       for (int i = 0; i < n; ++i) acc += fast_tanh(cjs[i] * sc + bc);
-      pooled[(int64_t)blk * C + c] = acc * inv_n;
+      gst1<kStSaved>(pooled + (int64_t)blk * C + c, acc * inv_n);
     }
     return;
   }
@@ -214,7 +215,7 @@
 #pragma unroll
     for (int k = 0; k < 4; ++k) {
       const int c = c0 + k * TH;
-      if (c < cend) pooled[(int64_t)blk * C + c] = acc[k] * inv_n;
+      if (c < cend) gst1<kStSaved>(pooled + (int64_t)blk * C + c, acc[k] * inv_n);
     }
   }
 }
@@ -289,8 +290,8 @@
     }
   }
   if (c < C) {
-    partial[(int64_t)grp * 2 * C + c] = as;
-    partial[(int64_t)grp * 2 * C + C + c] = ab;
+    gst1<kStPartial>(partial + (int64_t)grp * 2 * C + c, as);
+    gst1<kStPartial>(partial + (int64_t)grp * 2 * C + C + c, ab);
   }
 }
 
@@ -328,8 +329,8 @@
     for (int k = 0; k < 4; ++k) {
       const int c = c0 + k * kCoeffThreads;
       if (c < C) {
-        A[(int64_t)blk * C + c] = as[k] * inv_n;
-        Bm[(int64_t)blk * C + c] = ab[k] * inv_n;
+        gst1<kStSaved>(A + (int64_t)blk * C + c, as[k] * inv_n);
+        gst1<kStSaved>(Bm + (int64_t)blk * C + c, ab[k] * inv_n);
       }
     }
   }
@@ -364,8 +365,8 @@
     }
   }
   if (c < C) {
-    partial[(int64_t)grp * 2 * C + c] = as;
-    partial[(int64_t)grp * 2 * C + C + c] = ab;
+    gst1<kStPartial>(partial + (int64_t)grp * 2 * C + c, as);
+    gst1<kStPartial>(partial + (int64_t)grp * 2 * C + C + c, ab);
   }
 }
 
diff --git a/feta_tmlr_amd/csrc/feta_colsum.h b/feta_tmlr_amd/csrc/feta_colsum.h
--- a/feta_tmlr_amd/csrc/feta_colsum.h
+++ b/feta_tmlr_amd/csrc/feta_colsum.h
@@ -3,6 +3,7 @@
 
 #include "feta_abi_common.h"
 #include <feta_device.h>
+#include "feta_gstore.h"
 
 namespace feta {
 
@@ -90,7 +91,7 @@
       }
       acc = red[tid % WQ];
     }
-    if (ok && slice == 0) *reinterpret_cast<float4*>(s.out + 4 * (int64_t)c4) = acc;
+    if (ok && slice == 0) gst4<kStPartial>(s.out + 4 * (int64_t)c4, acc.x, acc.y, acc.z, acc.w);
     return;
   }
   constexpr int COLS = 16, SL = THREADS / COLS;
@@ -116,7 +117,7 @@
   }
   if (col < s.C) {
     const float v = red[lc];
-    if (slice == 0) s.out[col] = v;
+    if (slice == 0) gst1<kStPartial>(s.out + col, v);
     if (s.bcast_out != nullptr)
       for (int r = slice; r < s.bcast_rows; r += SL) s.bcast_out[(int64_t)r * s.C + col] = v;
   }
diff --git a/feta_tmlr_amd/csrc/feta_device.h b/feta_tmlr_amd/csrc/feta_device.h
--- a/feta_tmlr_amd/csrc/feta_device.h
+++ b/feta_tmlr_amd/csrc/feta_device.h
@@ -96,6 +96,40 @@
   __builtin_amdgcn_fence(__ATOMIC_ACQUIRE, "workgroup", "local");
 }
 
+constexpr int kStPlain = 0, kStWt = 1, kStNt = 2;
+typedef unsigned long long __attribute__((address_space(1)))* feta_gu64;
+typedef unsigned int __attribute__((address_space(1)))* feta_gu32;
+template <int POL>
+__device__ __forceinline__ void gst_b128(void* p, f32x4 v) {
+  if constexpr (POL == kStWt) {
+    asm volatile("global_store_dwordx4 %0, %1, off sc1\n\ts_nop 1" : : "v"(p), "v"(v) : "memory");
+  } else if constexpr (POL == kStNt) {
+    __builtin_nontemporal_store(v, reinterpret_cast<f32x4*>(p));
+  } else {
+    *reinterpret_cast<f32x4*>(p) = v;
+  }
+}
+template <int POL>
+__device__ __forceinline__ void gst_b64(void* p, unsigned long long v) {
+  if constexpr (POL == kStWt) {
+    __hip_atomic_store((feta_gu64)p, v, __ATOMIC_RELAXED, __HIP_MEMORY_SCOPE_AGENT);
+  } else if constexpr (POL == kStNt) {
+    __builtin_nontemporal_store(v, reinterpret_cast<unsigned long long*>(p));
+  } else {
+    *reinterpret_cast<unsigned long long*>(p) = v;
+  }
+}
+template <int POL>
+__device__ __forceinline__ void gst_b32(void* p, float v) {
+  if constexpr (POL == kStWt) {
+    __hip_atomic_store((feta_gu32)p, __builtin_bit_cast(unsigned, v), __ATOMIC_RELAXED, __HIP_MEMORY_SCOPE_AGENT);
+  } else if constexpr (POL == kStNt) {
+    __builtin_nontemporal_store(v, reinterpret_cast<float*>(p));
+  } else {
+    *reinterpret_cast<float*>(p) = v;
+  }
+}
+
 __device__ __forceinline__ float fast_exp(float x) { return __expf(x); }
 __device__ __forceinline__ float fast_tanh(float x) {
   return 1.0f - 2.0f * __builtin_amdgcn_rcpf(1.0f + __expf(2.0f * x));
diff --git a/feta_tmlr_amd/csrc/feta_gstore.h b/feta_tmlr_amd/csrc/feta_gstore.h
--- /dev/null
+++ b/feta_tmlr_amd/csrc/feta_gstore.h
@@ -0,0 +1,39 @@
+#pragma once
+#include <feta_device.h>
+
+#ifndef FETA_ST_SAVED
+#define FETA_ST_SAVED 1
+#endif
+#ifndef FETA_ST_PARTIAL
+#define FETA_ST_PARTIAL 1
+#endif
+#ifndef FETA_ST_HANDOFF
+#define FETA_ST_HANDOFF 0
+#endif
+#ifndef FETA_ST_BF16
+#define FETA_ST_BF16 0
+#endif
+
+namespace feta {
+
+constexpr int kStSaved = FETA_ST_SAVED, kStPartial = FETA_ST_PARTIAL, kStHandoff = FETA_ST_HANDOFF;
+
+template <int POL>
+__device__ __forceinline__ void gst1(float* p, float v) {
+  gst_b32<POL>(p, v);
+}
+template <int POL>
+__device__ __forceinline__ void gst2(float* p, float a, float b) {
+  const float t[2] = {a, b};
+  unsigned long long u;
+  __builtin_memcpy(&u, t, 8);
+  gst_b64<POL>(p, u);
+}
+template <int POL>
+__device__ __forceinline__ void gst4(float* p, float a, float b, float c, float d) {
+  f32x4 v;
+  v[0] = a; v[1] = b; v[2] = c; v[3] = d;
+  gst_b128<POL>(p, v);
+}
+
+}
diff --git a/feta_tmlr_amd/csrc/feta_lin_dw.h b/feta_tmlr_amd/csrc/feta_lin_dw.h
--- a/feta_tmlr_amd/csrc/feta_lin_dw.h
+++ b/feta_tmlr_amd/csrc/feta_lin_dw.h
@@ -1,6 +1,7 @@
 #pragma once
 #include "feta_abi_common.h"
 #include <feta_device.h>
+#include "feta_gstore.h"
 #include "feta_tiles.h"
 
 namespace feta {
@@ -123,11 +124,8 @@
   float* out = a.dw + (int64_t)(i0 + 32 * iw + 8 * g) * a.K + j0 + 32 * jw + 2 * lq;
 #pragma unroll
   for (int r = 0; r < 4; ++r) {
-    float2 v0, v1;
-    v0.x = a00[r]; v0.y = a01[r];
-    v1.x = a10[r]; v1.y = a11[r];
-    *reinterpret_cast<float2*>(out + (int64_t)(2 * r) * a.K) = v0;
-    *reinterpret_cast<float2*>(out + (int64_t)(2 * r + 1) * a.K) = v1;
+    gst2<kStPartial>(out + (int64_t)(2 * r) * a.K, a00[r], a01[r]);
+    gst2<kStPartial>(out + (int64_t)(2 * r + 1) * a.K, a10[r], a11[r]);
   }
   if (a.db != nullptr && tj == 0) {
     float* red = feta_lds;
@@ -138,7 +136,7 @@
       const int c4 = threadIdx.x >> 2, e = threadIdx.x & 3;
       float sv = 0.0f;
       for (int k = 0; k < kDwThreads / 32; ++k) sv += red[(c4 + 32 * k) * 4 + e];
-      a.db[i0 + threadIdx.x] = sv;
+      gst1<kStPartial>(a.db + i0 + threadIdx.x, sv);
     }
   }
 }
diff --git a/feta_tmlr_amd/csrc/feta_lp.h b/feta_tmlr_amd/csrc/feta_lp.h
--- a/feta_tmlr_amd/csrc/feta_lp.h
+++ b/feta_tmlr_amd/csrc/feta_lp.h
@@ -1,4 +1,5 @@
 #pragma once
+#include "feta_gstore.h"
 #include "feta_tiles.h"
 
 namespace feta {
@@ -56,6 +57,12 @@
   }
   static __device__ __forceinline__ Vec ldv(const float* p) { return Vec{*reinterpret_cast<const float4*>(p)}; }
   static __device__ __forceinline__ void stv(float* p, const Vec& v) { *reinterpret_cast<float4*>(p) = v.raw; }
+  template <int POL>
+  static __device__ __forceinline__ void gst1(float* p, float v) { feta::gst1<POL>(p, v); }
+  template <int POL>
+  static __device__ __forceinline__ void gst4(float* p, float a, float b, float c, float d) { feta::gst4<POL>(p, a, b, c, d); }
+  template <int POL>
+  static __device__ __forceinline__ void gstv(float* p, const Vec& v) { feta::gst4<POL>(p, v.raw.x, v.raw.y, v.raw.z, v.raw.w); }
   static __device__ __forceinline__ void unpack(const Vec& v, float (&f)[VEC]) {
     f[0] = v.raw.x; f[1] = v.raw.y; f[2] = v.raw.z; f[3] = v.raw.w;
   }
@@ -103,6 +110,22 @@
   }
   static __device__ __forceinline__ Vec ldv(const bf16_t* p) { return *reinterpret_cast<const Vec*>(p); }
   static __device__ __forceinline__ void stv(bf16_t* p, const Vec& v) { *reinterpret_cast<Vec*>(p) = v; }
+  static constexpr int pol(int p) { return FETA_ST_BF16 ? p : kStPlain; }
+  template <int POL>
+  static __device__ __forceinline__ void gst1(bf16_t* p, float v) { st1(p, v); }
+  template <int POL>
+  static __device__ __forceinline__ void gst4(bf16_t* p, float a, float b, float c, float d) {
+    const bf16x4_pk t = pack_bf16x4(a, b, c, d);
+    unsigned long long u;
+    __builtin_memcpy(&u, &t, 8);
+    gst_b64<pol(POL)>(p, u);
+  }
+  template <int POL>
+  static __device__ __forceinline__ void gstv(bf16_t* p, const Vec& v) {
+    f32x4 t;
+    __builtin_memcpy(&t, &v, 16);
+    gst_b128<pol(POL)>(p, t);
+  }
   static __device__ __forceinline__ void unpack(const Vec& v, float (&f)[VEC]) {
 #pragma unroll
     for (int i = 0; i < 4; ++i) {
diff --git a/feta_tmlr_amd/csrc/ffn.hip b/feta_tmlr_amd/csrc/ffn.hip
--- a/feta_tmlr_amd/csrc/ffn.hip
+++ b/feta_tmlr_amd/csrc/ffn.hip
@@ -212,7 +212,7 @@
     v[2] = fmaxf(v[2] + b1v[t].z, 0.0f);
     v[3] = fmaxf(v[3] + b1v[t].w, 0.0f);
     ho[t] = L::mk(v);
-    if (rok) L::st4(gh + (int64_t)row * FF + o + 4 * g, v[0], v[1], v[2], v[3]);
+    if (rok) L::template gst4<kStSaved>(gh + (int64_t)row * FF + o + 4 * g, v[0], v[1], v[2], v[3]);
   }
   FFN_STAMP(3);
   f32x4 yp[4];
@@ -251,8 +251,8 @@
       v[r] = own + theirs[(t * 4 + r) * 64 + lane] + bb[r] + res;
     }
     if (rok) {
-      if (a.y_f32) *reinterpret_cast<float4*>(a.y + (int64_t)row * D + o2) = make_float4(v[0], v[1], v[2], v[3]);
-      else L::st4(gy + (int64_t)row * D + o2, v[0], v[1], v[2], v[3]);
+      if (a.y_f32) gst4<kStHandoff>(a.y + (int64_t)row * D + o2, v[0], v[1], v[2], v[3]);
+      else L::template gst4<kStHandoff>(gy + (int64_t)row * D + o2, v[0], v[1], v[2], v[3]);
     }
     if (want_stats) {
       const float kk[4] = {ksv[t].x, ksv[t].y, ksv[t].z, ksv[t].w};
@@ -298,16 +298,16 @@
         const int o2 = 16 * (2 * hh + t) + 4 * g;
         const float o0 = vv[t][0] * rstd * lgv[t].x + lbv[t].x, o1 = vv[t][1] * rstd * lgv[t].y + lbv[t].y;
         const float o2v = vv[t][2] * rstd * lgv[t].z + lbv[t].z, o3 = vv[t][3] * rstd * lgv[t].w + lbv[t].w;
-        if (a.y_ln_f32) *reinterpret_cast<float4*>(a.y_ln_out + (int64_t)row * D + o2) = make_float4(o0, o1, o2v, o3);
-        else L::st4(reinterpret_cast<T*>(a.y_ln_out) + (int64_t)row * D + o2, o0, o1, o2v, o3);
+        if (a.y_ln_f32) gst4<kStHandoff>(a.y_ln_out + (int64_t)row * D + o2, o0, o1, o2v, o3);
+        else L::template gst4<kStHandoff>(reinterpret_cast<T*>(a.y_ln_out) + (int64_t)row * D + o2, o0, o1, o2v, o3);
       }
     }
   }
   FFN_STAMP(5);
   }
-  if (want_stats && tid < 2 * D) a.y_stats[(int64_t)blockIdx.x * 2 * D + tid] = tot1[0];
+  if (want_stats && tid < 2 * D) gst1<kStHandoff>(a.y_stats + (int64_t)blockIdx.x * 2 * D + tid, tot1[0]);
   if (want_stats && blockIdx.x == 0 && tid < D)
-    a.y_stats[(int64_t)main_grid * 2 * D + tid] = a.y_shift != nullptr ? a.y_shift[tid] : 0.0f;
+    gst1<kStHandoff>(a.y_stats + (int64_t)main_grid * 2 * D + tid, a.y_shift != nullptr ? a.y_shift[tid] : 0.0f);
 }
 
 template <class T, int FF>
diff --git a/feta_tmlr_amd/csrc/ffn_bwd.hip b/feta_tmlr_amd/csrc/ffn_bwd.hip
--- a/feta_tmlr_amd/csrc/ffn_bwd.hip
+++ b/feta_tmlr_amd/csrc/ffn_bwd.hip
@@ -280,7 +280,7 @@
         const float v[4] = {acc[0] + res[0], acc[1] + res[1], acc[2] + res[2], acc[3] + res[3]};
         const int row = r0 + 16 * rt + lq;
         const bool rok = row < a.M;
-        if (rok) L::st4(gdx + (int64_t)row * D + 16 * w + 4 * g, v[0], v[1], v[2], v[3]);
+        if (rok) L::template gst4<kStHandoff>(gdx + (int64_t)row * D + 16 * w + 4 * g, v[0], v[1], v[2], v[3]);
         if (want_sums) {
 #pragma unroll
           for (int r = 0; r < 4; ++r) {
@@ -297,8 +297,8 @@
       for (int r = 0; r < 4; ++r) {
         const float s1 = row16_sum(sum1[r]), s2 = row16_sum(sum2[r]);
         if (lq == 0) {
-          a.sum_out[((int64_t)xblk * 2 + 0) * D + 16 * w + 4 * g + r] = s1;
-          a.sum_out[((int64_t)xblk * 2 + 1) * D + 16 * w + 4 * g + r] = s2;
+          gst1<kStHandoff>(a.sum_out + ((int64_t)xblk * 2 + 0) * D + 16 * w + 4 * g + r, s1);
+          gst1<kStHandoff>(a.sum_out + ((int64_t)xblk * 2 + 1) * D + 16 * w + 4 * g + r, s2);
         }
       }
     }
@@ -434,8 +434,8 @@
   for (int ct = 0; ct < 2; ++ct)
 #pragma unroll
     for (int r = 0; r < 4; ++r) {
-      pW2[(int64_t)(16 * w + 4 * g + r) * FF + c0 + 16 * ct + lq] = aW2[ct][r];
-      pW1[(int64_t)(c0 + 16 * ct + 4 * g + r) * D + 16 * w + lq] = aW1[ct][r];
+      gst1<kStPartial>(pW2 + (int64_t)(16 * w + 4 * g + r) * FF + c0 + 16 * ct + lq, aW2[ct][r]);
+      gst1<kStPartial>(pW1 + (int64_t)(c0 + 16 * ct + 4 * g + r) * D + 16 * w + lq, aW1[ct][r]);
     }
   __syncthreads();
   float* red2 = after;
@@ -463,21 +463,21 @@
     const int c4 = tid / VEC, e = tid % VEC;
     float sv = 0.0f;
     for (int k = 0; k < kRowThreads / RV; ++k) sv += red2[(c4 + RV * k) * VEC + e];
-    pb2[tid] = sv;
+    gst1<kStPartial>(pb2 + tid, sv);
     if (gln) {
       float sg = 0.0f, sb = 0.0f;
       for (int k = 0; k < kRowThreads / RV; ++k) {
         sg += red3[(c4 + RV * k) * VEC + e];
         sb += red4[(c4 + RV * k) * VEC + e];
       }
-      pb1[FF + tid] = sg;
-      pb1[FF + D + tid] = sb;
+      gst1<kStPartial>(pb1 + FF + tid, sg);
+      gst1<kStPartial>(pb1 + FF + D + tid, sb);
     }
   }
   if (tid < kFbSlice) {
     const int t = tid >> 4, cc = tid & 15;
-    pb1[c0 + tid] = (red1[(0 * 2 + t) * 16 + cc] + red1[(1 * 2 + t) * 16 + cc]) +
-                    (red1[(2 * 2 + t) * 16 + cc] + red1[(3 * 2 + t) * 16 + cc]);
+    gst1<kStPartial>(pb1 + c0 + tid, (red1[(0 * 2 + t) * 16 + cc] + red1[(1 * 2 + t) * 16 + cc]) +
+                                         (red1[(2 * 2 + t) * 16 + cc] + red1[(3 * 2 + t) * 16 + cc]));
   }
 }
 
diff --git a/feta_tmlr_amd/csrc/filter.hip b/feta_tmlr_amd/csrc/filter.hip
--- a/feta_tmlr_amd/csrc/filter.hip
+++ b/feta_tmlr_amd/csrc/filter.hip
@@ -1515,10 +1515,10 @@
   for (int i = 0; i < NT_MAX; ++i) {
     const int idx = tid + 256 * i, node = idx >> 4, q = idx & 15;
     if (node < a.N) {
-      *reinterpret_cast<float4*>(tok_row(a.y, a.ysb, a.ysn, b, node, 0, DH) + 4 * q) =
-          *reinterpret_cast<const float4*>(Xs + node * XP + 4 * q);
-      *reinterpret_cast<float4*>(tok_row(c.out, a.ysb, a.ysn, b, node, 0, DH) + 4 * q) =
-          *reinterpret_cast<const float4*>(Ys + node * XP + 4 * q);
+      const float4 fv = *reinterpret_cast<const float4*>(Xs + node * XP + 4 * q);
+      const float4 ov = *reinterpret_cast<const float4*>(Ys + node * XP + 4 * q);
+      gst4<kStHandoff>(tok_row(a.y, a.ysb, a.ysn, b, node, 0, DH) + 4 * q, fv.x, fv.y, fv.z, fv.w);
+      gst4<kStHandoff>(tok_row(c.out, a.ysb, a.ysn, b, node, 0, DH) + 4 * q, ov.x, ov.y, ov.z, ov.w);
     }
   }
 }
```
